# iracigt/ceres-raytracer

Measured on AMD Instinct MI355X. Metric: Mrays/sec (primary+shadow) on dragon.obj 1920x1080; 1/2/4/8-GPU scaling, higher is better.
Workload: dtype f32; 1 GPU; dragon_1080: dragon.obj 1920x1080 primary+shadow, 16 copies of the config view per step; views=config, W=1920, H=1080, row_block=1080, parallelism=one GPU, whole frames, float_framebuffer=True, streams=8

## Files before the change

ceres-raytracer_amd/__init__.py:

```python
import ctypes
import os
import sys

import numpy as np

_PKG = os.path.dirname(os.path.abspath(__file__))
LIB_PATH = os.environ.get("CERES_LIB") or os.path.join(_PKG, "libceres_hip.so")
CLI_PATH = os.path.join(_PKG, "render")

if _PKG not in sys.path:
    sys.path.insert(0, _PKG)
import configs

MODE_FULL, MODE_PRIMARY = 0, 1
MODE_ROBUST = 0x10
MODE_QBVH4 = 0x20
MODE_FMA = 0x40
ARITH_EXACT, ARITH_FMA = 0, 1


def cfg_mode(cfg, arith=ARITH_EXACT):
    return ((MODE_PRIMARY if cfg["mode"] == "primary" else MODE_FULL) | (MODE_ROBUST if cfg.get("robust") else 0)
            | (MODE_FMA if arith else 0))
SCENE_STATS = 1
SCENE_FIRST_ORDER = 2

EXPORTED_SYMBOLS = (
    "ceres_obj_load", "ceres_proc_mesh", "ceres_rotate_triangles", "ceres_bvh_build", "ceres_bvh_build_gpu",
    "ceres_bvh_build_device", "ceres_obj_load_gpu", "ceres_obj_parse_device", "ceres_rotate_triangles_device",
    "ceres_device_free", "ceres_camera_basis", "ceres_obj_load_f64", "ceres_proc_mesh_f64", "ceres_rotate_triangles_f64",
    "ceres_bvh_build_f64", "ceres_camera_basis_f64", "ceres_orbit_cameras_f64", "ceres_scene_create_f64",
    "ceres_render_f64", "ceres_render_records_f64", "ceres_obj_load_f64_arith", "ceres_proc_mesh_f64_arith",
    "ceres_rotate_triangles_f64_arith", "ceres_bvh_build_f64_arith", "ceres_camera_basis_f64_arith",
    "ceres_orbit_cameras_f64_arith",
    "ceres_free", "ceres_scene_create", "ceres_scene_create_device", "ceres_scene_destroy", "ceres_scene_info", "ceres_scene_shadow_stacks", "ceres_render_f32",
    "ceres_render_device", "ceres_render_batch_device", "ceres_render_multi_f32", "ceres_device_count", "ceres_assemble_rgb8_packed", "ceres_render_records", "ceres_tiling_local_rows",
    "ceres_scene_set_timing", "ceres_scene_read_timing", "ceres_scene_wave_log", "ceres_fetch_counters",
    "ceres_debug_compact_order", "ceres_debug_kept_tiles",
    "ceres_cpu_scene_create", "ceres_cpu_scene_destroy", "ceres_render_cpu_f32", "ceres_cpu_scene_create_f64",
    "ceres_render_cpu_f64",
    "ceres_orbit_cameras", "ceres_assemble_rgb8",
    "ceres_kernel_names", "ceres_last_error", "ceres_version",
    "ceres_obj_load_arith", "ceres_proc_mesh_arith", "ceres_rotate_triangles_arith", "ceres_bvh_build_arith",
    "ceres_camera_basis_arith", "ceres_orbit_cameras_arith", "ceres_content_hash",
    "ceres_bvh_build_gpu_arith", "ceres_bvh_build_device_arith", "ceres_obj_load_gpu_arith",
    "ceres_obj_parse_device_arith", "ceres_rotate_triangles_device_arith",
    "ceres_trace_rays", "ceres_trace_rays_device", "ceres_trace_rays_cpu",
    "ceres_trace_rays_f64", "ceres_trace_rays_f64_device", "ceres_trace_rays_cpu_f64",
    "ceres_shade_rays", "ceres_shade_rays_device", "ceres_shade_rays_cpu", "ceres_camera_rays",
    "ceres_shade_rays_f64", "ceres_shade_rays_f64_device", "ceres_shade_rays_cpu_f64", "ceres_camera_rays_f64",
    "ceres_scene_refit", "ceres_scene_refit_device", "ceres_scene_refit_f64", "ceres_scene_refit_f64_device",
    "ceres_cpu_scene_refit", "ceres_cpu_scene_refit_f64", "ceres_scene_read_boxes",
    "ceres_scene_sah_cost", "ceres_scene_rebuild", "ceres_scene_rebuild_device", "ceres_scene_update",
    "ceres_scene_update_device", "ceres_cpu_scene_sah_cost", "ceres_cpu_scene_rebuild", "ceres_cpu_scene_rebuild_f64",
    "ceres_cpu_scene_update", "ceres_cpu_scene_update_f64",
)

HIT_DTYPE = np.dtype([("prim", np.int32), ("t", np.float32), ("u", np.float32), ("v", np.float32)])
FLT_MAX = np.float32(np.finfo(np.float32).max)
HIT64_DTYPE = np.dtype([("prim", np.int32), ("pad", np.uint32), ("t", np.float64), ("u", np.float64), ("v", np.float64)])
DBL_MAX = np.float64(np.finfo(np.float64).max)


class CeresError(RuntimeError):
    pass


class _Stats(ctypes.Structure):
    _fields_ = [("rays", ctypes.c_uint64), ("hits", ctypes.c_uint64), ("primary_rays", ctypes.c_uint64),
                ("shadow_rays", ctypes.c_uint64), ("node_pairs", ctypes.c_uint64), ("tri_tests", ctypes.c_uint64),
                ("ms", ctypes.c_double)]


class _UpdateInfo(ctypes.Structure):
    _fields_ = [("cost", ctypes.c_double), ("built_cost", ctypes.c_double), ("new_cost", ctypes.c_double),
                ("rebuilt", ctypes.c_int32), ("reserved", ctypes.c_int32)]

    def as_dict(self):
        return dict(cost=self.cost, built_cost=self.built_cost, new_cost=self.new_cost, rebuilt=int(self.rebuilt))


class Tiling(ctypes.Structure):
    _fields_ = [("row_block", ctypes.c_uint32), ("rank", ctypes.c_uint32), ("world", ctypes.c_uint32),
                ("bands", ctypes.c_uint32)]


_lib = None
_fp = ctypes.POINTER(ctypes.c_float)
_dp = ctypes.POINTER(ctypes.c_double)
_u32p = ctypes.POINTER(ctypes.c_uint32)
_u64p = ctypes.POINTER(ctypes.c_uint64)
_sz = ctypes.c_size_t
_vp = ctypes.c_void_p


def build(verbose=False):
    import subprocess
    r = subprocess.run(["make", "-C", os.path.join(_PKG, "csrc"), "-j4", "all"], capture_output=True, text=True)
    if verbose or r.returncode:
        sys.stdout.write(r.stdout)
        sys.stderr.write(r.stderr)
    if r.returncode:
        raise CeresError("build of libceres_hip.so failed")


def lib():
    global _lib
    if _lib is not None:
        return _lib
    if not os.path.exists(LIB_PATH):
        raise CeresError(f"{LIB_PATH} is missing: run __graft_entry__.build() (no CPU fallback exists)")
    if "torch" not in sys.modules:
        try:
            import torch
        except ImportError:
            pass
    L = ctypes.CDLL(LIB_PATH)
    L.ceres_last_error.restype = ctypes.c_char_p
    L.ceres_version.restype = ctypes.c_char_p
    L.ceres_kernel_names.restype = ctypes.c_char_p
    L.ceres_obj_load.argtypes = [ctypes.c_char_p, ctypes.POINTER(_fp), ctypes.POINTER(_fp), ctypes.POINTER(_sz)]
    L.ceres_proc_mesh.argtypes = [ctypes.c_int, ctypes.POINTER(_fp), ctypes.POINTER(_fp), ctypes.POINTER(_sz)]
    L.ceres_rotate_triangles.argtypes = [_fp, _sz, ctypes.c_int, ctypes.c_float]
    L.ceres_bvh_build.argtypes = [_fp, _sz, ctypes.POINTER(_u32p), ctypes.POINTER(_sz), ctypes.POINTER(_u64p)]
    L.ceres_bvh_build_gpu.argtypes = [_fp, _sz, ctypes.POINTER(_u32p), ctypes.POINTER(_sz), ctypes.POINTER(_u64p),
                                      ctypes.c_int]
    L.ceres_bvh_build_device.argtypes = [_vp, _sz, _vp, _vp, ctypes.POINTER(_sz), _vp]
    L.ceres_obj_load_gpu.argtypes = [ctypes.c_char_p, ctypes.POINTER(_fp), ctypes.POINTER(_fp), ctypes.POINTER(_sz),
                                     ctypes.c_int]
    L.ceres_obj_parse_device.argtypes = [_vp, _sz, ctypes.POINTER(_vp), ctypes.POINTER(_vp), ctypes.POINTER(_sz), _vp]
    L.ceres_rotate_triangles_device.argtypes = [_vp, _sz, ctypes.c_int, ctypes.c_float, _vp]
    L.ceres_device_free.argtypes = [_vp]
    L.ceres_device_free.restype = None
    L.ceres_camera_basis.argtypes = [_fp, _fp, _fp, ctypes.c_float, _sz, _sz, _fp]
    L.ceres_obj_load_f64.argtypes = [ctypes.c_char_p, ctypes.POINTER(_dp), ctypes.POINTER(_dp), ctypes.POINTER(_sz)]
    L.ceres_proc_mesh_f64.argtypes = [ctypes.c_int, ctypes.POINTER(_dp), ctypes.POINTER(_dp), ctypes.POINTER(_sz)]
    L.ceres_rotate_triangles_f64.argtypes = [_dp, _sz, ctypes.c_int, ctypes.c_double]
    L.ceres_bvh_build_f64.argtypes = [_dp, _sz, ctypes.POINTER(_u64p), ctypes.POINTER(_sz), ctypes.POINTER(_u64p)]
    L.ceres_camera_basis_f64.argtypes = [_dp, _dp, _dp, ctypes.c_double, _sz, _sz, _dp]
    L.ceres_orbit_cameras_f64.argtypes = [_dp, _dp, _dp, _dp, ctypes.c_double, _sz, _sz, _dp, ctypes.c_double,
                                          ctypes.c_uint32, ctypes.c_int, _dp, _dp, _dp]
    L.ceres_obj_load_f64_arith.argtypes = [ctypes.c_char_p, ctypes.POINTER(_dp), ctypes.POINTER(_dp), ctypes.POINTER(_sz),
                                           ctypes.c_int]
    L.ceres_proc_mesh_f64_arith.argtypes = [ctypes.c_int, ctypes.POINTER(_dp), ctypes.POINTER(_dp), ctypes.POINTER(_sz),
                                            ctypes.c_int]
    L.ceres_rotate_triangles_f64_arith.argtypes = [_dp, _sz, ctypes.c_int, ctypes.c_double, ctypes.c_int]
    L.ceres_bvh_build_f64_arith.argtypes = [_dp, _sz, ctypes.POINTER(_u64p), ctypes.POINTER(_sz), ctypes.POINTER(_u64p),
                                            ctypes.c_int]
    L.ceres_camera_basis_f64_arith.argtypes = [_dp, _dp, _dp, ctypes.c_double, _sz, _sz, _dp, ctypes.c_int]
    L.ceres_orbit_cameras_f64_arith.argtypes = [_dp, _dp, _dp, _dp, ctypes.c_double, _sz, _sz, _dp, ctypes.c_double,
                                                ctypes.c_uint32, ctypes.c_int, _dp, _dp, _dp, ctypes.c_int]
    L.ceres_scene_create_f64.argtypes = [_dp, _sz, _dp, _vp, _sz, _u64p, ctypes.c_int, ctypes.c_uint32]
    L.ceres_scene_create_f64.restype = _vp
    L.ceres_render_f64.argtypes = [_vp, _dp, _dp, ctypes.c_int, _dp, ctypes.POINTER(ctypes.c_uint8), _sz, _sz,
                                   ctypes.POINTER(_Stats)]
    L.ceres_render_records_f64.argtypes = [_vp, _dp, _dp, ctypes.c_int, _sz, _sz, ctypes.POINTER(ctypes.c_int32), _dp,
                                           ctypes.POINTER(ctypes.c_int8), ctypes.POINTER(_Stats)]
    L.ceres_orbit_cameras.argtypes = [_fp, _fp, _fp, _fp, ctypes.c_float, _sz, _sz, _fp, ctypes.c_float,
                                      ctypes.c_uint32, ctypes.c_int, _fp, _fp, _fp]
    L.ceres_free.argtypes = [_vp]
    L.ceres_free.restype = None
    L.ceres_scene_create.argtypes = [_fp, _sz, _fp, _vp, _sz, _u64p, ctypes.c_int, ctypes.c_uint32]
    L.ceres_scene_create.restype = _vp
    L.ceres_scene_create_device.argtypes = [_vp, _sz, _vp, _vp, _sz, _vp, ctypes.c_int, ctypes.c_uint32, _vp]
    L.ceres_scene_create_device.restype = _vp
    L.ceres_scene_destroy.argtypes = [_vp]
    L.ceres_scene_destroy.restype = None
    L.ceres_scene_info.argtypes = [_vp, _u32p, _u32p, ctypes.POINTER(_sz), ctypes.POINTER(_sz)]
    L.ceres_scene_shadow_stacks.argtypes = [_vp, _u32p, _u32p]
    L.ceres_render_f32.argtypes = [_vp, _fp, _fp, ctypes.c_int, _fp, ctypes.POINTER(ctypes.c_uint8), _sz, _sz,
                                   ctypes.POINTER(_Stats)]
    L.ceres_render_device.argtypes = [_vp, _fp, _fp, ctypes.c_int, _sz, _sz, ctypes.POINTER(Tiling), _vp, _vp, _vp, _vp]
    L.ceres_render_batch_device.argtypes = [_vp, ctypes.c_uint32, _fp, _fp, ctypes.c_int, _sz, _sz,
                                            ctypes.POINTER(Tiling), _vp, _vp, _vp, _vp]
    L.ceres_render_multi_f32.argtypes = [ctypes.POINTER(_vp), ctypes.c_uint32, ctypes.c_uint32, _fp, _fp, ctypes.c_int, _fp,
                                         ctypes.POINTER(ctypes.c_uint8), _sz, _sz, ctypes.POINTER(_Stats)]
    L.ceres_assemble_rgb8_packed.argtypes = [_vp, _vp, ctypes.c_uint32, _sz, _sz, ctypes.c_uint32, ctypes.c_uint32, _vp]
    L.ceres_assemble_rgb8.argtypes = [_vp, _sz, _vp, ctypes.c_uint32, _sz, _sz, ctypes.c_uint32, ctypes.c_uint32, _vp]
    L.ceres_render_records.argtypes = [_vp, _fp, _fp, ctypes.c_int, _sz, _sz, ctypes.POINTER(ctypes.c_int32), _fp,
                                       ctypes.POINTER(ctypes.c_int8), ctypes.POINTER(_Stats)]
    L.ceres_tiling_local_rows.argtypes = [_sz, ctypes.POINTER(Tiling)]
    L.ceres_tiling_local_rows.restype = _sz
    L.ceres_scene_set_timing.argtypes = [_vp, ctypes.c_int]
    L.ceres_scene_read_timing.argtypes = [_vp, ctypes.POINTER(ctypes.c_double), ctypes.POINTER(ctypes.c_double),
                                          _u64p]
    L.ceres_scene_wave_log.argtypes = [_vp, _u64p, _sz, ctypes.POINTER(_sz)]
    L.ceres_fetch_counters.argtypes = [ctypes.c_int, _u64p, ctypes.c_int]
    if hasattr(L, "ceres_debug_compact_order"):
        L.ceres_debug_compact_order.argtypes = [_vp, _u32p, _u32p, _u32p, _sz]
        L.ceres_debug_kept_tiles.argtypes = [_sz, _sz, ctypes.c_uint32, ctypes.c_uint32, ctypes.POINTER(ctypes.c_uint16), _u32p,
                                             _u32p, _sz]
    L.ceres_cpu_scene_create.argtypes = [_fp, _sz, _fp, _vp, _sz, _u64p]
    L.ceres_cpu_scene_create.restype = _vp
    L.ceres_cpu_scene_destroy.argtypes = [_vp]
    L.ceres_cpu_scene_destroy.restype = None
    L.ceres_render_cpu_f32.argtypes = [_vp, _fp, _fp, ctypes.c_int, _fp, ctypes.POINTER(ctypes.c_uint8), _sz, _sz,
                                       ctypes.POINTER(_Stats), ctypes.c_int]
    L.ceres_cpu_scene_create_f64.argtypes = [_dp, _sz, _dp, _vp, _sz, _u64p]
    L.ceres_cpu_scene_create_f64.restype = _vp
    L.ceres_render_cpu_f64.argtypes = [_vp, _dp, _dp, ctypes.c_int, _dp, ctypes.POINTER(ctypes.c_uint8), _sz, _sz,
                                       ctypes.POINTER(_Stats), ctypes.c_int]
    L.ceres_trace_rays.argtypes = [_vp, _vp, _sz, ctypes.c_int, _vp, _vp, ctypes.POINTER(_Stats)]
    L.ceres_trace_rays_device.argtypes = [_vp, _vp, _sz, ctypes.c_int, _vp, _vp, _vp, _vp]
    L.ceres_trace_rays_cpu.argtypes = [_vp, _vp, _sz, ctypes.c_int, _vp, _vp, ctypes.POINTER(_Stats), ctypes.c_int]
    L.ceres_trace_rays_f64.argtypes = L.ceres_trace_rays.argtypes
    L.ceres_trace_rays_f64_device.argtypes = L.ceres_trace_rays_device.argtypes
    L.ceres_trace_rays_cpu_f64.argtypes = L.ceres_trace_rays_cpu.argtypes
    L.ceres_shade_rays.argtypes = [_vp, _vp, _sz, _fp, ctypes.c_int, _vp, _vp, _vp, _vp, ctypes.POINTER(_Stats)]
    L.ceres_shade_rays_device.argtypes = [_vp, _vp, _sz, _fp, ctypes.c_int, _vp, _vp, _vp, _vp, _vp, _vp]
    L.ceres_shade_rays_cpu.argtypes = L.ceres_shade_rays.argtypes + [ctypes.c_int]
    L.ceres_camera_rays.argtypes = [_fp, _sz, _sz, ctypes.c_int, _vp]
    L.ceres_shade_rays_f64.argtypes = [_vp, _vp, _sz, _dp, ctypes.c_int, _vp, _vp, _vp, _vp, ctypes.POINTER(_Stats)]
    L.ceres_shade_rays_f64_device.argtypes = [_vp, _vp, _sz, _dp, ctypes.c_int, _vp, _vp, _vp, _vp, _vp, _vp]
    L.ceres_shade_rays_cpu_f64.argtypes = L.ceres_shade_rays_f64.argtypes + [ctypes.c_int]
    L.ceres_camera_rays_f64.argtypes = [_dp, _sz, _sz, ctypes.c_int, _vp]
    L.ceres_scene_refit.argtypes = [_vp, _fp, _sz, _fp]
    L.ceres_scene_refit_f64.argtypes = [_vp, _dp, _sz, _dp]
    L.ceres_scene_refit_device.argtypes = [_vp, _vp, _sz, _vp, _vp]
    L.ceres_scene_refit_f64_device.argtypes = [_vp, _vp, _sz, _vp, _vp]
    L.ceres_cpu_scene_refit.argtypes = [_vp, _fp, _sz, _fp]
    L.ceres_cpu_scene_refit_f64.argtypes = [_vp, _dp, _sz, _dp]
    L.ceres_scene_read_boxes.argtypes = [_vp, _vp, ctypes.POINTER(_sz), _fp, ctypes.POINTER(_sz)]
    _ui = ctypes.POINTER(_UpdateInfo)
    L.ceres_scene_sah_cost.argtypes = [_vp, _dp, _vp]
    L.ceres_scene_rebuild.argtypes = [_vp, _fp, _sz, _fp, ctypes.c_int]
    L.ceres_scene_rebuild_device.argtypes = [_vp, _vp, _sz, _vp, ctypes.c_int, _vp]
    L.ceres_scene_update.argtypes = [_vp, _fp, _sz, _fp, ctypes.c_int, ctypes.c_double, _ui]
    L.ceres_scene_update_device.argtypes = [_vp, _vp, _sz, _vp, ctypes.c_int, ctypes.c_double, _ui, _vp]
    L.ceres_cpu_scene_sah_cost.argtypes = [_vp, _dp]
    L.ceres_cpu_scene_rebuild.argtypes = [_vp, _fp, _sz, _fp, ctypes.c_int]
    L.ceres_cpu_scene_rebuild_f64.argtypes = [_vp, _dp, _sz, _dp, ctypes.c_int]
    L.ceres_cpu_scene_update.argtypes = [_vp, _fp, _sz, _fp, ctypes.c_int, ctypes.c_double, _ui]
    L.ceres_cpu_scene_update_f64.argtypes = [_vp, _dp, _sz, _dp, ctypes.c_int, ctypes.c_double, _ui]
    L.ceres_content_hash.argtypes = [_vp, _sz]
    L.ceres_content_hash.restype = ctypes.c_uint64
    L.ceres_obj_load_arith.argtypes = L.ceres_obj_load.argtypes + [ctypes.c_int]
    L.ceres_proc_mesh_arith.argtypes = L.ceres_proc_mesh.argtypes + [ctypes.c_int]
    L.ceres_rotate_triangles_arith.argtypes = L.ceres_rotate_triangles.argtypes + [ctypes.c_int]
    L.ceres_bvh_build_arith.argtypes = L.ceres_bvh_build.argtypes + [ctypes.c_int]
    L.ceres_camera_basis_arith.argtypes = L.ceres_camera_basis.argtypes + [ctypes.c_int]
    L.ceres_orbit_cameras_arith.argtypes = L.ceres_orbit_cameras.argtypes + [ctypes.c_int]
    L.ceres_bvh_build_gpu_arith.argtypes = L.ceres_bvh_build_gpu.argtypes + [ctypes.c_int]
    L.ceres_bvh_build_device_arith.argtypes = L.ceres_bvh_build_device.argtypes + [ctypes.c_int]
    L.ceres_obj_load_gpu_arith.argtypes = L.ceres_obj_load_gpu.argtypes + [ctypes.c_int]
    L.ceres_obj_parse_device_arith.argtypes = L.ceres_obj_parse_device.argtypes + [ctypes.c_int]
    L.ceres_rotate_triangles_device_arith.argtypes = L.ceres_rotate_triangles_device.argtypes + [ctypes.c_int]
    _lib = L
    return L


def _check(rc):
    if rc != 0:
        raise CeresError(f"ceres error {rc}: {lib().ceres_last_error().decode()}")


def _p(a, t):
    return None if a is None else a.ctypes.data_as(ctypes.POINTER(t))


def _take(ptr, count, dtype):
    if count == 0:
        lib().ceres_free(ctypes.cast(ptr, _vp))
        return np.zeros(0, dtype)
    a = np.ctypeslib.as_array(ptr, shape=(count,)).copy().view(dtype)
    lib().ceres_free(ctypes.cast(ptr, _vp))
    return a


class Camera:

    def __init__(self, eye, dir, up, fov, dtype=np.float32, arith=ARITH_EXACT):
        self.dtype = np.dtype(dtype)
        self.eye = np.asarray(eye, self.dtype)
        self.dir = np.asarray(dir, self.dtype)
# ... 457 lines not shown
        rgb = np.empty(3 * W * H, np.uint8) if want_rgb8 else None
        st = _Stats()
        fn = lib().ceres_render_f64 if self.f64 else lib().ceres_render_f32
        _check(fn(self._h, _p(b, ct), _p(s, ct), int(mode), _p(px, ct), _p(rgb, ctypes.c_uint8), W, H, ctypes.byref(st)))
        return px, rgb, dict(rays=st.rays, hits=st.hits, primary_rays=st.primary_rays, shadow_rays=st.shadow_rays,
                             node_pairs=st.node_pairs, tri_tests=st.tri_tests, ms=st.ms)

    def records(self, basis12, sun, W, H, mode=MODE_FULL):
        dt, ct = (np.float64, ctypes.c_double) if self.f64 else (np.float32, ctypes.c_float)
        b = np.ascontiguousarray(basis12, dt)
        s = np.ascontiguousarray(sun, dt)
        prim = np.empty(W * H, np.int32)
        tuv = np.empty(3 * W * H, dt)
        sh = np.empty(W * H, np.int8)
        st = _Stats()
        fn = lib().ceres_render_records_f64 if self.f64 else lib().ceres_render_records
        _check(fn(self._h, _p(b, ct), _p(s, ct), int(mode), W, H, _p(prim, ctypes.c_int32), _p(tuv, ct),
                  _p(sh, ctypes.c_int8), ctypes.byref(st)))
        return prim, tuv.reshape(-1, 3), sh, dict(rays=st.rays, hits=st.hits, node_pairs=st.node_pairs,
                                                  tri_tests=st.tri_tests)

    def render_device(self, basis12, sun, W, H, mode=MODE_FULL, tiling=None, d_pixels=0, d_rgb8=0, d_counters=0,
                      stream=0):
        b = np.ascontiguousarray(basis12, np.float32)
        s = np.ascontiguousarray(sun, np.float32)
        t = ctypes.byref(tiling) if tiling is not None else None
        _check(lib().ceres_render_device(self._h, _p(b, ctypes.c_float), _p(s, ctypes.c_float), int(mode), W, H, t,
                                         d_pixels or None, d_rgb8 or None, d_counters or None, stream or None))

    def render_batch_device(self, basis12, sun3, W, H, mode=MODE_FULL, tiling=None, d_pixels=0, d_rgb8=0,
                            d_counters=0, stream=0):
        b = np.ascontiguousarray(basis12, np.float32).reshape(-1, 12)
        s = np.ascontiguousarray(sun3, np.float32).reshape(-1, 3)
        if b.shape[0] != s.shape[0]:
            raise CeresError("render_batch_device: %d cameras but %d suns" % (b.shape[0], s.shape[0]))
        t = ctypes.byref(tiling) if tiling is not None else None
        _check(lib().ceres_render_batch_device(self._h, b.shape[0], _p(b, ctypes.c_float), _p(s, ctypes.c_float),
                                               int(mode), W, H, t, d_pixels or None, d_rgb8 or None,
                                               d_counters or None, stream or None))

    def trace(self, rays, mode=0, closest=True, occluded=False):
        fn = lib().ceres_trace_rays_f64 if self.f64 else lib().ceres_trace_rays
        return _trace_host(lambda r, n, m, h, o, st: fn(self._h, r, n, m, h, o, st), rays, mode, closest, occluded, self.f64)

    def trace_device(self, d_rays32, n_rays, mode=0, d_hits16=0, d_occluded=0, d_counters=0, stream=0):
        fn = lib().ceres_trace_rays_f64_device if self.f64 else lib().ceres_trace_rays_device
        _check(fn(self._h, d_rays32 or None, int(n_rays), int(mode), d_hits16 or None, d_occluded or None,
                  d_counters or None, stream or None))

    def shade(self, rays, sun, mode=0, pixels=True, rgb8=False, hits=False, status=False):
        fn = lib().ceres_shade_rays_f64 if self.f64 else lib().ceres_shade_rays
        return _shade_host(lambda r, n, s, m, px, q, h, stt, st: fn(self._h, r, n, s, m, px, q, h, stt, st),
                           rays, sun, mode, pixels, rgb8, hits, status, self.f64)

    def shade_device(self, d_rays32, n_rays, sun, mode=0, d_pixels=0, d_rgb8=0, d_hits16=0, d_status=0, d_counters=0,
                     stream=0):
        dt, ct = (np.float64, ctypes.c_double) if self.f64 else (np.float32, ctypes.c_float)
        fn = lib().ceres_shade_rays_f64_device if self.f64 else lib().ceres_shade_rays_device
        s = np.ascontiguousarray(sun, dt).reshape(3)
        _check(fn(self._h, d_rays32 or None, int(n_rays), _p(s, ct), int(mode), d_pixels or None, d_rgb8 or None,
                  d_hits16 or None, d_status or None, d_counters or None, stream or None))

    def set_timing(self, on):
        _check(lib().ceres_scene_set_timing(self._h, 1 if on else 0))

    def wave_log(self, max_waves=1 << 16):
        out = np.zeros(8 * max_waves, np.uint64)
        n = _sz()
        _check(lib().ceres_scene_wave_log(self._h, _p(out, ctypes.c_uint64), max_waves, ctypes.byref(n)))
        return out[: 8 * n.value].reshape(-1, 8)

    def compact_order(self):
        info = np.zeros(8, np.uint32)
        _check(lib().ceres_debug_compact_order(self._h, _p(info, ctypes.c_uint32), None, None, 0))
        if not info[0]:
            return None
        cap = int(info[6]) + 16
        order, source = np.zeros(cap, np.uint32), np.zeros(cap, np.uint32)
        _check(lib().ceres_debug_compact_order(self._h, _p(info, ctypes.c_uint32), _p(order, ctypes.c_uint32),
                                               _p(source, ctypes.c_uint32), cap))
        return {"host_tiles": int(info[1]), "device_tiles": int(info[2]), "groups": int(info[3]), "tpw": int(info[4]),
                "deal": int(info[5]), "order": order[:(int(info[2]) + 7) // 8 * 8], "source": source[:int(info[6])]}

    def read_timing(self):
        p, q, n = ctypes.c_double(), ctypes.c_double(), ctypes.c_uint64()
        _check(lib().ceres_scene_read_timing(self._h, ctypes.byref(p), ctypes.byref(q), ctypes.byref(n)))
        return p.value, q.value, n.value


def source_sha16(repo=None):
    import glob
    import hashlib
    repo = repo or os.path.dirname(_PKG)
    inc = sorted(glob.glob(os.path.join(repo, "include", "*.h")) + glob.glob(os.path.join(repo, "include", "ceres", "*.hpp")))
    csrc = os.path.join(_PKG, "csrc")
    names = sorted(n for n in os.listdir(csrc) if n.endswith((".cpp", ".hip", ".hpp")))
    h = hashlib.sha256()
    for f in inc + [os.path.join(csrc, n) for n in names]:
        with open(f, "rb") as fh:
            h.update(fh.read())
    return h.hexdigest()[:16]


def native_provenance():
    import hashlib
    v = lib().ceres_version().decode()
    built = v.rsplit(" src ", 1)[1] if " src " in v else None
    with open(LIB_PATH, "rb") as fh:
        so_sha = hashlib.sha256(fh.read()).hexdigest()
    now = source_sha16()
    return {"lib": os.path.relpath(LIB_PATH, os.path.dirname(_PKG)), "version": v, "so_sha256": so_sha,
            "built_from_sources_sha16": built, "tree_sources_sha16": now, "built_from_this_tree": built == now}


FETCH_KINDS = ("bvh2_vector", "bvh4_vector", "bvh4_scalar", "tri_vector", "tri_scalar", "shade_vector",
               "store_vector", "order_scalar")
COUNT_LIB_PATH = os.path.join(_PKG, "variants", "libceres_hip_count.so")


def fetch_counters(device=0, reset=True):
    out = np.zeros(8, np.uint64)
    _check(lib().ceres_fetch_counters(int(device), _p(out, ctypes.c_uint64), 1 if reset else 0))
    return {k: int(v) for k, v in zip(FETCH_KINDS, out)}


def render_multi(scenes, basis12, sun, W, H, row_block=8, mode=MODE_FULL, want_pixels=True, want_rgb8=True):
    b = np.ascontiguousarray(basis12, np.float32)
    s = np.ascontiguousarray(sun, np.float32)
    px = np.empty(3 * W * H, np.float32) if want_pixels else None
    rgb = np.empty(3 * W * H, np.uint8) if want_rgb8 else None
    hs = (_vp * len(scenes))(*[sc._h for sc in scenes])
    st = _Stats()
    _check(lib().ceres_render_multi_f32(hs, len(scenes), int(row_block), _p(b, ctypes.c_float), _p(s, ctypes.c_float),
                                        int(mode), _p(px, ctypes.c_float), _p(rgb, ctypes.c_uint8), W, H,
                                        ctypes.byref(st)))
    return px, rgb, dict(rays=st.rays, hits=st.hits, primary_rays=st.primary_rays, shadow_rays=st.shadow_rays,
                         node_pairs=st.node_pairs, tri_tests=st.tri_tests, ms=st.ms)


def orbit_cameras(camera, sun, W, H, n_frames, axis=(0, 1, 0), step_deg=None, rotate_first=True, want_dirs=False):
    n = int(n_frames)
    step = np.float32(360.0) / np.float32(n) if step_deg is None else np.float32(step_deg)
    b = np.zeros((n, 12), np.float32)
    s3 = np.zeros((n, 3), np.float32)
    d3 = np.zeros((n, 3), np.float32)
    ax = np.asarray(axis, np.float32)
    sn = np.asarray(sun, np.float32)
    _check(lib().ceres_orbit_cameras_arith(_p(camera.eye, ctypes.c_float), _p(camera.dir, ctypes.c_float),
                                           _p(camera.up, ctypes.c_float), _p(sn, ctypes.c_float), camera.fov, W, H,
                                           _p(ax, ctypes.c_float), float(step), n, 1 if rotate_first else 0,
                                           _p(b, ctypes.c_float), _p(s3, ctypes.c_float), _p(d3, ctypes.c_float),
                                           camera.arith))
    return (b, s3, d3) if want_dirs else (b, s3)


def bench_views(camera, sun, W, H, F, basis0=None):
    F = int(F)
    b12 = np.zeros((F, 12), np.float32)
    s3 = np.zeros((F, 3), np.float32)
    steps = np.asarray([configs.orbit_step(f, F) for f in range(F)], np.float32)
    b12[0] = camera.basis(W, H) if basis0 is None else np.asarray(basis0, np.float32)
    s3[0] = np.asarray(sun, np.float32)
    for f in range(1, F):
        b, s = orbit_cameras(camera, sun, W, H, 2, axis=configs.BENCH_AXIS, step_deg=float(steps[f]),
                             rotate_first=False)
        b12[f], s3[f] = b[1], s[1]
    return b12, s3, steps


def pose(cfg, frame=0, arith=ARITH_EXACT):
# ... 91 lines not shown
```

ceres-raytracer_amd/csrc/ceres_types.hpp:

```cpp
#pragma once
#include <cstddef>
#include <cstdint>
#include <vector>

namespace ceres {

struct Tri48 {
    float p0[3], e1[3], e2[3], n[3];
};
static_assert(sizeof(Tri48) == 48, "Tri48");

struct RefNode {
    float bounds[6];
    uint32_t primitive_count;
    uint32_t first_child_or_primitive;
};
static_assert(sizeof(RefNode) == 32, "RefNode");

struct alignas(16) SiblingPair {
    float lb[6];
    float rb[6];
    uint32_t lcount, lfirst;
    uint32_t rcount, rfirst;
};
// ... 43 lines not shown
            const int group = w == kNode4Empty ? 2 : (w & kNode4MaxCount) ? 0 : 1;
            if (group != pass) continue;
            t.lo_x[k] = r.lo_x[c]; t.hi_x[k] = r.hi_x[c];
            t.lo_y[k] = r.lo_y[c]; t.hi_y[k] = r.hi_y[c];
            t.lo_z[k] = r.lo_z[c]; t.hi_z[k] = r.hi_z[c];
            t.child[k] = w;
            if (src) ts[k] = src[c];
            nl += group == 0;
            ++k;
        }
    t.nleaf = nl;
    t.unused[0] = t.unused[1] = t.unused[2] = 0;
    r = t;
    if (src) for (int c = 0; c < 4; ++c) src[c] = ts[c];
}

struct alignas(64) QNode4 {
    float ox, oy, oz, sx;
    float sy, sz;
    uint32_t qlx, qhx;
    uint32_t qly, qhy, qlz, qhz;
    uint32_t child[4];
};
static_assert(sizeof(QNode4) == 64, "QNode4");

constexpr int kShards = 32;
struct alignas(128) Shard {
    uint32_t queued;
    uint32_t error;
    unsigned long long hits;
    unsigned long long pairs;
    unsigned long long tests;
    uint32_t pad[24];
};
static_assert(sizeof(Shard) == 128, "Shard");

constexpr int kMaxFrames = 64;
constexpr int kFramesPerLaunch = 56;
struct FrameCam {
    float eye[3], dir[3], iu[3], iv[3], sun[3];
};

constexpr uint32_t kTileXBits = 13, kTileYBits = 13;
constexpr uint32_t pack_tile(uint32_t f, uint32_t y, uint32_t x) { return (f << (kTileXBits + kTileYBits)) | (y << kTileXBits) | x; }

struct CullRect { uint16_t i0, i1, j0, j1; };

struct KParams {
    FrameCam cam[kFramesPerLaunch];
    CullRect cull_rect[kFramesPerLaunch];
    uint32_t frames;
    uint32_t W, H;
    uint32_t row_block, rank, world, local_rows;
    uint32_t bands;
    uint32_t band_magic;
    uint32_t row_blocks_per_frame;
    uint32_t stack_entries;
    uint32_t root_leaf_count, root_leaf_first;
    float root_box[6];
    uint32_t root_box_ok;
    uint32_t cull;
    uint32_t shadow_stack_entries;
    uint32_t steal_first;
    uint32_t packets;
    uint32_t tiles_x;
    uint32_t lds_entries;
    uint32_t tile_packed;
    const uint32_t* tile_order;
    const SiblingPair* pairs;
    const Node4* nodes4;
    const QNode4* qnodes4;
    const Tri48* tris;
    const uint32_t* orig;
    const float* norms;
    float* pixels;
    uint8_t* rgb8;
    Shard* shards;
    int32_t* rec_prim;
    float* rec_tuv;
    int8_t* rec_shadow;
    unsigned long long* wave_log;
    uint32_t fill_stride, fill_magic;
    uint32_t n_tiles;
};

struct CompactArgs {
    uint32_t* buf;
    uint32_t tpw;
    uint32_t deal;
    uint32_t want_tiles;
    uint32_t off_result, off_counts, off_rows;
};
static_assert(sizeof(KParams) + sizeof(CompactArgs) <= 4096, "KParams + CompactArgs must fit the 4 KB kernel-argument limit");
static_assert(sizeof(KParams) <= 4096, "KParams must fit the 4 KB kernel-argument limit");

struct DeviceLayout {
    float root_box[6] = {0, 0, 0, 0, 0, 0};
    SiblingPair* pairs = nullptr;
    Node4* nodes4 = nullptr;
    Tri48* tris = nullptr;
    uint32_t* orig = nullptr;
    size_t n_pairs = 0, n_nodes4 = 0;
    uint32_t depth = 0, stack4 = 0, root_leaf_count = 0, root_leaf_first = 0;
    uint32_t* src4 = nullptr;
};
#ifdef __HIPCC__
int relayout_device(const Tri48* d_tris, uint32_t n_tri, const RefNode* d_nodes, uint32_t n_nodes, const uint32_t* d_prim,
                    hipStream_t stream, DeviceLayout& out);
#endif

int relayout_bvh(const RefNode* nodes, size_t n_nodes, const uint64_t* prim, size_t n_tri, const Tri48* tris,
                 std::vector<SiblingPair>& pairs, std::vector<Tri48>& leaf_tris, std::vector<uint32_t>& orig,
                 uint32_t& depth, uint32_t& root_leaf_count, uint32_t& root_leaf_first);
int build_shadow_bvh4(const std::vector<SiblingPair>& pairs, std::vector<Node4>& out, uint32_t& stack_bound,
                      uint32_t& not_collapsed, std::vector<uint32_t>* src4 = nullptr);
int order_shadow_bvh4(std::vector<Node4>& nodes, uint32_t& first_bound, std::vector<uint32_t>* src4 = nullptr);
int relayout_bvh64(const RefNode64* nodes, size_t n_nodes, const uint64_t* prim, size_t n_tri, const Tri96* tris,
                   std::vector<SiblingPair64>& pairs, std::vector<Tri96>& leaf_tris, std::vector<uint32_t>& orig,
                   uint32_t& depth, uint32_t& root_leaf_count, uint32_t& root_leaf_first);

}
```

ceres-raytracer_amd/csrc/render_hip.hip:

```cpp
#include <hip/hip_runtime.h>

#include <algorithm>
#include <chrono>
#include <cfloat>
#include <cmath>
#include <cstdint>
#include <cstdlib>
#include <cstring>
#include <new>
#include <string>
#include <type_traits>
#include <vector>

#include "ceres_render.h"
#include "ceres_types.hpp"
#include "host_common.hpp"
#include "pow24.hpp"

#pragma clang fp contract(off)

#ifndef CERES_COUNTING
#define CERES_COUNTING 0
#endif
#ifndef CERES_TILES_PER_WAVE
#define CERES_TILES_PER_WAVE 4
#endif
#ifndef CERES_TPW_BY_SIZE
#define CERES_TPW_BY_SIZE 1
#endif
#ifndef CERES_FRAME_MAJOR_PIXELS
#define CERES_FRAME_MAJOR_PIXELS (1u << 20)
#endif
#ifndef CERES_SPLIT_UNIFORM
#define CERES_SPLIT_UNIFORM 1
#endif
#ifndef CERES_ROOT_TEST
#define CERES_ROOT_TEST 1
#endif
#ifndef CERES_OCTANT_SLAB
#define CERES_OCTANT_SLAB 3
#endif
#ifndef CERES_SHADOW_PACKET
#define CERES_SHADOW_PACKET 1
#endif
#ifndef CERES_TRUST_STACK_BOUND
#define CERES_TRUST_STACK_BOUND 1
#endif
#ifndef CERES_PAIR_STORES
#define CERES_PAIR_STORES 1
#endif
#ifndef CERES_STACK_GUARD
#define CERES_STACK_GUARD CERES_COUNTING
#endif
#ifndef CERES_ASSEMBLE_NT
#define CERES_ASSEMBLE_NT 0
#endif
#ifndef CERES_LOCAL_ORDER
#define CERES_LOCAL_ORDER 1
#endif
#ifndef CERES_LOCAL_CHUNK_BATCH
#define CERES_LOCAL_CHUNK_BATCH 128
#endif
#ifndef CERES_XCD_GROUP_TILES
#define CERES_XCD_GROUP_TILES 16
#endif
#ifndef CERES_LOCAL_CHUNK_SOLO
#define CERES_LOCAL_CHUNK_SOLO 16
#endif
#ifndef CERES_RCP_UNIFORM
#define CERES_RCP_UNIFORM 2
#endif
#ifndef CERES_RCP_IFTHEN
#define CERES_RCP_IFTHEN 1
#endif
#ifndef CERES_PK_PACKET
#define CERES_PK_PACKET 1
#endif
#ifndef CERES_LOAD_ALWAYS
#define CERES_LOAD_ALWAYS 1
#endif
#ifndef CERES_CULL
#define CERES_CULL 1
#endif
#ifndef CERES_COMPACT
#define CERES_COMPACT 1
#endif
#ifndef CERES_TRI_SELECT
#define CERES_TRI_SELECT 1
#endif

namespace ceres {

char* error_buffer() {
    static thread_local char buf[kErrorBufferSize] = "";
    return buf;
}

namespace dev {

constexpr int kBlock = 256;

struct F3 { float x, y, z; };
__device__ __forceinline__ F3 operator+(F3 a, F3 b) { return {a.x + b.x, a.y + b.y, a.z + b.z}; }
__device__ __forceinline__ F3 operator-(F3 a, F3 b) { return {a.x - b.x, a.y - b.y, a.z - b.z}; }
__device__ __forceinline__ F3 operator*(F3 a, float s) { return {a.x * s, a.y * s, a.z * s}; }
__device__ __forceinline__ float dot(F3 a, F3 b) { float s = a.x * b.x; s += a.y * b.y; s += a.z * b.z; return s; }
__device__ __forceinline__ F3 cross(F3 a, F3 b) { return {a.y * b.z - a.z * b.y, a.z * b.x - a.x * b.z, a.x * b.y - a.y * b.x}; }
template <bool kU = false>
__device__ __forceinline__ float rcp_exact(float x) {
    const uint32_t m = __float_as_uint(x) & 0x7fffffffu;
    if (kU) {
        const bool slow = m - 0x00800000u >= 0x7e000000u - 0x00800000u;
        if (__builtin_expect(__ballot(slow) != 0, 0)) {
            const float q = 1.0f / x;
            const float r0 = __builtin_amdgcn_rcpf(x);
            return slow ? q : __builtin_fmaf(__builtin_fmaf(-x, r0, 1.0f), r0, r0);
        }
        const float r0 = __builtin_amdgcn_rcpf(x);
        return __builtin_fmaf(__builtin_fmaf(-x, r0, 1.0f), r0, r0);
    }
    if constexpr (CERES_RCP_IFTHEN) {
        const float r0 = __builtin_amdgcn_rcpf(x);
        float r = __builtin_fmaf(__builtin_fmaf(-x, r0, 1.0f), r0, r0);
        if (__builtin_expect(m - 0x00800000u >= 0x7e000000u - 0x00800000u, 0)) r = 1.0f / x;
        return r;
    }
    if (__builtin_expect(m - 0x00800000u >= 0x7e000000u - 0x00800000u, 0)) return 1.0f / x;
    const float r0 = __builtin_amdgcn_rcpf(x);
    return __builtin_fmaf(__builtin_fmaf(-x, r0, 1.0f), r0, r0);
}

__device__ __forceinline__ float rcp_fast(float x) {
    const float r0 = __builtin_amdgcn_rcpf(x);
    return __builtin_fmaf(__builtin_fmaf(-x, r0, 1.0f), r0, r0);
}
__device__ __forceinline__ F3 normalize(F3 v) { float inv = 1.0f / sqrtf(dot(v, v)); return v * inv; }
__device__ __forceinline__ F3 f3(const float* p) { return {p[0], p[1], p[2]}; }

template <bool kG> __device__ __forceinline__ float dotA(F3 a, F3 b) {
    if constexpr (kG) return __builtin_fmaf(a.z, b.z, __builtin_fmaf(a.x, b.x, a.y * b.y));
    else return dot(a, b);
}
template <bool kG> __device__ __forceinline__ float dotB(F3 a, F3 b) {
    if constexpr (kG) return __builtin_fmaf(a.z, b.z, __builtin_fmaf(a.y, b.y, a.x * b.x));
    else return dot(a, b);
}
template <bool kG> __device__ __forceinline__ F3 crossG(F3 a, F3 b) {
    if constexpr (kG)
        return {__builtin_fmaf(a.y, b.z, -(a.z * b.y)), __builtin_fmaf(a.z, b.x, -(a.x * b.z)),
                __builtin_fmaf(a.x, b.y, -(a.y * b.x))};
    else return cross(a, b);
}
template <bool kG> __device__ __forceinline__ F3 normalizeG(F3 v) { float inv = 1.0f / sqrtf(dotA<kG>(v, v)); return v * inv; }

__device__ __forceinline__ bool uniform_id(uint32_t id, uint32_t& r) {
    r = __builtin_amdgcn_readfirstlane(id);
    return __ballot(id != r) == 0;
}
enum FetchKind : int {
    kFBvh2V = 0,
    kFBvh4V,
    kFBvh4S,
    kFTriV,
    kFTriS,
    kFShadeV,
    kFStoreV,
    kFOrderS,
    kFKinds
};
// ... 130 lines not shown
    const float u = dotA<kG>(r, tr.e2) * inv_det;
    const float v = dotB<kG>(r, tr.e1) * inv_det;
    const float w = 1.0f - u - v;
    const float t = dotA<kG>(tr.n, c) * inv_det;
    const float x1 = u >= 0 ? v : -1.0f;
    const float x2 = x1 >= 0 ? w : -1.0f;
    const float x3 = x2 >= 0 ? t : -1.0f;
    return __ballot((x3 >= tmin) & (x3 <= tmax));
}

template <bool kRobust>
struct Slab {
    float ix, iy, iz;
    float sx, sy, sz;
    F3 o;
};
__device__ __forceinline__ float pad_ulps2(float x) {
    return isfinite(x) ? __uint_as_float(__float_as_uint(x) + 2u) : x;
}
template <bool kRobust, class RK = CamRay>
__device__ __forceinline__ Slab<kRobust> make_slab(F3 o, F3 d) {
    Slab<kRobust> s;
    if constexpr (kRobust) {
        s.ix = 1.0f / d.x; s.iy = 1.0f / d.y; s.iz = 1.0f / d.z;
        s.sx = pad_ulps2(s.ix); s.sy = pad_ulps2(s.iy); s.sz = pad_ulps2(s.iz);
    } else {
        auto safe_inv = [](float x) {
            const float c = fabsf(x) < FLT_EPSILON ? copysignf(FLT_EPSILON, x) : x;
            if constexpr (RK::kUnitDir) return rcp_fast(c);
            else return rcp_exact<false>(c);
        };
        s.ix = safe_inv(d.x); s.iy = safe_inv(d.y); s.iz = safe_inv(d.z);
        s.sx = (-o.x) * s.ix; s.sy = (-o.y) * s.iy; s.sz = (-o.z) * s.iz;
    }
    s.o = o;
    return s;
}
template <bool kRobust, int kOct = -1>
__device__ __forceinline__ void slab_box(const Slab<kRobust>& s, float lox, float hix, float loy, float hiy, float loz,
                                         float hiz, float tmin, float tmax, float& e, float& x) {
    if constexpr (!kRobust && kOct >= 0) {
        const float nx = (kOct & 1) ? hix : lox, fx = (kOct & 1) ? lox : hix;
        const float ny = (kOct & 2) ? hiy : loy, fy = (kOct & 2) ? loy : hiy;
        const float nz = (kOct & 4) ? hiz : loz, fz = (kOct & 4) ? loz : hiz;
        e = fmaxf(__builtin_fmaf(nx, s.ix, s.sx), fmaxf(__builtin_fmaf(ny, s.iy, s.sy), fmaxf(__builtin_fmaf(nz, s.iz, s.sz), tmin)));
        x = fminf(__builtin_fmaf(fx, s.ix, s.sx), fminf(__builtin_fmaf(fy, s.iy, s.sy), fminf(__builtin_fmaf(fz, s.iz, s.sz), tmax)));
    } else if constexpr (kRobust) {
        const bool nx = __float_as_uint(s.ix) >> 31, ny = __float_as_uint(s.iy) >> 31, nz = __float_as_uint(s.iz) >> 31;
        const float ex = ((nx ? hix : lox) - s.o.x) * s.ix, xx = ((nx ? lox : hix) - s.o.x) * s.sx;
        const float ey = ((ny ? hiy : loy) - s.o.y) * s.iy, xy = ((ny ? loy : hiy) - s.o.y) * s.sy;
        const float ez = ((nz ? hiz : loz) - s.o.z) * s.iz, xz = ((nz ? loz : hiz) - s.o.z) * s.sz;
        e = fmaxf(ex, fmaxf(ey, fmaxf(ez, tmin)));
        x = fminf(xx, fminf(xy, fminf(xz, tmax)));
    } else {
        const float a0 = __builtin_fmaf(lox, s.ix, s.sx), a1 = __builtin_fmaf(hix, s.ix, s.sx);
        const float b0 = __builtin_fmaf(loy, s.iy, s.sy), b1 = __builtin_fmaf(hiy, s.iy, s.sy);
        const float c0 = __builtin_fmaf(loz, s.iz, s.sz), c1 = __builtin_fmaf(hiz, s.iz, s.sz);
        e = fmaxf(fminf(a0, a1), fmaxf(fminf(b0, b1), fmaxf(fminf(c0, c1), tmin)));
        x = fminf(fmaxf(a0, a1), fminf(fmaxf(b0, b1), fminf(fmaxf(c0, c1), tmax)));
    }
}

template <typename Fn>
__device__ __forceinline__ bool with_uniform_octant(const Slab<false>& s, Fn&& fn) {
    const uint32_t oct = (__float_as_uint(s.ix) >> 31) | (__float_as_uint(s.iy) >> 31) << 1 | (__float_as_uint(s.iz) >> 31) << 2;
    uint32_t r;
    if (!uniform_id(oct, r)) return false;
    switch (r) {
        case 0: fn(std::integral_constant<int, 0>{}); break;
        case 1: fn(std::integral_constant<int, 1>{}); break;
        case 2: fn(std::integral_constant<int, 2>{}); break;
        case 3: fn(std::integral_constant<int, 3>{}); break;
        case 4: fn(std::integral_constant<int, 4>{}); break;
        case 5: fn(std::integral_constant<int, 5>{}); break;
        case 6: fn(std::integral_constant<int, 6>{}); break;
        default: fn(std::integral_constant<int, 7>{}); break;
    }
    return true;
}

template <bool kAnyHit, bool kStats, int kS = kBlock, typename StkT = uint32_t*, bool kRobust = false, int kOct = -1,
          bool kG = false, class RK = CamRay, class PT>
__device__ __forceinline__ bool trace(const PT& P, F3 o, F3 d, StkT stk, Hit& best,
                                      uint32_t& n_pairs, uint32_t& n_tests, bool& overflow, RK rk = RK{}) {
    const float tmin = rk.tmin();
    float tmax = rk.tmax();
    bool have = false;
    constexpr bool kU = CERES_RCP_UNIFORM == 1 || (CERES_RCP_UNIFORM == 2 && kOct == -2);
    if (P.root_leaf_count) {
        if (kStats) n_tests += P.root_leaf_count;
        for (uint32_t k = P.root_leaf_first; k < P.root_leaf_first + P.root_leaf_count; ++k) {
            float t, u, v;
            CERES_COUNT_V(kFTriV, 48);
            if (tri_test<kG, kU, RK>(load_tri(P.tris + k), o, d, tmin, tmax, t, u, v)) {
                best = {k, t, u, v}; have = true;
                if (kAnyHit) return true;
                tmax = t;
            }
        }
        return have;
    }
    const Slab<kRobust> sl = make_slab<kRobust, RK>(o, d);
    if constexpr (!kRobust && kOct == -1 && (CERES_OCTANT_SLAB & 1)) {
        bool r = false;
        if (with_uniform_octant(sl, [&](auto k) {
                r = trace<kAnyHit, kStats, kS, StkT, kRobust, decltype(k)::value, kG, RK>(P, o, d, stk, best, n_pairs, n_tests, overflow, rk);
            }))
            return r;
    }
    if (P.root_box_ok) {
        float e, x;
        slab_box<kRobust, kOct>(sl, P.root_box[0], P.root_box[1], P.root_box[2], P.root_box[3], P.root_box[4],
                          P.root_box[5], tmin, tmax, e, x);
        if (!(e <= x)) {
            if (kStats) ++n_pairs;
            return false;
        }
    }
    uint32_t sp = 0;
    if (CERES_TRI_SELECT && !kAnyHit) best.slot = kNoSlot;
    const float4* q = reinterpret_cast<const float4*>(P.pairs);
    float4 A = q[0], B = q[1], C = q[2];
    uint4 L = reinterpret_cast<const uint4*>(q)[3];
    CERES_COUNT_V(kFBvh2V, 64);
    while (true) {
        if (kStats) ++n_pairs;
        const uint32_t top = stk[(sp ? sp - 1 : 0) * kS];
        float le, lx, re, rx;
        slab_box<kRobust, kOct>(sl, A.x, A.y, A.z, A.w, B.x, B.y, tmin, tmax, le, lx);
        slab_box<kRobust, kOct>(sl, B.z, B.w, C.x, C.y, C.z, C.w, tmin, tmax, re, rx);
        const bool hit_l = le <= lx, hit_r = re <= rx;
        const bool go_l = hit_l && !L.x, go_r = hit_r && !L.z;
        const bool both = go_l && go_r, none = !go_l && !go_r;
        const bool swap = le > re;
        const bool done = none && sp == 0;
        const uint32_t near = both ? (swap ? L.w : L.y) : (go_l ? L.y : L.w);
        const uint32_t nxt = none ? top : near;
        if (kStats || !CERES_TRUST_STACK_BOUND || RK::kClampStack) {
            overflow |= both && sp >= P.stack_entries;
            stk[(sp < P.stack_entries ? sp : P.stack_entries) * kS] = swap ? L.y : L.w;
            sp = both ? (sp < P.stack_entries ? sp + 1 : sp) : (none ? (sp ? sp - 1 : 0) : sp);
        } else {
            stk[sp * kS] = swap ? L.y : L.w;
            sp = sp + (both ? 1u : 0u) - (none ? 1u : 0u);
        }
        const uint32_t nl = hit_l ? L.x : 0u, nr = hit_r ? L.z : 0u;
        const uint32_t n_leaf = nl + nr, k2 = L.w - nl;
        if (kStats) n_tests += n_leaf;
        float4 nA, nB, nC;
        uint4 nL;
        if (RK::kLoadAlways || (CERES_LOAD_ALWAYS && kOct != -2)) {
            const float4* nq = reinterpret_cast<const float4*>(P.pairs + (done ? 0u : nxt));
            nA = nq[0]; nB = nq[1]; nC = nq[2]; nL = reinterpret_cast<const uint4*>(nq)[3];
            CERES_COUNT_V(kFBvh2V, 64);
        } else if (!done) {
            const float4* nq = reinterpret_cast<const float4*>(P.pairs + nxt);
            nA = nq[0]; nB = nq[1]; nC = nq[2]; nL = reinterpret_cast<const uint4*>(nq)[3];
            CERES_COUNT_V(kFBvh2V, 64);
        }
        for (uint32_t j = 0; j < n_leaf; ++j) {
            const uint32_t idx = (j < nl ? L.y : k2) + j;
            float t, u, v;
            if (CERES_TRI_SELECT && !kAnyHit) {
                const bool h = tri_test_u<kG, kU, RK>(P.tris, idx, o, d, tmin, tmax, t, u, v);
                best.slot = h ? idx : best.slot; best.t = h ? t : best.t;
                best.u = h ? u : best.u; best.v = h ? v : best.v;
                tmax = h ? t : tmax;
                continue;
            }
            if (tri_test_u<kG, kU, RK>(P.tris, idx, o, d, tmin, tmax, t, u, v)) {
                best = {idx, t, u, v}; have = true;
                if (kAnyHit) return true;
                tmax = t;
            }
        }
        if (done) break;
        A = nA; B = nB; C = nC; L = nL;
    }
    if (CERES_TRI_SELECT && !kAnyHit) return best.slot != kNoSlot;
    return have;
}

template <bool kStats, int kS, typename StkT, bool kRobust, int kOct, bool kG>
__device__ __forceinline__ bool guarded_trace(const KParams& P, F3 o, F3 d, StkT stk, Hit& best, uint32_t& n_pairs,
                                              uint32_t& n_tests, bool& overflow) {
    constexpr bool kGuard = !kStats && CERES_TRUST_STACK_BOUND && CERES_STACK_GUARD;
    const uint32_t slot = P.stack_entries * kS;
    if (kGuard) stk[slot] = stack_guard<StkT>();
    const bool hit = trace<false, kStats, kS, StkT, kRobust, kOct, kG>(P, o, d, stk, best, n_pairs, n_tests, overflow);
    if (kGuard) overflow |= uint32_t(stk[slot]) != stack_guard<StkT>();
    return hit;
}

struct N4 { float4 lx, hx, ly, hy, lz, hz; uint4 ch; };
__device__ __forceinline__ N4 load_n4(const Node4* n) {
    const float4* q = reinterpret_cast<const float4*>(n);
    const uint4* u = reinterpret_cast<const uint4*>(n);
    return {q[0], q[1], q[2], q[3], q[4], q[5], u[6]};
}
__device__ __forceinline__ uint32_t n4_count(uint32_t w) { return w & kNode4MaxCount; }
__device__ __forceinline__ uint32_t n4_first(uint32_t w) { return w >> kNode4CountBits; }
__device__ __forceinline__ N4 load_n4_u(const Node4* nodes, uint32_t cur) {
    uint32_t r;
    if (uniform_id(cur, r)) {
        CERES_COUNT_S(kFBvh4S, 112);
        const Node4* q = nodes + r;
        return {sload_f4(q, 0), sload_f4(q, 1), sload_f4(q, 2), sload_f4(q, 3), sload_f4(q, 4), sload_f4(q, 5),
                sload_u4(q, 6)};
    }
    CERES_COUNT_V(kFBvh4V, 112);
    return load_n4(nodes + cur);
}
__device__ __forceinline__ float4 qdecode(uint32_t w, float scale, float origin) {
    return make_float4(__builtin_fmaf(float(w & 0xffu), scale, origin), __builtin_fmaf(float((w >> 8) & 0xffu), scale, origin),
                       __builtin_fmaf(float((w >> 16) & 0xffu), scale, origin), __builtin_fmaf(float(w >> 24), scale, origin));
}
__device__ __forceinline__ N4 load_q4_u(const QNode4* nodes, uint32_t cur) {
    float4 a, b;
    uint4 c, d;
    uint32_t r;
    if (uniform_id(cur, r)) {
        CERES_COUNT_S(kFBvh4S, 64);
        const QNode4* q = nodes + r;
        a = sload_f4(q, 0); b = sload_f4(q, 1); c = sload_u4(q, 2); d = sload_u4(q, 3);
    } else {
        CERES_COUNT_V(kFBvh4V, 64);
        const float4* q = reinterpret_cast<const float4*>(nodes + cur);
        a = q[0]; b = q[1];
        c = reinterpret_cast<const uint4*>(q)[2]; d = reinterpret_cast<const uint4*>(q)[3];
    }
    return {qdecode(__float_as_uint(b.z), a.w, a.x), qdecode(__float_as_uint(b.w), a.w, a.x),
            qdecode(c.x, b.x, a.y), qdecode(c.y, b.x, a.y), qdecode(c.z, b.y, a.z), qdecode(c.w, b.y, a.z), d};
}
template <bool kQ, class PT>
__device__ __forceinline__ N4 load_shadow_node(const PT& P, uint32_t cur) {
    if constexpr (kQ) return load_q4_u(P.qnodes4, cur);
    else return load_n4_u(P.nodes4, cur);
}
__device__ __forceinline__ float pick(float4 v, uint32_t c) { return c == 0 ? v.x : c == 1 ? v.y : c == 2 ? v.z : v.w; }
__device__ __forceinline__ uint32_t pick(uint4 v, uint32_t c) { return c == 0 ? v.x : c == 1 ? v.y : c == 2 ? v.z : v.w; }

template <bool kStats, int kS = kBlock, typename StkT = uint32_t*, bool kRobust = false, bool kQ = false, int kOct = -1,
          bool kG = false, class RK = CamRay, class PT>
__device__ __forceinline__ bool trace_any4(const PT& P, F3 o, F3 d, StkT stk, uint32_t& n_pairs,
                                           uint32_t& n_tests, bool& overflow, RK rk = RK{}) {
    const float tmin = rk.tmin(), tmax = rk.tmax();
    if (P.root_leaf_count) {
        Hit h;
        return trace<true, kStats, kS, StkT, kRobust, -1, kG, RK>(P, o, d, stk, h, n_pairs, n_tests, overflow, rk);
    }
    const Slab<kRobust> sl = make_slab<kRobust, RK>(o, d);
    if constexpr (!kRobust && kOct == -1 && (CERES_OCTANT_SLAB & 2)) {
        bool r = false;
        if (with_uniform_octant(sl, [&](auto k) {
                r = trace_any4<kStats, kS, StkT, kRobust, kQ, decltype(k)::value, kG, RK>(P, o, d, stk, n_pairs, n_tests, overflow, rk);
            }))
            return r;
    }
    uint32_t sp = 0, cur = 0;
    while (true) {
        if (kStats) ++n_pairs;
        float e[4];
        uint32_t leaf_mask = 0, inner_mask = 0;
        auto classify = [&](const float4& LX, const float4& HX, const float4& LY, const float4& HY, const float4& LZ,
                            const float4& HZ, const uint4& CH) {
            const float lx[4] = {LX.x, LX.y, LX.z, LX.w}, hx[4] = {HX.x, HX.y, HX.z, HX.w};
            const float ly[4] = {LY.x, LY.y, LY.z, LY.w}, hy[4] = {HY.x, HY.y, HY.z, HY.w};
            const float lz[4] = {LZ.x, LZ.y, LZ.z, LZ.w}, hz[4] = {HZ.x, HZ.y, HZ.z, HZ.w};
            const uint32_t chw[4] = {CH.x, CH.y, CH.z, CH.w};
#pragma unroll
            for (int c = 0; c < 4; ++c) {
                float x;
// ... 535 lines not shown
            uint32_t mail = 0, donor = 0;
            const uint32_t r = __popcll(idle & lt_mask);
            const bool thief = !active && r < n_don;
            if (thief) { mail = L.mail[wbase + r]; donor = L.from[wbase + r]; }
            const float ox = __shfl(w.o.x, donor, 64), oy = __shfl(w.o.y, donor, 64), oz = __shfl(w.o.z, donor, 64);
            const float dx = __shfl(w.d.x, donor, 64), dy = __shfl(w.d.y, donor, 64), dz = __shfl(w.d.z, donor, 64);
            const float jx = __shfl(w.ix, donor, 64), jy = __shfl(w.iy, donor, 64), jz = __shfl(w.iz, donor, 64);
            const float tx = __shfl(w.sx, donor, 64), ty = __shfl(w.sy, donor, 64), tz = __shfl(w.sz, donor, 64);
            const uint32_t down = __shfl(owner, donor, 64);
            if (thief) {
                w.o = F3{ox, oy, oz}; w.d = F3{dx, dy, dz};
                w.ix = jx; w.iy = jy; w.iz = jz; w.sx = tx; w.sy = ty; w.sz = tz;
                owner = down;
                cur = mail;
                top = bot = cnt = 0;
                active = true;
            }
            __builtin_amdgcn_wave_barrier();
        }
    }
    __builtin_amdgcn_wave_barrier();
}

template <bool kRobust = false, bool kG = false>
__device__ __forceinline__ RayWork make_shadow_ray(F3 o, F3 sun) {
    RayWork w;
    w.o = o;
    w.d = normalizeG<kG>(sun - o);
    const Slab<kRobust> sl = make_slab<kRobust>(o, w.d);
    w.ix = sl.ix; w.iy = sl.iy; w.iz = sl.iz; w.sx = sl.sx; w.sy = sl.sy; w.sz = sl.sz;
    return w;
}

template <typename StkT, bool kRobust, bool kQ, bool kG>
__device__ __forceinline__ bool shadow_packet(const KParams& P, bool hit, const RayWork& w, uint32_t lane, bool& blocked) {
    if constexpr (!kRobust && !kQ && CERES_SHADOW_PACKET && std::is_same<StkT, uint16_t*>::value) {
        const uint64_t act = __ballot(hit);
        if (!act) { blocked = false; return true; }
        const uint32_t oct = (__float_as_uint(w.ix) >> 31) | (__float_as_uint(w.iy) >> 31) << 1 |
                             (__float_as_uint(w.iz) >> 31) << 2;
        const int first = __builtin_ctzll(act);
        const uint32_t oct0 = uint32_t(__builtin_amdgcn_readlane(int(oct), first));
        const bool finite = isfinite(w.ix) && isfinite(w.iy) && isfinite(w.iz) && isfinite(w.sx) && isfinite(w.sy) &&
                            isfinite(w.sz);
        if (!P.packets || P.shadow_stack_entries > 64 || P.root_leaf_count || __ballot(hit && (oct != oct0 || !finite)))
            return false;
        auto bc = [&](float x) { return hit ? x : __int_as_float(__builtin_amdgcn_readlane(__float_as_int(x), first)); };
        const F3 o{bc(w.o.x), bc(w.o.y), bc(w.o.z)}, d{bc(w.d.x), bc(w.d.y), bc(w.d.z)};
        const Slab<false> sl{bc(w.ix), bc(w.iy), bc(w.iz), bc(w.sx), bc(w.sy), bc(w.sz), o};
        uint64_t occ = 0;
        switch (oct0) {
            case 0: occ = packet_any4<0, kG>(P, sl, o, d, act, lane); break;
            case 1: occ = packet_any4<1, kG>(P, sl, o, d, act, lane); break;
            case 2: occ = packet_any4<2, kG>(P, sl, o, d, act, lane); break;
            case 3: occ = packet_any4<3, kG>(P, sl, o, d, act, lane); break;
            case 4: occ = packet_any4<4, kG>(P, sl, o, d, act, lane); break;
            case 5: occ = packet_any4<5, kG>(P, sl, o, d, act, lane); break;
            case 6: occ = packet_any4<6, kG>(P, sl, o, d, act, lane); break;
            default: occ = packet_any4<7, kG>(P, sl, o, d, act, lane); break;
        }
        blocked = (occ >> lane) & 1u;
        return true;
    }
    return false;
}

template <bool kG, bool kBands = false>
__device__ __forceinline__ void shade_pixel(const KParams& P, uint32_t f, uint32_t lr, uint32_t i, uint32_t pix,
                                            bool blocked, F3 sun_line, uint32_t slot, float hu, float hv,
                                            uint32_t& occluded, float c[3]) {
    if (P.rec_shadow) P.rec_shadow[pix] = blocked ? 1 : 0;
    c[0] = c[1] = c[2] = 0.f;
    if (blocked) {
        ++occluded;
    } else {
        const F3 view = primary_dir<kG>(P, f, i, global_row<kBands>(P, f, lr));
        CERES_COUNT_V(kFShadeV, 40);
        shade<kG>(sun_line, P.norms + 9 * size_t(P.orig[slot]), view, hu, hv, c);
    }
}

constexpr int kFusedB = 64;
constexpr size_t kLdsPerCu = 160 * 1024;
template <bool kStats, typename StkT, int kMinW, bool kRobust, bool kSteal, bool kQ, bool kG, int kTPWo = 0, bool kBands = false>
__global__ __launch_bounds__(kFusedB) __attribute__((amdgpu_waves_per_eu(kMinW))) void ceres_fused(const KParams P) {
    constexpr int kB = kFusedB;
    constexpr bool kPacketsCompiled = !kStats && !kSteal && !kRobust && !kQ && CERES_SHADOW_PACKET && std::is_same<StkT, uint16_t*>::value;
    extern __shared__ __attribute__((aligned(16))) uint32_t lds[];
    __shared__ StealLdsT<kB> L;
    const uint32_t lane = threadIdx.x, tid = lane;
    constexpr uint32_t kTPWp = (kStats || kSteal) ? 1 : kTPWo ? uint32_t(kTPWo) : uint32_t(CERES_TILES_PER_WAVE);
    constexpr bool kPair = CERES_PAIR_STORES && !kStats && !kSteal && kTPWp >= 2 && std::is_same<StkT, uint16_t*>::value;
    __shared__ typename std::conditional<kPair, PairStash, NoStash>::type S;
    auto tile_pixel = [&](uint32_t t, uint32_t& f_, uint32_t& lr_, uint32_t& i_) {
        uint32_t by_, bx_;
        if (P.tile_packed) {
            bx_ = t & ((1u << kTileXBits) - 1u);
            by_ = (t >> kTileXBits) & ((1u << kTileYBits) - 1u);
            f_ = t >> (kTileXBits + kTileYBits);
        } else {
            const uint32_t per_frame_ = P.tiles_x * P.row_blocks_per_frame;
            f_ = t / per_frame_;
            const uint32_t rem = t - f_ * per_frame_;
            by_ = rem / P.tiles_x; bx_ = rem - by_ * P.tiles_x;
        }
        const uint32_t lx = (lane & 1) | ((lane >> 1) & 2) | ((lane >> 2) & 4), ly = ((lane >> 1) & 1) | ((lane >> 2) & 2) | ((lane >> 3) & 4);
        i_ = bx_ * 8u + lx;
        lr_ = by_ * 8u + ly;
        return i_ < P.W && lr_ < P.local_rows && (!kBands || global_row<true>(P, f_, lr_) < P.H);
    };
    bool stashed = false;
    auto flush = [&](uint32_t t_prev) {
        if constexpr (kPair) {
            uint32_t pf, plr, pi;
            if (tile_pixel(t_prev, pf, plr, pi)) store_pixel(P, pf, plr, pi, S.c[0][lane], S.c[1][lane], S.c[2][lane]);
        }
        stashed = false;
    };
    auto emit = [&](uint32_t q, bool last, uint32_t t_prev, bool act, uint32_t f_, uint32_t lr_, uint32_t i_, float c0, float c1,
                    float c2) {
        if constexpr (kPair) {
            if (!(q & 1u) && !last) {
                S.c[0][lane] = c0; S.c[1][lane] = c1; S.c[2][lane] = c2;
                stashed = true;
                return;
            }
            if (stashed) flush(t_prev);
        }
        if (act) store_pixel(P, f_, lr_, i_, c0, c1, c2);
    };
    StkT stk;
    if constexpr (std::is_same<StkT, Stk24>::value)
        stk = Stk24{reinterpret_cast<uint16_t*>(lds) + tid,
                    reinterpret_cast<uint8_t*>(lds) + size_t(P.lds_entries) * kB * 2 + tid};
    else
        stk = reinterpret_cast<StkT>(lds) + tid;
    constexpr uint32_t kTile = 8;
    constexpr uint32_t kTPW = (kStats || kSteal) ? 1 : kTPWo ? uint32_t(kTPWo) : uint32_t(CERES_TILES_PER_WAVE);
    const uint32_t n_tiles = P.n_tiles;
    uint32_t group = blockIdx.x;
    if constexpr (!kStats) {
        const uint32_t tile_groups = (n_tiles + kTPW - 1) / kTPW;
        if (P.fill_stride) {
            const uint32_t oct = blockIdx.x >> 3, x = blockIdx.x & 7u, nfo = (gridDim.x >> 3) - (tile_groups + 7u) / 8u;
            const uint32_t q = __umulhi(oct, P.fill_magic), r = oct - q * P.fill_stride;
            if (r == P.fill_stride - 1 && q < nfo) {
                fill_culled_rows<kBands>(P, q * 8u + x, lane);
                return;
            }
            group = (oct - (q < nfo ? q : nfo)) * 8u + x;
            if (group >= tile_groups) return;
        } else if (blockIdx.x >= tile_groups) {
            fill_culled_rows<kBands>(P, blockIdx.x - tile_groups, lane);
            return;
        }
    }
    uint32_t n_shadow = 0, occluded = 0, n_pairs = 0, n_tests = 0;
    bool overflow = false;
    static_assert(kTPW == 1 || kTPW == 2 || kTPW == 4 || kTPW == 8, "CERES_TILES_PER_WAVE must be 1, 2, 4 or 8");
    uint4 tiles4 = make_uint4(0, 0, 0, 0), tiles4b = make_uint4(0, 0, 0, 0);
    if constexpr (kTPW == 8) {
        tiles4 = sload_u4(P.tile_order + 8 * size_t(group), 0);
        tiles4b = sload_u4(P.tile_order + 8 * size_t(group), 1);
    } else if constexpr (kTPW == 4) {
        tiles4 = sload_u4(P.tile_order + 4 * size_t(group), 0);
    } else if constexpr (kTPW == 2) {
        tiles4.x = sload_u32(P.tile_order + 2 * size_t(group));
        tiles4.y = sload_u32(P.tile_order + 2 * size_t(group) + 1);
    } else {
        tiles4.x = sload_u32(P.tile_order + group);
    }
    CERES_COUNT_S(kFOrderS, 4 * kTPW);
    const uint32_t n_here = kTPW == 1 || n_tiles - group * kTPW >= kTPW ? kTPW : n_tiles - group * kTPW;
    for (uint32_t q = 0; q < n_here; ++q) {
    const uint4 tq = q < 4 ? tiles4 : tiles4b;
    const uint32_t qq = q & 3;
    const uint32_t t = kTPW == 1 ? tiles4.x : qq == 0 ? tq.x : qq == 1 ? tq.y : qq == 2 ? tq.z : tq.w;
    const uint32_t qp = (q - 1) & 3;
    const uint4 tp = q - 1 < 4 ? tiles4 : tiles4b;
    const uint32_t t_prev = qp == 0 ? tp.x : qp == 1 ? tp.y : qp == 2 ? tp.z : tp.w;
    uint32_t f, lr, i;
    bool active = tile_pixel(t, f, lr, i);
    uint32_t px = (f * P.local_rows + lr) * P.W + i;
    auto redecode = [&]() {
        if constexpr (CERES_LEAN_WRITES) {
            uint32_t tr = t;
            asm volatile("" : "+s"(tr));
            active = tile_pixel(tr, f, lr, i);
            px = (f * P.local_rows + lr) * P.W + i;
        }
    };
    bool hit = false;
    Hit h{0, 0.f, 0.f, 0.f};
    RayWork w{};
    uint64_t t_start = 0;
    if (kStats && P.wave_log) t_start = __builtin_amdgcn_s_memrealtime();
    const bool last_q = q + 1 == n_here;
    if (!kStats && P.cull && tile_misses_root(P, f, i >> 3, tile_rows_hit<kBands>(P, f, lr))) {
        if (stashed) flush(t_prev);
        continue;
    }
    if (active) {
        const F3 view = primary_dir<kG>(P, f, i, global_row<kBands>(P, f, lr));
        constexpr int kOctMode = (!kSteal || (CERES_OCTANT_SLAB & 4)) ? -1 : -2;
        hit = guarded_trace<kStats, kB, StkT, kRobust, kOctMode, kG>(P, f3(P.cam[f].eye), view, stk, h, n_pairs,
                                                                   n_tests, overflow);
        if (P.rec_prim) {
            redecode();
            P.rec_prim[px] = hit ? int32_t(P.orig[h.slot]) : -1;
            P.rec_tuv[3 * size_t(px)] = hit ? h.t : 0.f;
            P.rec_tuv[3 * size_t(px) + 1] = hit ? h.u : 0.f;
            P.rec_tuv[3 * size_t(px) + 2] = hit ? h.v : 0.f;
            P.rec_shadow[px] = -1;
        }
        if (hit) {
            CERES_COUNT_V(kFShadeV, 48);
            const TriV tr = load_tri(P.tris + h.slot);
            const F3 normal = normalizeG<kG>(tr.n);
            w = make_shadow_ray<kRobust, kG>(hit_point<kG>(tr, normal, h.u, h.v), f3(P.cam[f].sun));
        }
    }
    const uint32_t n_shadow_t = __popcll(__ballot(hit));
    n_shadow += n_shadow_t;
    uint64_t t_primary = 0;
    uint32_t prim_pairs = n_pairs, shadow_iters = 0;
    if (kStats && P.wave_log) t_primary = __builtin_amdgcn_s_memrealtime();
    bool pk_blocked = false;
    const bool pk = !kStats && !kSteal && shadow_packet<StkT, kRobust, kQ, kG>(P, hit, w, lane, pk_blocked);
    if (pk)
        L.blocked[tid] = pk_blocked ? 1u : 0u;
    else if constexpr (kSteal)
        steal_traverse<kStats, kB, StkT, kRobust, kQ, kG>(P, hit, w, stk, L, tid, lane, n_pairs, n_tests, overflow, &shadow_iters);
    else
        L.blocked[tid] = hit && trace_any4<kStats, kB, StkT, kRobust, kQ, kPacketsCompiled ? -2 : -1, kG>(
                                    P, w.o, w.d, stk, n_pairs, n_tests, overflow) ? 1u : 0u;
    redecode();
    float col[3] = {0.f, 0.f, 0.f};
    if (hit) shade_pixel<kG, kBands>(P, f, lr, i, px, L.blocked[tid] != 0, w.d, h.slot, h.u, h.v, occluded, col);
    emit(q, last_q, t_prev, active, f, lr, i, col[0], col[1], col[2]);
    if (kStats && P.wave_log) {
        const uint64_t t_end = __builtin_amdgcn_s_memrealtime();
        uint32_t mx = prim_pairs;
        for (int off = 32; off > 0; off >>= 1) mx = max(mx, uint32_t(__shfl_xor(int(mx), off, 64)));
        const uint32_t sp = wave_sum(prim_pairs), ss = wave_sum(n_pairs - prim_pairs);
        if (lane == 0) {
            unsigned long long* wl = P.wave_log + 8 * size_t(blockIdx.x);
            wl[0] = t_start; wl[1] = t_primary; wl[2] = t_end; wl[3] = mx; wl[4] = shadow_iters;
            wl[5] = n_shadow_t; wl[6] = sp; wl[7] = ss;
        }
    }
    }
    const uint32_t wo = wave_sum(occluded);
    const uint32_t shard = blockIdx.x % kShards;
    if (lane == 0 && n_shadow) {
        atomicAdd(&P.shards[shard].queued, n_shadow);
        atomicAdd(&P.shards[shard].hits, (unsigned long long)(n_shadow + wo));
    }
    if (kStats) {
        const uint32_t wp = wave_sum(n_pairs), wt = wave_sum(n_tests);
        if (lane == 0) {
            atomicAdd(&P.shards[shard].pairs, (unsigned long long)wp);
            atomicAdd(&P.shards[shard].tests, (unsigned long long)wt);
        }
    }
    if (overflow) atomicOr(&P.shards[shard].error, 1u);
}

__device__ __forceinline__ void order_tile(const KParams& P, uint32_t t, uint32_t& f, uint32_t& by, uint32_t& bx) {
    if (P.tile_packed) {
        bx = t & ((1u << kTileXBits) - 1u);
        by = (t >> kTileXBits) & ((1u << kTileYBits) - 1u);
        f = t >> (kTileXBits + kTileYBits);
    } else {
        const uint32_t per_frame = P.tiles_x * P.row_blocks_per_frame;
        f = t / per_frame;
        const uint32_t rem = t - f * per_frame;
        by = rem / P.tiles_x; bx = rem - by * P.tiles_x;
    }
}

__global__ __launch_bounds__(256) void ceres_cull_rows(const KParams P, const CompactArgs A) {
    const uint32_t lane = threadIdx.x & 63u, task = blockIdx.x * 4u + (threadIdx.x >> 6);
    const uint32_t tile_rows = P.row_blocks_per_frame;
    const uint32_t f = task / tile_rows, by = task - f * tile_rows;
    if (f >= P.frames) return;
    const bool hit = tile_rows_hit(P, f, by * 8u + (lane & 7u));
    if (lane == 0) A.buf[A.off_rows + task] = hit ? 1u : 0u;
}

__device__ __forceinline__ bool group_kept(const KParams& P, const CompactArgs& A, uint32_t g) {
    bool keep = false;
    for (uint32_t i = 0; i < A.tpw; ++i) {
        const uint32_t p = g * A.tpw + i;
        if (p >= P.n_tiles) break;
        uint32_t f, by, bx;
        order_tile(P, P.tile_order[p], f, by, bx);
        if (f >= P.frames || by >= P.row_blocks_per_frame) continue;
        keep = keep || !tile_misses_root(P, f, bx, A.buf[A.off_rows + f * P.row_blocks_per_frame + by] != 0u);
    }
    return keep;
}

constexpr uint32_t kCompactBlock = 1024;

__device__ __forceinline__ uint32_t block_sum_256(uint32_t x, uint32_t* sh) {
    x = wave_sum(x);
    __syncthreads();
    if ((threadIdx.x & 63u) == 0) sh[threadIdx.x >> 6] = x;
    __syncthreads();
    return sh[0] + sh[1] + sh[2] + sh[3];
}

__global__ __launch_bounds__(256) void ceres_order_count(const KParams P, const CompactArgs A) {
    __shared__ uint32_t sh[4];
    const uint32_t groups = (P.n_tiles + A.tpw - 1u) / A.tpw, g0 = blockIdx.x * kCompactBlock + threadIdx.x * 4u;
    uint32_t c = 0;
    for (uint32_t k = 0; k < 4u; ++k)
        if (g0 + k < groups && group_kept(P, A, g0 + k)) ++c;
    c = block_sum_256(c, sh);
    if (threadIdx.x == 0) A.buf[A.off_counts + blockIdx.x] = c;
}

__global__ __launch_bounds__(256) void ceres_order_compact(const KParams P, const CompactArgs A) {
    __shared__ uint32_t sh[4];
    __shared__ uint32_t wsum[4];
    const uint32_t groups = (P.n_tiles + A.tpw - 1u) / A.tpw, g0 = blockIdx.x * kCompactBlock + threadIdx.x * 4u;
    uint32_t before = 0, total = 0;
    for (uint32_t b = threadIdx.x; b < gridDim.x; b += 256u) {
        const uint32_t c = A.buf[A.off_counts + b];
        total += c;
        if (b < blockIdx.x) before += c;
    }
    before = block_sum_256(before, sh);
    total = block_sum_256(total, sh);
    const uint32_t rem = P.n_tiles % A.tpw;
    const uint32_t short_last = rem && group_kept(P, A, groups - 1u) ? A.tpw - rem : 0u;
    const uint32_t kept_tiles = total * A.tpw - short_last;
    const uint32_t run = 8u * A.deal, dealt = A.deal ? kept_tiles / (run * A.tpw) * run : 0u;
    bool keep[4];
    uint32_t mine = 0;
    for (uint32_t k = 0; k < 4u; ++k) {
        keep[k] = g0 + k < groups && group_kept(P, A, g0 + k);
        mine += keep[k] ? 1u : 0u;
    }
    const uint32_t lane = threadIdx.x & 63u, wave = threadIdx.x >> 6;
    uint32_t x = mine;
    for (uint32_t off = 1; off < 64u; off <<= 1) {
        const uint32_t y = __shfl_up(x, off, 64);
        if (lane >= off) x += y;
    }
    if (lane == 63u) wsum[wave] = x;
    __syncthreads();
    uint32_t k = before + x - mine;
    for (uint32_t w = 0; w < wave; ++w) k += wsum[w];
    for (uint32_t j = 0; j < 4u; ++j) {
        if (!keep[j]) continue;
        uint32_t slot = k++;
        if (slot < dealt) {
            const uint32_t r = slot % run;
            slot = slot - r + (r % A.deal) * 8u + r / A.deal;
        }
        for (uint32_t i = 0; i < A.tpw; ++i) {
            const uint32_t p = (g0 + j) * A.tpw + i;
            A.buf[slot * A.tpw + i] = p < P.n_tiles ? P.tile_order[p] : 0u;
        }
    }
    if (blockIdx.x == gridDim.x - 1u) {
        const uint32_t end = total * A.tpw, padded = (kept_tiles + 7u) / 8u * 8u;
        if (end + threadIdx.x < padded) A.buf[end + threadIdx.x] = 0u;
        if (threadIdx.x == 0) {
// ... 168 lines not shown
            q[0] = quantize(col[0]); q[1] = quantize(col[1]); q[2] = quantize(col[2]);
        }
        if (P.status) P.status[r] = hit ? (blocked ? 2 : 1) : 0;
    }
    if (P.counters) {
        const uint32_t nh = __popcll(__ballot(hit)), nb = __popcll(__ballot(blocked));
        if (lane == 0 && nh) {
            atomicAdd(&P.counters[0], (unsigned long long)nh);
            atomicAdd(&P.counters[1], (unsigned long long)(nh + nb));
            atomicAdd(&P.counters[3], (unsigned long long)nh);
        }
        if (blockIdx.x == 0 && lane == 0) {
            atomicAdd(&P.counters[0], (unsigned long long)P.n_rays);
            atomicAdd(&P.counters[2], (unsigned long long)P.n_rays);
        }
        if (overflow) atomicOr(&P.counters[6], 1ull);
    }
}

__device__ __forceinline__ uint32_t rank_rows(uint32_t H, uint32_t rb, uint32_t r, uint32_t world) {
    const uint32_t nb = (H + rb - 1) / rb;
    if (r >= nb) return 0;
    const uint32_t mine = (nb - 1 - r) / world + 1;
    const bool has_last = (nb - 1) % world == r;
    return mine * rb - (has_last ? nb * rb - H : 0);
}

template <bool kVec, bool kPacked = false>
__global__ __launch_bounds__(256) void ceres_assemble(const uint8_t* __restrict__ src, size_t rank_stride,
                                                      uint8_t* __restrict__ dst, uint32_t frames, uint32_t H,
                                                      uint32_t row_bytes, uint32_t rb, uint32_t world) {
    const uint32_t units = kVec ? row_bytes / 16 : row_bytes;
    for (uint32_t oy = blockIdx.y; oy < frames * H; oy += gridDim.y) {
        const uint32_t f = oy / H, y = oy - f * H;
        const uint32_t j = H - 1 - y;
        const uint32_t b = j / rb, r = b % world;
        const uint32_t k = (b / world) * rb + j % rb;
        const uint32_t n = rank_rows(H, rb, r, world);
        size_t base = size_t(r) * rank_stride;
        if (kPacked) {
            base = 0;
            for (uint32_t p = 0; p < r; ++p) base += size_t(frames) * rank_rows(H, rb, p, world) * row_bytes;
        }
        const uint8_t* s = src + base + (size_t(f) * n + (n - 1 - k)) * row_bytes;
        uint8_t* d = dst + size_t(oy) * row_bytes;
        for (uint32_t u = blockIdx.x * blockDim.x + threadIdx.x; u < units; u += gridDim.x * blockDim.x) {
            if (kVec) {
#if CERES_ASSEMBLE_NT
                const U4v x = __builtin_nontemporal_load(reinterpret_cast<const U4v*>(s) + u);
                __builtin_nontemporal_store(x, reinterpret_cast<U4v*>(d) + u);
#else
                reinterpret_cast<uint4*>(d)[u] = reinterpret_cast<const uint4*>(s)[u];
#endif
            }
            else d[u] = s[u];
        }
    }
}

}
}

using namespace ceres;

#include "scene_internal.hpp"

namespace {

#define HIP_TRY(expr)                                                                         \
    do {                                                                                      \
        hipError_t e_ = (expr);                                                               \
        if (e_ != hipSuccess) return set_error(CERES_EHIP, "%s: %s", #expr, hipGetErrorString(e_)); \
    } while (0)

template <typename T>
void dfree(T*& p) { if (p) { (void)hipFree(p); p = nullptr; } }

}

void ceres::scene_release(ceres_scene* s) {
    if (!s) return;
    (void)hipSetDevice(s->device);
    dfree(s->d_pairs64); dfree(s->d_tris64); dfree(s->d_norms64);
    dfree(s->d_src4); dfree(s->d_refit_levels); dfree(s->d_refit_root); dfree(s->d_cost);
    if (s->d_refit_stage) { (void)hipFree(s->d_refit_stage); s->d_refit_stage = nullptr; }
    for (auto& o : s->orders) dfree(o.d);
    for (auto& d : s->retired) dfree(d);
    for (auto& c : s->compact) dfree(c.d);
    s->orders.clear(); s->retired.clear(); s->retired_bytes = 0; s->compact.clear();
    dfree(s->d_pairs); dfree(s->d_nodes4); dfree(s->d_qnodes4); dfree(s->d_tris); dfree(s->d_orig); dfree(s->d_norms);
    dfree(s->d_shards); dfree(s->d_counters); dfree(s->d_wave_log); dfree(s->d_pixels); dfree(s->d_rgb8);
    for (auto e : s->ev_pool) (void)hipEventDestroy(e);
    for (auto e : s->ev_used) (void)hipEventDestroy(e);
    s->ev_pool.clear(); s->ev_used.clear();
    for (auto e : s->band_events) (void)hipEventDestroy(e);
    s->band_events.clear();
    dfree(s->d_band_counters);
    dfree(s->d_lit); dfree(s->d_lit_count);
    if (s->h_lit_pinned) (void)hipHostFree(s->h_lit_pinned);
    s->h_lit_pinned = nullptr;
    if (s->h_small) (void)hipHostFree(s->h_small);
    s->h_small = nullptr;
    if (s->ev_count) (void)hipEventDestroy(s->ev_count);
    s->ev_count = nullptr;
    if (s->copy_stream) (void)hipStreamDestroy(s->copy_stream);
    s->copy_stream = nullptr;
    if (s->stream) (void)hipStreamDestroy(s->stream);
    s->stream = nullptr;
}

namespace {

size_t local_rows_of(size_t H, uint32_t rb, uint32_t rank, uint32_t world);
size_t local_rows_of(size_t H, const ceres_tiling& t) {
    if (t.bands && t.world > 1) return t.row_block;
    return local_rows_of(H, t.row_block, t.rank, t.world);
}
size_t local_rows_of(size_t H, uint32_t rb, uint32_t rank, uint32_t world) {
    const size_t nblocks = (H + rb - 1) / rb;
    size_t rows = 0;
    for (size_t b = rank; b < nblocks; b += world) rows += std::min<size_t>(rb, H - b * rb);
    return rows;
}

int ensure_workspace(ceres_scene* s, size_t px, bool want_px, bool want_rgb) {
    if ((want_px || want_rgb) && px > s->px_cap) {
        dfree(s->d_pixels); dfree(s->d_rgb8);
        HIP_TRY(hipMalloc(&s->d_pixels, px * 3 * sizeof(float)));
        HIP_TRY(hipMalloc(&s->d_rgb8, px * 3));
        s->px_cap = px;
    }
    return CERES_OK;
}

int retire_buffer(ceres_scene* s, uint32_t* d, size_t words) {
    s->retired.push_back(d);
    s->retired_bytes += (words * sizeof(uint32_t) + kAllocGranule - 1) / kAllocGranule * kAllocGranule;
    if (s->retired_bytes > ceres::kRetiredBytes || s->retired.size() >= ceres::kMaxRetired) {
        HIP_TRY(hipDeviceSynchronize());
        for (auto& r : s->retired) dfree(r);
        s->retired.clear();
        s->retired_bytes = 0;
    }
    return CERES_OK;
}

static void prepare_host_count(ceres_scene::TileOrder& o, const std::vector<uint32_t>& ids, uint32_t bx, uint32_t by, uint32_t tpw);

int upload_tile_order(ceres_scene* s, size_t W, size_t H, const ceres_tiling& t, uint32_t frames, uint32_t tile,
                      std::vector<uint32_t>& order, hipStream_t stream, const ceres_scene::TileOrder** out, bool packed,
                      uint32_t bx, uint32_t by, bool keep_curve, std::vector<uint32_t>* curve = nullptr, uint32_t deal = 0) {
    const size_t n = order.size();
    ceres_scene::TileOrder o;
    if (keep_curve) {
        prepare_host_count(o, curve ? *curve : order, bx, by, tile >> 16);
        keep_curve = o.countable;
    }
    if (packed) {
        const uint32_t per_frame = bx * by;
        auto pack = [&](std::vector<uint32_t>& v) {
            for (auto& id : v) {
                const uint32_t f = id / per_frame, rem = id - f * per_frame, y = rem / bx;
                id = pack_tile(f, y, rem - y * bx);
            }
        };
        pack(order);
        if (keep_curve && curve) pack(*curve);
// ... 134 lines not shown
        if (want_curve) {
            curve.resize(n);
            for (size_t p = 0; p < n; ++p) curve[p] = mk[p].second;
        }
        deal = uint32_t(cw);
        return;
    }
    uint64_t st = 0x9e3779b97f4a7c15ull;
    for (size_t b0 = 0; b0 < n; b0 += dev::kTileShuffleWindow) {
        const size_t len = std::min<size_t>(dev::kTileShuffleWindow, n - b0);
        for (size_t q = len - 1; q > 0; --q) {
            st = st * 6364136223846793005ull + 1442695040888963407ull;
            std::swap(order[b0 + q], order[b0 + size_t((st >> 33) % (q + 1))]);
        }
    }
    if (CERES_XCD_GROUP_TILES && frames > 1) xcd_group_rows(order, bx, per_frame, tpw);
}

int quantize_nodes4(const std::vector<Node4>& in, std::vector<QNode4>& out) {
    out.assign(in.size(), QNode4{});
    for (size_t k = 0; k < in.size(); ++k) {
        const Node4& n = in[k];
        QNode4& q = out[k];
        const float* lo[3] = {n.lo_x, n.lo_y, n.lo_z};
        const float* hi[3] = {n.hi_x, n.hi_y, n.hi_z};
        float org[3], scl[3];
        uint32_t ql[3] = {0, 0, 0}, qh[3] = {0, 0, 0};
        for (int a = 0; a < 3; ++a) {
            float mn = INFINITY, mx = -INFINITY;
            for (int c = 0; c < 4; ++c)
                if (n.child[c] != kNode4Empty) { mn = std::min(mn, lo[a][c]); mx = std::max(mx, hi[a][c]); }
            if (mn > mx) { mn = 0.f; mx = 0.f; }
            if (!std::isfinite(mn) || !std::isfinite(mx))
                return set_error(CERES_EUNSUPPORTED, "CERES_MODE_QBVH4: non-finite BVH bounds");
            const double ext = double(mx) - double(mn);
            int e = ext > 0 ? int(std::ceil(std::log2(ext / 250.0))) : -126;
            e = std::max(e, -126);
            float sc = std::ldexp(1.0f, e);
            org[a] = mn;
            for (int c = 0; c < 4; ++c) {
                uint32_t bl = 255, bh = 0;
                if (n.child[c] != kNode4Empty) {
                    double fl = std::floor((double(lo[a][c]) - double(mn)) / double(sc));
                    double fh = std::ceil((double(hi[a][c]) - double(mn)) / double(sc));
                    int il = int(std::max(0.0, std::min(255.0, fl))), ih = int(std::max(0.0, std::min(255.0, fh)));
                    while (il > 0 && std::fma(float(il), sc, mn) > lo[a][c]) --il;
                    while (ih < 255 && std::fma(float(ih), sc, mn) < hi[a][c]) ++ih;
                    if (std::fma(float(il), sc, mn) > lo[a][c] || std::fma(float(ih), sc, mn) < hi[a][c])
                        return set_error(CERES_EUNSUPPORTED, "CERES_MODE_QBVH4: bound not representable");
                    bl = uint32_t(il); bh = uint32_t(ih);
                }
                ql[a] |= bl << (8 * c);
                qh[a] |= bh << (8 * c);
            }
            scl[a] = sc;
        }
        q.ox = org[0]; q.oy = org[1]; q.oz = org[2];
        q.sx = scl[0]; q.sy = scl[1]; q.sz = scl[2];
        q.qlx = ql[0]; q.qhx = qh[0]; q.qly = ql[1]; q.qhy = qh[1]; q.qlz = ql[2]; q.qhz = qh[2];
        for (int c = 0; c < 4; ++c) q.child[c] = n.child[c];
    }
    return CERES_OK;
}

int build_qnodes4(ceres_scene* s) {
    if (!s->n_nodes4 || !s->d_nodes4) return CERES_OK;
    std::vector<Node4> n4(s->n_nodes4);
    HIP_TRY(hipMemcpy(n4.data(), s->d_nodes4, n4.size() * sizeof(Node4), hipMemcpyDeviceToHost));
    std::vector<QNode4> q;
    if (int rc = quantize_nodes4(n4, q)) return rc;
    HIP_TRY(hipMalloc(&s->d_qnodes4, q.size() * sizeof(QNode4)));
    HIP_TRY(hipMemcpy(s->d_qnodes4, q.data(), q.size() * sizeof(QNode4), hipMemcpyHostToDevice));
    return CERES_OK;
}

void set_root_box(ceres_scene* s, const float root[6], const SiblingPair& p0) {
    for (int k = 0; k < 6; ++k) s->root_box[k] = root[k];
    auto inside = [&](const float* c) {
        return c[0] >= root[0] && c[1] <= root[1] && c[2] >= root[2] && c[3] <= root[3] && c[4] >= root[4] && c[5] <= root[5];
    };
    s->root_box_ok = (!s->root_leaf_count && inside(p0.lb) && inside(p0.rb)) ? 1u : 0u;
}

static CullRect cull_rect(const FrameCam& c, const float root[6], uint32_t W, uint32_t H) {
    const CullRect keep{0u, 0xffffu, 0u, 0xffffu};
    if (W > 0xffffu || H > 0xffffu) return keep;
    double e[3], iu[3], iv[3], d[3];
    for (int k = 0; k < 3; ++k) { e[k] = c.eye[k]; iu[k] = c.iu[k]; iv[k] = c.iv[k]; d[k] = c.dir[k]; }
    double sc = 0;
    for (int k = 0; k < 3; ++k) sc = std::max(sc, std::fabs(e[k]));
    for (int k = 0; k < 6; ++k) sc = std::max(sc, std::fabs(double(root[k])));
    const double pad = 1e-4 * sc;
    auto cr = [](const double* a, const double* b, double* o) {
        o[0] = a[1] * b[2] - a[2] * b[1]; o[1] = a[2] * b[0] - a[0] * b[2]; o[2] = a[0] * b[1] - a[1] * b[0]; };
    double c0[3], c1[3], c2[3];
    cr(iv, d, c0); cr(d, iu, c1); cr(iu, iv, c2);
    const double det = iu[0] * c0[0] + iu[1] * c0[1] + iu[2] * c0[2];
    double u0 = HUGE_VAL, u1 = -HUGE_VAL, v0 = HUGE_VAL, v1 = -HUGE_VAL;
    for (int k = 0; k < 8; ++k) {
        const double X[3] = {(k & 1) ? root[1] + pad : root[0] - pad, (k & 2) ? root[3] + pad : root[2] - pad,
                             (k & 4) ? root[5] + pad : root[4] - pad};
        const double r[3] = {X[0] - e[0], X[1] - e[1], X[2] - e[2]};
        const double pw = r[0] * c0[0] + r[1] * c0[1] + r[2] * c0[2], qw = r[0] * c1[0] + r[1] * c1[1] + r[2] * c1[2];
        const double ww = r[0] * c2[0] + r[1] * c2[1] + r[2] * c2[2];
        if (!(ww / det > 0.01 * std::sqrt(r[0] * r[0] + r[1] * r[1] + r[2] * r[2]))) return keep;
        u0 = std::min(u0, pw / ww); u1 = std::max(u1, pw / ww); v0 = std::min(v0, qw / ww); v1 = std::max(v1, qw / ww);
    }
    const double m = 2e-3 * (1 + std::max(std::max(std::fabs(u0), std::fabs(u1)), std::max(std::fabs(v0), std::fabs(v1))));
    auto lo = [](double x, uint32_t n) { return x <= 0 ? 0u : x >= n ? n : uint32_t(std::floor(x)); };
    const double a0 = (u0 - m + 1) * W / 2 - 0.5 - 1, a1 = (u1 + m + 1) * W / 2 - 0.5 + 1;
    const double b0 = (v0 - m + 1) * H / 2 - 0.5 - 1, b1 = (v1 + m + 1) * H / 2 - 0.5 + 1;
    if (!(a0 == a0 && a1 == a1 && b0 == b0 && b1 == b1)) return keep;
    if (a1 < 0 || b1 < 0) return CullRect{1u, 0u, 1u, 0u};
    return CullRect{uint16_t(lo(a0, W)), uint16_t(std::min<double>(std::ceil(a1), 0xffff)),
                    uint16_t(lo(b0, H)), uint16_t(std::min<double>(std::ceil(b1), 0xffff))};
}

static bool launch_culls_a_tile(const KParams& P) {
    const uint32_t tiles_x = (P.W + 7u) / 8u;
    for (uint32_t f = 0; f < P.frames; ++f) {
        const CullRect& r = P.cull_rect[f];
        const bool all_cols = dev::cull_cols_hit(r, P.W, 0) && dev::cull_cols_hit(r, P.W, tiles_x - 1);
        for (uint32_t lr0 = 0; lr0 < P.local_rows; lr0 += 8) {
            bool exists = false, hit = false;
            for (uint32_t lr = lr0; lr < lr0 + 8 && lr < P.local_rows; ++lr) {
                const uint32_t j = P.world == 1 ? lr
                                   : P.bands    ? ((P.rank + f) % P.world) * P.row_block + lr
                                                : ((lr / P.row_block) * P.world + P.rank) * P.row_block + lr % P.row_block;
                if (P.bands && P.world > 1 && j >= P.H) continue;
                exists = true;
                hit = hit || (j >= r.j0 && j <= r.j1);
            }
            if (exists && !(hit && all_cols)) return true;
        }
    }
    return false;
}

static void prepare_host_count(ceres_scene::TileOrder& o, const std::vector<uint32_t>& ids, uint32_t bx, uint32_t by, uint32_t tpw) {
    const size_t n = ids.size(), pf = size_t(bx) * by;
    o.shapes.clear(); o.h_curve.clear(); o.countable = false;
    bool same = tpw <= 4 && pf % tpw == 0;
    for (size_t p = 0; same && p < n; ++p) same = ids[p % pf] < pf && ids[p] == ids[p % pf] + (p / pf) * pf;
    std::vector<ceres_scene::TileOrder::SubsetBoxes> shapes;
    const size_t stride = size_t(bx) + 1;
    for (size_t g = 0; same && g < pf / tpw; ++g)
        for (uint32_t mask = 1; same && mask < (1u << tpw); ++mask) {
            uint32_t x0 = ~0u, x1 = 0, y0 = ~0u, y1 = 0;
            for (uint32_t i = 0; i < tpw; ++i)
                if (mask >> i & 1u) {
                    const uint32_t id = ids[g * tpw + i], y = id / bx, x = id - y * bx;
                    x0 = std::min(x0, x); x1 = std::max(x1, x); y0 = std::min(y0, y); y1 = std::max(y1, y);
                }
            auto it = std::find_if(shapes.begin(), shapes.end(), [&](const auto& b) { return b.w == x1 - x0 && b.h == y1 - y0; });
            if (it == shapes.end()) {
                if (shapes.size() == ceres::kCountShapes) { same = false; break; }
                shapes.emplace_back();
                it = shapes.end() - 1;
                it->w = x1 - x0; it->h = y1 - y0;
                it->sum.assign((size_t(by) + 1) * stride, 0);
            }
            it->sum[(size_t(y0) + 1) * stride + x0 + 1] += (__builtin_popcount(mask) & 1) ? 1 : -1;
        }
    if (same) {
        for (auto& b : shapes)
            for (size_t y = 1; y <= by; ++y)
                for (size_t x = 1; x <= bx; ++x)
                    b.sum[y * stride + x] += b.sum[(y - 1) * stride + x] + b.sum[y * stride + x - 1] - b.sum[(y - 1) * stride + x - 1];
        o.shapes = std::move(shapes);
        o.countable = true;
    } else if (n <= ceres::kCountWalkTiles) {
        o.h_curve = ids;
        o.countable = true;
    }
}

static uint32_t count_kept_tiles(const KParams& P, const ceres_scene::TileOrder& o, uint32_t tpw) {
    const uint32_t tiles_x = P.tiles_x, tile_rows = P.row_blocks_per_frame, per_frame = tiles_x * tile_rows;
    std::vector<uint32_t> c0(P.frames, 1u), c1(P.frames, 0u), r0(P.frames, 1u), r1(P.frames, 0u);
    for (uint32_t f = 0; f < P.frames; ++f) {
        const CullRect& r = P.cull_rect[f];
        bool any = false;
        for (uint32_t bx = 0; bx < tiles_x; ++bx)
            if (dev::cull_cols_hit(r, P.W, bx)) { if (!any) c0[f] = bx; c1[f] = bx; any = true; }
        any = false;
        for (uint32_t by = 0; by < tile_rows; ++by) {
            const uint32_t lo = 8u * by, hi = std::min(lo + 7u, P.local_rows - 1u);
            if (std::max<uint32_t>(lo, r.j0) <= std::min<uint32_t>(hi, r.j1)) { if (!any) r0[f] = by; r1[f] = by; any = true; }
        }
    }
    if (!o.shapes.empty()) {
        const size_t stride = size_t(tiles_x) + 1;
        int64_t kept = 0;
        for (uint32_t f = 0; f < P.frames; ++f)
            for (const auto& b : o.shapes) {
                if (c0[f] + b.w > c1[f] || r0[f] + b.h > r1[f]) continue;
                const size_t xa = c0[f], xb = size_t(c1[f]) - b.w + 1, ya = r0[f], yb = size_t(r1[f]) - b.h + 1;
                kept += int64_t(b.sum[yb * stride + xb]) - b.sum[ya * stride + xb] - b.sum[yb * stride + xa] + b.sum[ya * stride + xa];
            }
// ... 117 lines not shown
        std::memcpy(c.eye, basis12 + 12 * f, 12); std::memcpy(c.dir, basis12 + 12 * f + 3, 12);
        std::memcpy(c.iu, basis12 + 12 * f + 6, 12); std::memcpy(c.iv, basis12 + 12 * f + 9, 12);
        std::memcpy(c.sun, sun + 3 * f, 12);
    }
    P.frames = frames;
    P.W = uint32_t(W); P.H = uint32_t(H);
    P.row_block = t.row_block; P.rank = t.rank; P.world = t.world; P.local_rows = uint32_t(rows);
    P.bands = t.bands;
    P.band_magic = t.bands ? uint32_t(((uint64_t(1) << 32) + t.world - 1) / t.world) : 0u;
    P.row_blocks_per_frame = by;
    P.stack_entries = s->stack_entries;
    P.shadow_stack_entries = s->shadow_stack_entries;
    P.packets = (s->n_pairs * sizeof(SiblingPair) + s->n_nodes4 * sizeof(Node4) + s->n_tri * sizeof(Tri48)) <
                kDramSceneBytes ? 1u : 0u;
    P.root_leaf_count = s->root_leaf_count; P.root_leaf_first = s->root_leaf_first;
    for (int k = 0; k < 6; ++k) P.root_box[k] = s->root_box[k];
    P.root_box_ok = CERES_ROOT_TEST ? s->root_box_ok : 0u;
    P.cull = (CERES_CULL && P.root_box_ok && !(s->flags & CERES_SCENE_STATS) && !d_rec_prim && W <= 0xffffu && H <= 0xffffu) ? 1u : 0u;
    uint32_t fill_tasks = 0;
    if (P.cull) {
        for (uint32_t f = 0; f < frames; ++f) P.cull_rect[f] = cull_rect(P.cam[f], P.root_box, P.W, P.H);
        if (rows && launch_culls_a_tile(P)) fill_tasks = frames * uint32_t((rows + 7) / 8);
        else P.cull = 0u;
    }
    P.pairs = s->d_pairs; P.nodes4 = s->d_nodes4; P.tris = s->d_tris; P.orig = s->d_orig; P.norms = s->d_norms;
    P.qnodes4 = s->d_qnodes4;
    P.pixels = d_pixels; P.rgb8 = d_rgb8; P.shards = s->d_shards;
    P.rec_prim = d_rec_prim; P.rec_tuv = d_rec_tuv; P.rec_shadow = d_rec_shadow;

    const bool stats = (s->flags & CERES_SCENE_STATS) != 0;
    const bool full = mode == CERES_MODE_FULL;
    hipEvent_t e0 = nullptr, e1 = nullptr;
    if (s->timing && rows) {
        while (s->ev_pool.size() < 2) { hipEvent_t e; HIP_TRY(hipEventCreate(&e)); s->ev_pool.push_back(e); }
        e0 = s->ev_pool.back(); s->ev_pool.pop_back();
        e1 = s->ev_pool.back(); s->ev_pool.pop_back();
        s->ev_used.push_back(e0); s->ev_used.push_back(e1);
    }
    constexpr uint32_t ftile = 8;
    const uint32_t fbx = uint32_t((W + ftile - 1) / ftile), fby = uint32_t((rows + ftile - 1) / ftile);
    const ceres_scene::TileOrder* tile_order = nullptr;
    const bool packed = frames <= (1u << (32 - kTileXBits - kTileYBits)) &&
                        fbx <= (1u << kTileXBits) && fby <= (1u << kTileYBits);
    const uint32_t tpw = (!stats && (frames > 1 || t.bands)) ? batch_tiles_per_wave(size_t(W) * rows, stack_width(s->n_pairs, s->n_nodes4), qbvh)
                                                : 1u;
    if (full && rows)
        if (int rc = ensure_tile_order(s, W, H, t, rows, frames, fbx, fby, ftile, stream, &tile_order, packed, tpw)) return rc;
    const bool need_clean = d_counters || !full;
    if (first && need_clean && s->shards_dirty) HIP_TRY(hipMemsetAsync(s->d_shards, 0, sizeof(Shard) * kShards, stream));
    s->shards_dirty = true;
    if (rows) {
        if (e0) HIP_TRY(hipEventRecord(e0, stream));
        if (full) {
            const int stw = stack_width(s->n_pairs, s->n_nodes4);
            const bool st16 = stw == 2;
            const bool steal = frames == 1 && !t.bands;
            P.steal_first = steal && !stats && ((s->flags & CERES_SCENE_FIRST_ORDER) ||
                                                lds_limits_waves(std::max(s->stack_entries + 1, s->shadow_stack_entries), stw))
                                ? 1u : 0u;
            P.shadow_stack_entries = (!steal || P.steal_first) ? s->shadow_stack_first : s->shadow_stack_entries;
            P.lds_entries = uint32_t(std::max(s->stack_entries + 1, P.shadow_stack_entries));
            const size_t flds = size_t(P.lds_entries) * dev::kFusedB * stw;
            if (int rc = check_fused_lds(s, P, stw, flds)) return rc;
            if (!stats)
                if (const char* g = std::getenv("CERES_DEBUG_GUARD_SLOT")) {
                    const long k = std::strtol(g, nullptr, 10);
                    if (k > 0 && uint32_t(k) < P.stack_entries) P.stack_entries = uint32_t(k);
                }
            P.tile_order = tile_order->d;
            P.tile_packed = packed ? 1u : 0u;
            P.tiles_x = fbx;
            P.row_blocks_per_frame = fby;
            uint32_t n_tiles = fbx * fby * frames;
            bool compacted = false;
            if (CERES_COMPACT && P.cull && fill_tasks && tile_order->d_curve && tpw > 1 && P.packets) {
                const uint32_t kept = count_kept_tiles(P, *tile_order, tpw);
                if (kept < n_tiles) {
                    const uint32_t groups = (n_tiles + tpw - 1) / tpw, nb = (groups + dev::kCompactBlock - 1) / dev::kCompactBlock;
                    ceres::CompactArgs A{};
                    A.tpw = tpw; A.deal = tile_order->deal; A.want_tiles = kept;
                    A.off_result = (groups * tpw + 8u + 3u) / 4u * 4u;
                    A.off_counts = A.off_result + 4u;
                    A.off_rows = A.off_counts + nb;
                    ceres_scene::CompactBuf* cb = nullptr;
                    if (int rc = compact_buffer(s, stream, size_t(A.off_rows) + size_t(frames) * fby, &cb)) return rc;
                    A.buf = cb->d;
                    KParams Q = P;
                    Q.tile_order = tile_order->d_curve;
                    Q.n_tiles = n_tiles;
                    hipLaunchKernelGGL(dev::ceres_cull_rows, dim3((frames * fby + 3u) / 4u), dim3(256), 0, stream, Q, A);
                    hipLaunchKernelGGL(dev::ceres_order_count, dim3(nb), dim3(256), 0, stream, Q, A);
                    hipLaunchKernelGGL(dev::ceres_order_compact, dim3(nb), dim3(256), 0, stream, Q, A);
                    HIP_TRY(hipGetLastError());
                    cb->src = tile_order->d_curve; cb->n = n_tiles; cb->host_tiles = kept; cb->tpw = tpw;
                    cb->deal = A.deal; cb->off_result = A.off_result;
                    P.tile_order = cb->d;
                    n_tiles = kept;
                    compacted = true;
                }
            }
            if (!stats && frames > 1) { s->last_fused_stream = stream; s->last_fused_compacted = compacted; }
            P.n_tiles = n_tiles;
            const uint32_t tile_groups = (n_tiles + tpw - 1) / tpw;
            dim3 fgrid(tile_groups + fill_tasks), fblock(dev::kFusedB);
            if (CERES_FILL_SPREAD > (steal ? 1 : 0) && fill_tasks) {
                const uint64_t nto = (tile_groups + 7) / 8, nfo = (fill_tasks + 7) / 8, stride = (nto + nfo) / nfo;
                if (stride >= 2 && (nto + nfo) * stride < (uint64_t(1) << 32)) {
                    fgrid.x = uint32_t((nto + nfo) * 8);
                    P.fill_stride = uint32_t(stride);
                    P.fill_magic = uint32_t(((uint64_t(1) << 32) + stride - 1) / stride);
                }
            }
            if (stats) {
                const size_t waves = size_t(fbx) * fby * frames;
                if (s->wave_log_waves < waves) {
                    dfree(s->d_wave_log);
                    HIP_TRY(hipMalloc(&s->d_wave_log, waves * 64));
                    s->wave_log_waves = waves;
                }
                HIP_TRY(hipMemsetAsync(s->d_wave_log, 0, waves * 64, stream));
                P.wave_log = s->d_wave_log;
                s->last_grid_waves = waves;
            }
            constexpr int w32 = CERES_FUSED_MINW32;
            auto fused = [&](auto rt, auto st, auto gt) {
                constexpr bool R = decltype(rt)::value, T = decltype(st)::value, G = decltype(gt)::value;
                constexpr int w16 = T ? CERES_FUSED_MINW16_SOLO : CERES_FUSED_MINW16;
                if constexpr (!R) {
                    if (qbvh) {
                        if (st16) hipLaunchKernelGGL((dev::ceres_fused<false, uint16_t*, w16, false, T, true, G>), fgrid, fblock, flds, stream, P);
                        else if (stw == 3) hipLaunchKernelGGL((dev::ceres_fused<false, dev::Stk24, w32, false, T, true, G>), fgrid, fblock, flds, stream, P);
                        else hipLaunchKernelGGL((dev::ceres_fused<false, uint32_t*, w32, false, T, true, G>), fgrid, fblock, flds, stream, P);
                        return;
                    }
                }
                if (stats && st16) hipLaunchKernelGGL((dev::ceres_fused<true, uint16_t*, 1, R, T, false, G>), fgrid, fblock, flds, stream, P);
                else if (stats && stw == 3) hipLaunchKernelGGL((dev::ceres_fused<true, dev::Stk24, w32, R, T, false, G>), fgrid, fblock, flds, stream, P);
                else if (stats) hipLaunchKernelGGL((dev::ceres_fused<true, uint32_t*, w32, R, T, false, G>), fgrid, fblock, flds, stream, P);
                else if (st16) {
                    if constexpr (!T) {
                        if (tpw == 2) { hipLaunchKernelGGL((dev::ceres_fused<false, uint16_t*, w16, R, T, false, G, 2>), fgrid, fblock, flds, stream, P); return; }
                    }
                    constexpr int w16b = T ? CERES_FUSED_MINW16_SOLO : CERES_FUSED_MINW16_TPW4;
                    hipLaunchKernelGGL((dev::ceres_fused<false, uint16_t*, w16b, R, T, false, G>), fgrid, fblock, flds, stream, P);
                }
                else if (stw == 3) hipLaunchKernelGGL((dev::ceres_fused<false, dev::Stk24, w32, R, T, false, G>), fgrid, fblock, flds, stream, P);
                else hipLaunchKernelGGL((dev::ceres_fused<false, uint32_t*, w32, R, T, false, G>), fgrid, fblock, flds, stream, P);
            };
            auto fused_g = [&](auto rt, auto st) {
                if (gfma) fused(rt, st, std::true_type{});
                else fused(rt, st, std::false_type{});
            };
            auto fused_s = [&](auto rt) {
                if (steal) fused_g(rt, std::true_type{});
                else fused_g(rt, std::false_type{});
            };
            auto fused_bands = [&](auto gt) {
                constexpr bool G = decltype(gt)::value;
                if (st16) {
                    if (tpw == 2) hipLaunchKernelGGL((dev::ceres_fused<false, uint16_t*, CERES_FUSED_MINW16, false, false, false, G, 2, true>), fgrid, fblock, flds, stream, P);
                    else hipLaunchKernelGGL((dev::ceres_fused<false, uint16_t*, CERES_FUSED_MINW16_TPW4, false, false, false, G, 0, true>), fgrid, fblock, flds, stream, P);
                } else if (stw == 3) hipLaunchKernelGGL((dev::ceres_fused<false, dev::Stk24, w32, false, false, false, G, 0, true>), fgrid, fblock, flds, stream, P);
                else hipLaunchKernelGGL((dev::ceres_fused<false, uint32_t*, w32, false, false, false, G, 0, true>), fgrid, fblock, flds, stream, P);
            };
            if (t.bands) {
                if (gfma) fused_bands(std::true_type{});
                else fused_bands(std::false_type{});
            } else if (robust) fused_s(std::true_type{});
            else fused_s(std::false_type{});
        } else {
            const size_t lds = size_t(s->stack_entries + 1) * dev::kBlock * 4;
            if (lds > s->max_lds_per_block)
                return set_error(CERES_EINVAL, "render: primary-only traversal stack needs %zu B of LDS per workgroup (%zu available)",
                                 lds, s->max_lds_per_block);
            uint32_t fill_y = (((fill_tasks + dev::kBlock / 64 - 1) / (dev::kBlock / 64)) + bx - 1) / bx;
            if (size_t(by) * frames + fill_y > 65535u) { P.cull = 0u; fill_y = 0; }
            const dim3 grid(bx, by * frames + fill_y), block(dev::kBlock);
            auto primary = [&](auto rt, auto gt) {
                constexpr bool R = decltype(rt)::value, G = decltype(gt)::value;
                if (stats) hipLaunchKernelGGL((dev::ceres_primary<true, R, G>), grid, block, lds, stream, P);
                else hipLaunchKernelGGL((dev::ceres_primary<false, R, G>), grid, block, lds, stream, P);
            };
            auto primary_g = [&](auto rt) {
                if (gfma) primary(rt, std::true_type{});
                else primary(rt, std::false_type{});
            };
            if (robust) primary_g(std::true_type{});
            else primary_g(std::false_type{});
        }
        HIP_TRY(hipGetLastError());
        if (e1) HIP_TRY(hipEventRecord(e1, stream));
    }
    if (d_counters && last) {
        hipLaunchKernelGGL(dev::ceres_finalize, dim3(1), dim3(64), 0, stream, s->d_shards,
                           batch_primary, d_counters);
        HIP_TRY(hipGetLastError());
        s->shards_dirty = false;
    }
    return CERES_OK;
}

int launch(ceres_scene* s, uint32_t frames, const float* basis12, const float* sun, int mode, size_t W, size_t H,
           const ceres_tiling* tiling, float* d_pixels, uint8_t* d_rgb8, uint64_t* d_counters, hipStream_t stream,
           int32_t* d_rec_prim = nullptr, float* d_rec_tuv = nullptr, int8_t* d_rec_shadow = nullptr) {
    if (frames == 0 || frames > uint32_t(kMaxFrames))
        return set_error(CERES_EINVAL, "render: %u frames per batch (1..%d)", frames, kMaxFrames);
    if (!basis12 || !sun) return set_error(CERES_EINVAL, "render: null argument");
    ceres_tiling t{uint32_t(H), 0, 1};
    if (tiling) t = *tiling;
    if (t.world == 0 || t.rank >= t.world || t.row_block == 0) return set_error(CERES_EINVAL, "render: bad tiling");
    uint64_t primary = uint64_t(frames) * W * local_rows_of(H, t);
    if (t.bands && t.world > 1) {
        primary = 0;
        for (uint32_t f = 0; f < frames; ++f) {
            const size_t b = (t.rank + f) % t.world, top = b * size_t(t.row_block);
            primary += uint64_t(W) * (top < H ? std::min<size_t>(t.row_block, H - top) : 0);
        }
    }
    if (frames <= uint32_t(kFramesPerLaunch))
        return launch_chunk(s, frames, basis12, sun, mode, W, H, tiling, d_pixels, d_rgb8, d_counters, stream, d_rec_prim,
                            d_rec_tuv, d_rec_shadow, true, true, primary);
    const size_t fp = W * local_rows_of(H, t);
    const uint32_t n_launch = (frames + kFramesPerLaunch - 1) / kFramesPerLaunch;
    for (uint32_t c = 0, f0 = 0; c < n_launch; ++c) {
        const uint32_t n = frames / n_launch + (c < frames % n_launch ? 1u : 0u);
        const size_t o = size_t(f0) * fp;
        ceres_tiling tc = t;
        if (t.bands) tc.rank = (t.rank + f0) % t.world;
        if (int rc = launch_chunk(s, n, basis12 + 12 * size_t(f0), sun + 3 * size_t(f0), mode, W, H, &tc,
                                  d_pixels ? d_pixels + 3 * o : nullptr, d_rgb8 ? d_rgb8 + 3 * o : nullptr, d_counters,
                                  stream, d_rec_prim ? d_rec_prim + o : nullptr, d_rec_tuv ? d_rec_tuv + 3 * o : nullptr,
                                  d_rec_shadow ? d_rec_shadow + o : nullptr, f0 == 0, f0 + n >= frames, primary))
            return rc;
        f0 += n;
    }
    return CERES_OK;
}

void fill_stats(ceres_stats* st, const uint64_t c[8], double ms) {
    if (!st) return;
    st->rays = c[0]; st->hits = c[1]; st->primary_rays = c[2]; st->shadow_rays = c[3];
    st->node_pairs = c[4]; st->tri_tests = c[5]; st->ms = ms;
}

}

namespace ceres {
int scene_after_refit(ceres_scene* s, const float root[6], const SiblingPair& p0) {
    set_root_box(s, root, p0);
    dfree(s->d_qnodes4);
    return CERES_OK;
}
int scene_adopt_layout(ceres_scene* s, DeviceLayout& L, hipStream_t st) {
    SiblingPair p0{};
    if (!L.root_leaf_count) {
        HIP_TRY(hipMemcpyAsync(&p0, L.pairs, sizeof p0, hipMemcpyDeviceToHost, st));
        HIP_TRY(hipStreamSynchronize(st));
    }
    s->d_pairs = L.pairs; s->d_nodes4 = L.nodes4; s->d_tris = L.tris; s->d_orig = L.orig;
    s->d_src4 = L.src4;
    s->n_pairs = L.n_pairs; s->n_nodes4 = L.n_nodes4;
    s->depth = L.depth; s->root_leaf_count = L.root_leaf_count; s->root_leaf_first = L.root_leaf_first;
    s->stack_entries = std::max<uint32_t>(1, L.depth);
    s->shadow_stack_entries = std::max<uint32_t>(1, L.stack4);
    s->shadow_stack_first = s->shadow_stack_entries;
    if (!L.root_leaf_count) {
        set_root_box(s, L.root_box, p0);
    } else {
        for (int k = 0; k < 6; ++k) s->root_box[k] = 0.f;
        s->root_box_ok = 0;
    }
    L = DeviceLayout{};
    return CERES_OK;
}
int frame_tile_order(ceres_scene* s, size_t W, size_t H, uint32_t tile, hipStream_t stream, const uint32_t** out) {
    const ceres_tiling t{uint32_t(H), 0, 1};
    const ceres_scene::TileOrder* o = nullptr;
    if (int rc = ensure_tile_order(s, W, H, t, H, 1, uint32_t((W + tile - 1) / tile), uint32_t((H + tile - 1) / tile), tile,
                                   stream, &o, false, 1u)) return rc;
    *out = o->d;
    return CERES_OK;
}
}

extern "C" {

const char* ceres_last_error(void) { return error_buffer(); }
extern const char ceres_src_sha[];
const char* ceres_version(void) {
    static const std::string v = std::string("ceres-mi355x 0.5 (gfx950) src ") + ceres_src_sha;
    return v.c_str();
}
int ceres_device_count(void) {
    int n = 0;
    if (hipGetDeviceCount(&n) != hipSuccess) return set_error(CERES_EHIP, "hipGetDeviceCount failed");
    return n;
}
const char* ceres_kernel_names(void) {
    return "ceres_fused,ceres_primary,ceres_finalize,ceres_assemble,ceres_cull_rows,ceres_order_count,ceres_order_compact,ceres_trace_rays_k,ceres_trace_rays64_k,ceres_shade_rays_k,ceres_shade_rays64_k";
}

size_t ceres_tiling_local_rows(size_t height, const ceres_tiling* t) {
    if (!t) return height;
    if (t->world == 0 || t->row_block == 0 || t->rank >= t->world) return 0;
    return local_rows_of(height, *t);
}

ceres_scene* ceres_scene_create(const float* tri48, size_t n_tri, const float* norm36, const void* nodes32,
                                size_t n_nodes, const uint64_t* prim64, int device, uint32_t flags) {
    if (!tri48 || !norm36 || !nodes32 || !prim64 || n_tri == 0 || n_nodes == 0) {
        set_error(CERES_EINVAL, "ceres_scene_create: empty scene or null argument");
        return nullptr;
    }
    if (n_tri > 0xffffffffull || n_nodes > 0xffffffffull) { set_error(CERES_EUNSUPPORTED, "scene too large"); return nullptr; }
    std::vector<SiblingPair> pairs;
    std::vector<Tri48> leaf_tris;
    std::vector<uint32_t> orig;
    uint32_t depth = 0, rlc = 0, rlf = 0;
    if (relayout_bvh(static_cast<const RefNode*>(nodes32), n_nodes, prim64, n_tri, reinterpret_cast<const Tri48*>(tri48),
                     pairs, leaf_tris, orig, depth, rlc, rlf))
        return nullptr;
    std::vector<Node4> nodes4;
    std::vector<uint32_t> src4;
    uint32_t stack4 = 0, not_collapsed = 0;
    if (!rlc && build_shadow_bvh4(pairs, nodes4, stack4, not_collapsed, &src4)) return nullptr;

    uint32_t stack4_first = stack4;
    if (!rlc && ((flags & CERES_SCENE_FIRST_ORDER) ||
                 lds_limits_waves(std::max(depth + 1, stack4), stack_width(pairs.size(), nodes4.size()))) &&
        order_shadow_bvh4(nodes4, stack4_first, &src4))
        return nullptr;
    if (nodes4.empty()) nodes4.emplace_back();
    src4.resize(nodes4.size() * 4, kNode4NoSource);
    auto* s = new (std::nothrow) ceres_scene;
    if (!s) { set_error(CERES_ENOMEM, "out of host memory"); return nullptr; }
    s->n_nodes4 = nodes4.size();
    s->shadow_stack_entries = std::max<uint32_t>(1, stack4);
    s->shadow_stack_first = std::max<uint32_t>(1, std::min(stack4, stack4_first));
    s->device = device; s->flags = flags; s->n_tri = n_tri; s->n_pairs = pairs.size();
    s->depth = depth; s->root_leaf_count = rlc; s->root_leaf_first = rlf;
    s->stack_entries = std::max<uint32_t>(1, depth);
    set_root_box(s, static_cast<const RefNode*>(nodes32)[0].bounds, pairs[0]);
    auto fail = [&]() -> ceres_scene* { scene_release(s); delete s; return nullptr; };
    int ndev = 0;
    if (hipGetDeviceCount(&ndev) != hipSuccess || ndev == 0) { set_error(CERES_EHIP, "no HIP device available"); return fail(); }
    if (device < 0 || device >= ndev) { set_error(CERES_EINVAL, "device %d out of range (%d devices)", device, ndev); return fail(); }
    auto body = [&]() -> int {
        HIP_TRY(hipSetDevice(device));
        hipDeviceProp_t prop;
        HIP_TRY(hipGetDeviceProperties(&prop, device));
        if (std::strncmp(prop.gcnArchName, "gfx950", 6) != 0)
            return set_error(CERES_EHIP, "device %d is %s, this build targets gfx950 only", device, prop.gcnArchName);
        s->num_cus = prop.multiProcessorCount;
        s->max_lds_per_block = prop.sharedMemPerBlock;
        HIP_TRY(hipStreamCreateWithFlags(&s->stream, hipStreamNonBlocking));
        HIP_TRY(hipMalloc(&s->d_pairs, pairs.size() * sizeof(SiblingPair)));
        HIP_TRY(hipMalloc(&s->d_nodes4, nodes4.size() * sizeof(Node4)));
        HIP_TRY(hipMemcpy(s->d_nodes4, nodes4.data(), nodes4.size() * sizeof(Node4), hipMemcpyHostToDevice));
        HIP_TRY(hipMalloc(&s->d_src4, src4.size() * sizeof(uint32_t)));
        HIP_TRY(hipMemcpy(s->d_src4, src4.data(), src4.size() * sizeof(uint32_t), hipMemcpyHostToDevice));
        HIP_TRY(hipMalloc(&s->d_tris, n_tri * sizeof(Tri48)));
        HIP_TRY(hipMalloc(&s->d_orig, n_tri * sizeof(uint32_t)));
        HIP_TRY(hipMalloc(&s->d_norms, n_tri * 36));
        HIP_TRY(hipMalloc(&s->d_shards, sizeof(Shard) * kShards));
        HIP_TRY(hipMalloc(&s->d_counters, 8 * sizeof(uint64_t)));
        HIP_TRY(hipMemcpy(s->d_pairs, pairs.data(), pairs.size() * sizeof(SiblingPair), hipMemcpyHostToDevice));
        HIP_TRY(hipMemcpy(s->d_tris, leaf_tris.data(), n_tri * sizeof(Tri48), hipMemcpyHostToDevice));
        HIP_TRY(hipMemcpy(s->d_orig, orig.data(), n_tri * sizeof(uint32_t), hipMemcpyHostToDevice));
        HIP_TRY(hipMemcpy(s->d_norms, norm36, n_tri * 36, hipMemcpyHostToDevice));
        return CERES_OK;
    };
    if (body()) return fail();
    return s;
}

ceres_scene* ceres_scene_create_device(const float* d_tri48, size_t n_tri, const float* d_norm36, const uint32_t* d_nodes32,
                                       size_t n_nodes, const uint32_t* d_prim32, int device, uint32_t flags, void* stream) {
    if (!d_tri48 || !d_norm36 || !d_nodes32 || !d_prim32 || n_tri == 0 || n_nodes == 0) {
        set_error(CERES_EINVAL, "ceres_scene_create_device: empty scene or null argument");
        return nullptr;
    }
    if (n_tri > 0xffffffffull || n_nodes > 0xffffffffull) { set_error(CERES_EUNSUPPORTED, "scene too large"); return nullptr; }
    auto* s = new (std::nothrow) ceres_scene;
    if (!s) { set_error(CERES_ENOMEM, "out of host memory"); return nullptr; }
    DeviceLayout L;
    auto fail = [&]() -> ceres_scene* {
        if (L.pairs) (void)hipFree(L.pairs);
        if (L.nodes4) (void)hipFree(L.nodes4);
        if (L.tris) (void)hipFree(L.tris);
        if (L.orig) (void)hipFree(L.orig);
        if (L.src4) (void)hipFree(L.src4);
        scene_release(s); delete s; return nullptr;
    };
    int ndev = 0;
    if (hipGetDeviceCount(&ndev) != hipSuccess || ndev == 0) { set_error(CERES_EHIP, "no HIP device available"); return fail(); }
    if (device < 0 || device >= ndev) { set_error(CERES_EINVAL, "device %d out of range (%d devices)", device, ndev); return fail(); }
    s->device = device; s->flags = flags; s->n_tri = n_tri;
    auto body = [&]() -> int {
        HIP_TRY(hipSetDevice(device));
        hipDeviceProp_t prop;
        HIP_TRY(hipGetDeviceProperties(&prop, device));
        if (std::strncmp(prop.gcnArchName, "gfx950", 6) != 0)
            return set_error(CERES_EHIP, "device %d is %s, this build targets gfx950 only", device, prop.gcnArchName);
        s->num_cus = prop.multiProcessorCount;
        s->max_lds_per_block = prop.sharedMemPerBlock;
        HIP_TRY(hipStreamCreateWithFlags(&s->stream, hipStreamNonBlocking));
        hipStream_t st = stream ? static_cast<hipStream_t>(stream) : s->stream;
        if (int rc = relayout_device(reinterpret_cast<const Tri48*>(d_tri48), uint32_t(n_tri),
                                     reinterpret_cast<const RefNode*>(d_nodes32), uint32_t(n_nodes), d_prim32, st, L))
            return rc;
        if (int rc = scene_adopt_layout(s, L, st)) return rc;
        HIP_TRY(hipMalloc(&s->d_norms, n_tri * 36));
        HIP_TRY(hipMemcpyAsync(s->d_norms, d_norm36, n_tri * 36, hipMemcpyDeviceToDevice, st));
        HIP_TRY(hipMalloc(&s->d_shards, sizeof(Shard) * kShards));
        HIP_TRY(hipMalloc(&s->d_counters, 8 * sizeof(uint64_t)));
        HIP_TRY(hipStreamSynchronize(st));
        return CERES_OK;
    };
    if (body()) return fail();
    return s;
}

void ceres_scene_destroy(ceres_scene* s) {
    if (!s) return;
    scene_release(s);
    delete s;
}

int ceres_scene_info(const ceres_scene* s, uint32_t* depth, uint32_t* stack_entries, size_t* n_pairs, size_t* device_bytes) {
    if (!s) return set_error(CERES_EINVAL, "null scene");
    if (depth) *depth = s->depth;
    if (stack_entries) *stack_entries = s->stack_entries;
    if (n_pairs) *n_pairs = s->n_pairs;
    if (device_bytes)
        *device_bytes = s->n_pairs * sizeof(SiblingPair) + s->n_nodes4 * sizeof(Node4) + s->n_tri * (sizeof(Tri48) + 4 + 36);
    return CERES_OK;
}

int ceres_scene_shadow_stacks(const ceres_scene* s, uint32_t* nearest_first, uint32_t* first_passing) {
    if (!s) return set_error(CERES_EINVAL, "null scene");
    if (nearest_first) *nearest_first = s->shadow_stack_entries;
    if (first_passing) *first_passing = s->shadow_stack_first;
    return CERES_OK;
}

int ceres_render_device(ceres_scene* s, const float basis12[12], const float sun[3], int mode, size_t W, size_t H,
                        const ceres_tiling* tiling, float* d_pixels, uint8_t* d_rgb8, uint64_t* d_counters, void* stream) {
    return launch(s, 1, basis12, sun, mode, W, H, tiling, d_pixels, d_rgb8, d_counters, static_cast<hipStream_t>(stream));
}

int ceres_render_batch_device(ceres_scene* s, uint32_t frames, const float* basis12, const float* sun3, int mode,
                              size_t W, size_t H, const ceres_tiling* tiling, float* d_pixels, uint8_t* d_rgb8,
// ... 514 lines not shown
                (rgb8 && hipMemcpyAsync(rgb8, dq, n_rays * 3, hipMemcpyDeviceToHost, s->stream) != hipSuccess) ||
                (hits16 && hipMemcpyAsync(hits16, dh, n_rays * 16, hipMemcpyDeviceToHost, s->stream) != hipSuccess) ||
                (status && hipMemcpyAsync(status, ds, n_rays, hipMemcpyDeviceToHost, s->stream) != hipSuccess) ||
                hipStreamSynchronize(s->stream) != hipSuccess || hipEventElapsedTime(&ms, e0, e1) != hipSuccess))
        rc = set_error(CERES_EHIP, "ceres_shade_rays: copy back failed");
    cleanup();
    if (rc) return rc;
    fill_stats(stats, c, double(ms));
    if (c[6]) return set_error(CERES_ESTACK, "traversal stack overflow");
    return CERES_OK;
}

int ceres_scene_wave_log(ceres_scene* s, uint64_t* out, size_t max_waves, size_t* n_waves) {
    if (!s || !out || !n_waves) return set_error(CERES_EINVAL, "ceres_scene_wave_log: null argument");
    if (!s->d_wave_log) return set_error(CERES_EINVAL, "wave log needs a CERES_SCENE_STATS scene and a full-mode render");
    HIP_TRY(hipSetDevice(s->device));
    HIP_TRY(hipDeviceSynchronize());
    const size_t n = std::min(max_waves, s->last_grid_waves);
    HIP_TRY(hipMemcpy(out, s->d_wave_log, n * 64, hipMemcpyDeviceToHost));
    *n_waves = n;
    return CERES_OK;
}

int ceres_debug_compact_order(ceres_scene* s, uint32_t info[8], uint32_t* order, uint32_t* source, size_t cap) {
    if (!s || !info) return set_error(CERES_EINVAL, "ceres_debug_compact_order: null argument");
    for (int k = 0; k < 8; ++k) info[k] = 0;
    if (!s->last_fused_compacted) return CERES_OK;
    const ceres_scene::CompactBuf* b = nullptr;
    for (const auto& c : s->compact)
        if (c.stream == s->last_fused_stream) b = &c;
    if (!b || !b->d) return set_error(CERES_EINVAL, "ceres_debug_compact_order: the launch's buffer is gone");
    HIP_TRY(hipSetDevice(s->device));
    HIP_TRY(hipStreamSynchronize(b->stream));
    uint32_t res[2] = {0, 0};
    HIP_TRY(hipMemcpy(res, b->d + b->off_result, sizeof res, hipMemcpyDeviceToHost));
    info[0] = 1; info[1] = b->host_tiles; info[2] = res[1]; info[3] = res[0]; info[4] = b->tpw; info[5] = b->deal; info[6] = b->n;
    const size_t padded = std::min<size_t>((size_t(res[1]) + 7) / 8 * 8, b->off_result);
    if (order) {
        if (cap < padded) return set_error(CERES_EINVAL, "ceres_debug_compact_order: %zu words needed", padded);
        HIP_TRY(hipMemcpy(order, b->d, padded * sizeof(uint32_t), hipMemcpyDeviceToHost));
    }
    if (source) {
        if (cap < b->n) return set_error(CERES_EINVAL, "ceres_debug_compact_order: %u words needed", b->n);
        HIP_TRY(hipMemcpy(source, b->src, size_t(b->n) * sizeof(uint32_t), hipMemcpyDeviceToHost));
    }
    return CERES_OK;
}

int ceres_debug_kept_tiles(size_t W, size_t H, uint32_t frames, uint32_t tpw, const uint16_t* rects, uint32_t info[4],
                           uint32_t* source, size_t cap) {
    if (!rects || !info) return set_error(CERES_EINVAL, "ceres_debug_kept_tiles: null argument");
    if (frames < 2 || frames > uint32_t(kFramesPerLaunch) || W == 0 || H == 0 || W > 0xffffu || H > 0xffffu ||
        (tpw != 2 && tpw != 4 && tpw != 8))
        return set_error(CERES_EINVAL, "ceres_debug_kept_tiles: 2..%d frames of at most 65535 x 65535 pixels, 2, 4 or 8 tiles per wave",
                         kFramesPerLaunch);
    const ceres_tiling t{uint32_t(H), 0, 1};
    const uint32_t bx = uint32_t((W + 7) / 8), by = uint32_t((H + 7) / 8);
    const bool packed = frames <= (1u << (32 - kTileXBits - kTileYBits)) && bx <= (1u << kTileXBits) && by <= (1u << kTileYBits);
    std::vector<uint32_t> order, curve;
    uint32_t deal = 0;
    build_tile_order(0, W, H, t, H, frames, bx, by, 8, tpw, true, order, curve, deal);
    ceres_scene::TileOrder o;
    std::vector<uint32_t>& src = deal ? curve : order;
    o.n = uint32_t(src.size());
    prepare_host_count(o, src, bx, by, tpw);
    if (packed)
        for (auto& id : src) {
            const uint32_t f = id / (bx * by), rem = id - f * (bx * by), y = rem / bx;
            id = pack_tile(f, y, rem - y * bx);
        }
    KParams P{};
    P.frames = frames; P.W = uint32_t(W); P.H = uint32_t(H); P.local_rows = uint32_t(H); P.row_block = uint32_t(H); P.world = 1;
    P.tiles_x = bx; P.row_blocks_per_frame = by; P.tile_packed = packed ? 1u : 0u;
    for (uint32_t f = 0; f < frames; ++f) P.cull_rect[f] = CullRect{rects[4 * f], rects[4 * f + 1], rects[4 * f + 2], rects[4 * f + 3]};
    info[0] = o.countable ? count_kept_tiles(P, o, tpw) : o.n;
    info[1] = o.n; info[2] = deal; info[3] = (packed ? 1u : 0u) | (!o.countable ? 0u : o.shapes.empty() ? 2u : 4u);
    if (source) {
        if (cap < o.n) return set_error(CERES_EINVAL, "ceres_debug_kept_tiles: %u words needed", o.n);
        std::memcpy(source, src.data(), size_t(o.n) * sizeof(uint32_t));
    }
    return CERES_OK;
}

int ceres_fetch_counters(int device, uint64_t out[8], int reset) {
    if (!out) return set_error(CERES_EINVAL, "ceres_fetch_counters: null argument");
#if CERES_COUNTING
    static_assert(dev::kFKinds == 8, "ceres_fetch_counters reports 8 kinds");
    HIP_TRY(hipSetDevice(device));
    HIP_TRY(hipDeviceSynchronize());
    unsigned long long h[dev::kFetchShards][dev::kFKinds];
    HIP_TRY(hipMemcpyFromSymbol(h, HIP_SYMBOL(dev::g_fetch), sizeof h));
    for (int k = 0; k < dev::kFKinds; ++k) {
        out[k] = 0;
        for (int q = 0; q < dev::kFetchShards; ++q) out[k] += h[q][k];
    }
    if (reset) {
        std::memset(h, 0, sizeof h);
        HIP_TRY(hipMemcpyToSymbol(HIP_SYMBOL(dev::g_fetch), h, sizeof h));
    }
    return CERES_OK;
#else
    (void)device; (void)reset;
    std::memset(out, 0, 8 * sizeof(uint64_t));
    return set_error(CERES_EUNSUPPORTED, "ceres_fetch_counters: only the counting build (make count) tallies fetches");
#endif
}

int ceres_scene_set_timing(ceres_scene* s, int enable) {
    if (!s) return set_error(CERES_EINVAL, "null scene");
    s->timing = enable != 0;
    return CERES_OK;
}

int ceres_scene_read_timing(ceres_scene* s, double* kernel_ms, double* shadow_ms, uint64_t* renders) {
    if (!s) return set_error(CERES_EINVAL, "null scene");
    HIP_TRY(hipSetDevice(s->device));
    double p = 0;
    const size_t n = s->ev_used.size() / 2;
    for (size_t k = 0; k < n; ++k) {
        hipEvent_t e0 = s->ev_used[2 * k], e1 = s->ev_used[2 * k + 1];
        HIP_TRY(hipEventSynchronize(e1));
        float a = 0.f;
        HIP_TRY(hipEventElapsedTime(&a, e0, e1));
        p += a;
    }
    for (auto e : s->ev_used) s->ev_pool.push_back(e);
    s->ev_used.clear();
    if (kernel_ms) *kernel_ms = p;
    if (shadow_ms) *shadow_ms = 0.0;
    if (renders) *renders = n;
    return CERES_OK;
}

}
```

ceres-raytracer_amd/csrc/scene_internal.hpp:

```cpp
#pragma once
#include <hip/hip_runtime.h>

#include <cstdint>
#include <utility>
#include <vector>

#include "ceres_types.hpp"

using ceres::SiblingPair; using ceres::SiblingPair64; using ceres::Node4; using ceres::Tri48; using ceres::Tri96;
using ceres::Shard;

struct ceres_scene {
    int device = 0;
    uint32_t flags = 0;
    size_t n_tri = 0, n_pairs = 0;
    uint32_t depth = 0, stack_entries = 1, root_leaf_count = 0, root_leaf_first = 0;
    float root_box[6] = {0, 0, 0, 0, 0, 0};
    uint32_t root_box_ok = 0;
    uint32_t shadow_stack_entries = 1;
    uint32_t shadow_stack_first = 1;
    size_t n_nodes4 = 0;
    SiblingPair* d_pairs = nullptr;
    Node4* d_nodes4 = nullptr;
    ceres::QNode4* d_qnodes4 = nullptr;
    struct TileOrder {
        size_t W = 0, H = 0;
        uint32_t row_block = 0, rank = 0, world = 0, frames = 0, tile = 0, bands = 0;
        bool packed = false;
        uint32_t* d = nullptr;
        size_t cap = 0;
        uint64_t used = 0;
        const uint32_t* d_curve = nullptr;
        uint32_t n = 0, deal = 0;
        struct SubsetBoxes {
            uint32_t w = 0, h = 0;
            std::vector<int32_t> sum;
        };
        std::vector<SubsetBoxes> shapes;
        std::vector<uint32_t> h_curve;
        bool countable = false;
    };
    struct CompactBuf {
        hipStream_t stream = nullptr;
        uint32_t* d = nullptr;
        size_t cap = 0;
        uint64_t used = 0;
        const uint32_t* src = nullptr;
        uint32_t n = 0, host_tiles = 0, tpw = 0, deal = 0, off_result = 0;
    };
    std::vector<CompactBuf> compact;
    hipStream_t last_fused_stream = nullptr;
    bool last_fused_compacted = false;
    std::vector<TileOrder> orders;
    std::vector<uint32_t*> retired;
    size_t retired_bytes = 0;
    uint64_t order_clock = 0;
    Tri48* d_tris = nullptr;
    uint32_t* d_orig = nullptr;
    float* d_norms = nullptr;
    Shard* d_shards = nullptr;
    bool shards_dirty = true;
    uint64_t* d_counters = nullptr;
    float* d_pixels = nullptr;
    uint8_t* d_rgb8 = nullptr;
    size_t px_cap = 0;
    hipStream_t stream = nullptr;
    hipStream_t copy_stream = nullptr;
    uint64_t* d_band_counters = nullptr;
    std::vector<hipEvent_t> band_events;
    uint4* d_lit = nullptr;
    uint32_t* d_lit_count = nullptr;
    size_t lit_cap = 0;
    uint32_t* h_small = nullptr;
    std::vector<uint4> h_lit;
    uint4* h_lit_pinned = nullptr;
    bool lit_zc = false;
    double last_lit_frac = 0.0;
    uint32_t dense_calls = 0;
    hipEvent_t ev_count = nullptr;
    int num_cus = 256;
    size_t max_lds_per_block = 64 * 1024;
    unsigned long long* d_wave_log = nullptr;
    size_t wave_log_waves = 0, last_grid_waves = 0;
    bool timing = false;
    std::vector<hipEvent_t> ev_pool;
    std::vector<hipEvent_t> ev_used;
    bool f64 = false;
    SiblingPair64* d_pairs64 = nullptr;
    Tri96* d_tris64 = nullptr;
    double* d_norms64 = nullptr;
    uint32_t* d_src4 = nullptr;
    uint32_t* d_refit_levels = nullptr;
    std::vector<uint32_t> refit_level_off;
    float* d_refit_root = nullptr;
    void* d_refit_stage = nullptr;
    double* d_cost = nullptr;
    double built_cost = 0.0;
    bool built_cost_known = false;
};

namespace ceres {
void host_fill_zero(float* dst, size_t n);
void host_scatter_lit(float* dst, const uint32_t* lit4, size_t n);
void scene_release(ceres_scene* s);
int scene_after_refit(ceres_scene* s, const float root[6], const SiblingPair& p0);
int scene_adopt_layout(ceres_scene* s, ceres::DeviceLayout& L, hipStream_t stream);
constexpr uint32_t kCostBlocks = 512;
int frame_tile_order(ceres_scene* s, size_t W, size_t H, uint32_t tile, hipStream_t stream, const uint32_t** out);
constexpr size_t kMaxTileOrders = 16;
constexpr size_t kCountWalkTiles = size_t(1) << 16;
constexpr size_t kCountShapes = 32;
constexpr size_t kMaxCompactBufs = 16;
constexpr size_t kDramSceneBytes = size_t(64) << 20;
#ifndef CERES_RETIRED_BYTES
#define CERES_RETIRED_BYTES (64u << 20)
#endif
constexpr size_t kRetiredBytes = CERES_RETIRED_BYTES;
constexpr size_t kMaxRetired = 64;
constexpr size_t kAllocGranule = 4096;
}
```

ceres-raytracer_amd/csrc/scene_refit.hip:

```cpp
#include <hip/hip_runtime.h>

#include <cstdint>
#include <cstring>
#include <vector>

#include "ceres_render.h"
#include "ceres_types.hpp"
#include "host_common.hpp"
#include "scene_internal.hpp"

namespace ceres {
namespace refit {

template <class S> __device__ __forceinline__ S lesser(S a, S b) { return b < a ? b : a; }
template <class S> __device__ __forceinline__ S greater(S a, S b) { return a < b ? b : a; }

template <class S> __device__ __forceinline__ void box_empty(S* b) {
    b[0] = b[2] = b[4] = S(INFINITY);
    b[1] = b[3] = b[5] = -S(INFINITY);
}
template <class S> __device__ __forceinline__ void box_point(S* b, S x, S y, S z) {
    b[0] = lesser(b[0], x); b[1] = greater(b[1], x);
    b[2] = lesser(b[2], y); b[3] = greater(b[3], y);
    b[4] = lesser(b[4], z); b[5] = greater(b[5], z);
// ... 118 lines not shown
    const uint64_t i = uint64_t(begin) + uint64_t(blockIdx.x) * 256u + threadIdx.x;
    if (i >= end) return;
    const uint32_t pair = list[i];
    if (pair >= n_pairs) return;
    const Pair& P = pairs[pair];
    const uint32_t count[2] = {P.lcount, P.rcount}, first[2] = {P.lfirst, P.rfirst};
    for (int side = 0; side < 2; ++side) {
        if (count[side] || first[side] >= n_pairs) continue;
        const uint32_t pos = atomicAdd(&list[n_pairs], 1u);
        if (pos < n_pairs) list[pos] = first[side];
    }
}

template <bool F64>
int ensure_levels(ceres_scene* s, hipStream_t st) {
    using L = Lay<F64>;
    if (!F64 && !s->d_refit_root) RF_TRY(hipMalloc(&s->d_refit_root, 18 * sizeof(float)));
    if (s->root_leaf_count || !s->refit_level_off.empty()) return CERES_OK;
    const uint32_t np = uint32_t(s->n_pairs);
    uint32_t* list = nullptr;
    RF_TRY(hipMalloc(&list, (size_t(np) + 1) * sizeof(uint32_t)));
    auto body = [&](std::vector<uint32_t>& off) -> int {
        const uint32_t zero = 0, one = 1;
        RF_TRY(hipMemcpyAsync(list, &zero, 4, hipMemcpyHostToDevice, st));
        RF_TRY(hipMemcpyAsync(list + np, &one, 4, hipMemcpyHostToDevice, st));
        for (uint32_t begin = 0, end = 1; begin < end;) {
            if (off.size() > 65) return set_error(CERES_EINVAL, "refit: sibling pairs deeper than 64 levels");
            hipLaunchKernelGGL((k_next_level<typename L::Pair>), grid_for(end - begin), dim3(256), 0, st, L::pairs(s), np, list, begin, end);
            RF_TRY(hipGetLastError());
            uint32_t tail = 0;
            RF_TRY(hipMemcpyAsync(&tail, list + np, 4, hipMemcpyDeviceToHost, st));
            RF_TRY(hipStreamSynchronize(st));
            if (tail > np) return set_error(CERES_EINVAL, "refit: sibling pairs do not form a tree");
            off.push_back(end);
            begin = end;
            end = tail;
        }
        return CERES_OK;
    };
    std::vector<uint32_t> off{0};
    if (int rc = body(off)) { (void)hipFree(list); return rc; }
    s->d_refit_levels = list;
    s->refit_level_off = std::move(off);
    return CERES_OK;
}

template <bool F64>
int refit_device(ceres_scene* s, const void* d_tri, size_t n_tri, const void* d_norm, hipStream_t stream, const char* who) {
    using L = Lay<F64>;
    using Pair = typename L::Pair; using Tri = typename L::Tri; using S = typename L::S;
    if (!s || !d_tri) return set_error(CERES_EINVAL, "%s: null argument", who);
    if (s->f64 != F64) return set_error(CERES_EINVAL, "%s: the scene is a %s scene", who, s->f64 ? "double" : "float");
    if (n_tri != s->n_tri) return set_error(CERES_EINVAL, "%s: %zu triangles, the scene has %zu", who, n_tri, s->n_tri);
    if (reinterpret_cast<uintptr_t>(d_tri) & 15u) return set_error(CERES_EINVAL, "%s: triangles not 16-byte aligned", who);
    RF_TRY(hipSetDevice(s->device));
    hipStream_t st = stream;
    if (int rc = ensure_levels<F64>(s, st)) return rc;
    const uint32_t nt = uint32_t(n_tri), np = uint32_t(s->n_pairs);
    hipLaunchKernelGGL((k_regather<L::kTriVec>), grid_for(nt), dim3(256), 0, st, static_cast<const uint4*>(d_tri), s->d_orig, nt,
                       reinterpret_cast<uint4*>(L::tris(s)));
    RF_TRY(hipGetLastError());
    if (d_norm) RF_TRY(hipMemcpyAsync(L::norms(s), d_norm, n_tri * L::kNormBytes, hipMemcpyDeviceToDevice, st));
    if (!s->root_leaf_count) {
        hipLaunchKernelGGL((k_leaf_boxes<Pair, Tri, S>), grid_for(2ull * np), dim3(256), 0, st, L::pairs(s), np, L::tris(s), nt);
        RF_TRY(hipGetLastError());
        const std::vector<uint32_t>& off = s->refit_level_off;
        const int levels = int(off.size()) - 1;
        for (int l = levels - 2; l >= 0; --l) {
            const uint32_t n = off[l + 1] - off[l];
            hipLaunchKernelGGL((k_inner_boxes<Pair, S>), grid_for(2ull * n), dim3(256), 0, st, L::pairs(s), np,
                               s->d_refit_levels + off[l], n);
            RF_TRY(hipGetLastError());
        }
    }
    if constexpr (!F64) {
        if (!s->root_leaf_count && s->d_src4 && s->d_nodes4) {
            hipLaunchKernelGGL(k_nodes4_boxes, grid_for(4ull * s->n_nodes4), dim3(256), 0, st, s->d_nodes4, uint32_t(s->n_nodes4),
                               s->d_src4, s->d_pairs, np);
            RF_TRY(hipGetLastError());
        }
        hipLaunchKernelGGL(k_root_box, dim3(1), dim3(64), 0, st, s->d_pairs, s->d_tris, nt, s->root_leaf_count, s->root_leaf_first,
                           s->d_refit_root);
        RF_TRY(hipGetLastError());
        float h[18];
        RF_TRY(hipMemcpyAsync(h, s->d_refit_root, sizeof h, hipMemcpyDeviceToHost, st));
        RF_TRY(hipStreamSynchronize(st));
        SiblingPair p0{};
        std::memcpy(p0.lb, h + 6, sizeof p0.lb);
        std::memcpy(p0.rb, h + 12, sizeof p0.rb);
        return scene_after_refit(s, h, p0);
    } else {
        RF_TRY(hipStreamSynchronize(st));
        return CERES_OK;
    }
}

template <bool F64>
int refit_host(ceres_scene* s, const void* tri, size_t n_tri, const void* norm, const char* who) {
    using L = Lay<F64>;
    if (!s || !tri) return set_error(CERES_EINVAL, "%s: null argument", who);
    if (s->f64 != F64) return set_error(CERES_EINVAL, "%s: the scene is a %s scene", who, s->f64 ? "double" : "float");
    if (n_tri != s->n_tri) return set_error(CERES_EINVAL, "%s: %zu triangles, the scene has %zu", who, n_tri, s->n_tri);
    RF_TRY(hipSetDevice(s->device));
    const size_t tri_bytes = n_tri * sizeof(typename L::Tri), norm_bytes = n_tri * L::kNormBytes;
    if (!s->d_refit_stage) RF_TRY(hipMalloc(&s->d_refit_stage, tri_bytes + norm_bytes));
    char* stage = static_cast<char*>(s->d_refit_stage);
    RF_TRY(hipMemcpyAsync(stage, tri, tri_bytes, hipMemcpyHostToDevice, s->stream));
    if (norm) RF_TRY(hipMemcpyAsync(stage + tri_bytes, norm, norm_bytes, hipMemcpyHostToDevice, s->stream));
    return refit_device<F64>(s, stage, n_tri, norm ? stage + tri_bytes : nullptr, s->stream, who);
}

}
}

using namespace ceres;

extern "C" {

int ceres_scene_refit(ceres_scene* s, const float* tri48, size_t n_tri, const float* norm36) {
    return refit::refit_host<false>(s, tri48, n_tri, norm36, "ceres_scene_refit");
}
int ceres_scene_refit_device(ceres_scene* s, const float* d_tri48, size_t n_tri, const float* d_norm36, void* stream) {
    return refit::refit_device<false>(s, d_tri48, n_tri, d_norm36, static_cast<hipStream_t>(stream), "ceres_scene_refit_device");
}
int ceres_scene_refit_f64(ceres_scene* s, const double* tri96, size_t n_tri, const double* norm72) {
    return refit::refit_host<true>(s, tri96, n_tri, norm72, "ceres_scene_refit_f64");
}
int ceres_scene_refit_f64_device(ceres_scene* s, const double* d_tri96, size_t n_tri, const double* d_norm72, void* stream) {
    return refit::refit_device<true>(s, d_tri96, n_tri, d_norm72, static_cast<hipStream_t>(stream), "ceres_scene_refit_f64_device");
}

int ceres_scene_read_boxes(ceres_scene* s, void* pair_boxes, size_t* n_pairs, float* node4_boxes, size_t* n_nodes4) {
    if (!s) return set_error(CERES_EINVAL, "ceres_scene_read_boxes: null scene");
    RF_TRY(hipSetDevice(s->device));
    RF_TRY(hipDeviceSynchronize());
    const bool tree = !s->root_leaf_count;
    const size_t np = tree ? s->n_pairs : 0, n4 = tree && !s->f64 ? s->n_nodes4 : 0;
    if (n_pairs) *n_pairs = np;
    if (n_nodes4) *n_nodes4 = n4;
    if (pair_boxes && np) {
        if (s->f64) RF_TRY(hipMemcpy2D(pair_boxes, 96, s->d_pairs64, sizeof(SiblingPair64), 96, np, hipMemcpyDeviceToHost));
        else RF_TRY(hipMemcpy2D(pair_boxes, 48, s->d_pairs, sizeof(SiblingPair), 48, np, hipMemcpyDeviceToHost));
    }
    if (node4_boxes && n4) RF_TRY(hipMemcpy2D(node4_boxes, 96, s->d_nodes4, sizeof(Node4), 96, n4, hipMemcpyDeviceToHost));
    return CERES_OK;
}

}
```

include/ceres_render.h:

```cpp
#ifndef CERES_RENDER_H
#define CERES_RENDER_H

#include <stddef.h>
#include <stdint.h>

#ifdef __cplusplus
extern "C" {
#endif

typedef enum {
    CERES_OK = 0,
    CERES_EINVAL = -1,
    CERES_EIO = -2,
    CERES_ENOMEM = -3,
    CERES_EHIP = -4,
    CERES_ESTACK = -5,
    CERES_EUNSUPPORTED = -6
} ceres_status;

typedef enum {
    CERES_MODE_FULL = 0,
    CERES_MODE_PRIMARY = 1,
    CERES_MODE_ROBUST = 0x10,
    CERES_MODE_QBVH4 = 0x20,
// ... 101 lines not shown
int ceres_scene_refit_f64(ceres_scene* scene, const double* tri96, size_t n_tri, const double* norm72);
int ceres_scene_refit_f64_device(ceres_scene* scene, const double* d_tri96, size_t n_tri, const double* d_norm72,
                                 void* stream);
int ceres_scene_read_boxes(ceres_scene* scene, void* pair_boxes, size_t* n_pairs, float* node4_boxes, size_t* n_nodes4);

typedef struct {
    double cost;
    double built_cost;
    double new_cost;
    int32_t rebuilt;
    int32_t reserved;
} ceres_update_info;
int ceres_scene_sah_cost(ceres_scene* scene, double* cost, void* stream);
int ceres_scene_rebuild_device(ceres_scene* scene, const float* d_tri48, size_t n_tri, const float* d_norm36, int arith,
                               void* stream);
int ceres_scene_rebuild(ceres_scene* scene, const float* tri48, size_t n_tri, const float* norm36, int arith);
int ceres_scene_update_device(ceres_scene* scene, const float* d_tri48, size_t n_tri, const float* d_norm36, int arith,
                              double max_ratio, ceres_update_info* info, void* stream);
int ceres_scene_update(ceres_scene* scene, const float* tri48, size_t n_tri, const float* norm36, int arith,
                       double max_ratio, ceres_update_info* info);


int ceres_render_f32(ceres_scene* scene, const float basis12[12], const float sun[3], int mode,
                     float* pixels, uint8_t* rgb8, size_t width, size_t height, ceres_stats* stats);

int ceres_render_device(ceres_scene* scene, const float basis12[12], const float sun[3], int mode,
                        size_t width, size_t height, const ceres_tiling* tiling,
                        float* d_pixels, uint8_t* d_rgb8, uint64_t* d_counters, void* stream);
int ceres_render_batch_device(ceres_scene* scene, uint32_t frames, const float* basis12,
                              const float* sun3, int mode, size_t width, size_t height,
                              const ceres_tiling* tiling, float* d_pixels, uint8_t* d_rgb8,
                              uint64_t* d_counters, void* stream);
int ceres_assemble_rgb8(const uint8_t* d_gathered, size_t rank_stride_bytes, uint8_t* d_out, uint32_t frames,
                        size_t width, size_t height, uint32_t row_block, uint32_t world, void* stream);
int ceres_device_count(void);
int ceres_render_multi_f32(ceres_scene* const* scenes, uint32_t world, uint32_t row_block,
                           const float basis12[12], const float sun[3], int mode, float* pixels,
                           uint8_t* rgb8, size_t width, size_t height, ceres_stats* stats);
int ceres_assemble_rgb8_packed(const uint8_t* d_gathered, uint8_t* d_out, uint32_t frames, size_t width,
                               size_t height, uint32_t row_block, uint32_t world, void* stream);
int ceres_render_records(ceres_scene* scene, const float basis12[12], const float sun[3], int mode,
                         size_t width, size_t height, int32_t* prim, float* tuv, int8_t* shadow,
                         ceres_stats* stats);
size_t ceres_tiling_local_rows(size_t height, const ceres_tiling* tiling);
int ceres_render_f64(ceres_scene* scene, const double basis12[12], const double sun[3], int mode,
                     double* pixels, uint8_t* rgb8, size_t width, size_t height, ceres_stats* stats);
int ceres_render_records_f64(ceres_scene* scene, const double basis12[12], const double sun[3], int mode,
                             size_t width, size_t height, int32_t* prim, double* tuv, int8_t* shadow,
                             ceres_stats* stats);

int ceres_trace_rays_device(ceres_scene* scene, const void* d_rays32, size_t n_rays, int mode, void* d_hits16,
                            uint8_t* d_occluded, uint64_t* d_counters, void* stream);
int ceres_trace_rays(ceres_scene* scene, const void* rays32, size_t n_rays, int mode, void* hits16, uint8_t* occluded,
                     ceres_stats* stats);

int ceres_trace_rays_f64_device(ceres_scene* scene, const void* d_rays64, size_t n_rays, int mode, void* d_hits32,
                                uint8_t* d_occluded, uint64_t* d_counters, void* stream);
int ceres_trace_rays_f64(ceres_scene* scene, const void* rays64, size_t n_rays, int mode, void* hits32, uint8_t* occluded,
                         ceres_stats* stats);

int ceres_shade_rays_device(ceres_scene* scene, const void* d_rays32, size_t n_rays, const float sun[3], int mode,
                            float* d_pixels, uint8_t* d_rgb8, void* d_hits16, uint8_t* d_status, uint64_t* d_counters,
                            void* stream);
int ceres_shade_rays(ceres_scene* scene, const void* rays32, size_t n_rays, const float sun[3], int mode, float* pixels,
                     uint8_t* rgb8, void* hits16, uint8_t* status, ceres_stats* stats);
int ceres_camera_rays(const float basis12[12], size_t width, size_t height, int arith, void* rays32);

int ceres_shade_rays_f64_device(ceres_scene* scene, const void* d_rays64, size_t n_rays, const double sun[3], int mode,
                                double* d_pixels, uint8_t* d_rgb8, void* d_hits32, uint8_t* d_status, uint64_t* d_counters,
                                void* stream);
int ceres_shade_rays_f64(ceres_scene* scene, const void* rays64, size_t n_rays, const double sun[3], int mode, double* pixels,
                         uint8_t* rgb8, void* hits32, uint8_t* status, ceres_stats* stats);
int ceres_camera_rays_f64(const double basis12[12], size_t width, size_t height, int arith, void* rays64);

int ceres_scene_set_timing(ceres_scene* scene, int enable);
int ceres_scene_read_timing(ceres_scene* scene, double* kernel_ms, double* shadow_ms, uint64_t* renders);

int ceres_scene_wave_log(ceres_scene* scene, uint64_t* out, size_t max_waves, size_t* n_waves);

int ceres_debug_compact_order(ceres_scene* scene, uint32_t info[8], uint32_t* order, uint32_t* source, size_t cap);
int ceres_debug_kept_tiles(size_t width, size_t height, uint32_t frames, uint32_t tiles_per_wave, const uint16_t* rects,
                           uint32_t info[4], uint32_t* source, size_t cap);

int ceres_fetch_counters(int device, uint64_t out[8], int reset);

typedef struct ceres_cpu_scene ceres_cpu_scene;
ceres_cpu_scene* ceres_cpu_scene_create(const float* tri48, size_t n_tri, const float* norm36, const void* nodes32,
                                        size_t n_nodes, const uint64_t* prim64);
void ceres_cpu_scene_destroy(ceres_cpu_scene* scene);
int ceres_render_cpu_f32(const ceres_cpu_scene* scene, const float basis12[12], const float sun[3], int mode,
                         float* pixels, uint8_t* rgb8, size_t width, size_t height, ceres_stats* stats, int threads);
ceres_cpu_scene* ceres_cpu_scene_create_f64(const double* tri96, size_t n_tri, const double* norm72, const void* nodes64,
                                            size_t n_nodes, const uint64_t* prim64);
int ceres_render_cpu_f64(const ceres_cpu_scene* scene, const double basis12[12], const double sun[3], int mode,
                         double* pixels, uint8_t* rgb8, size_t width, size_t height, ceres_stats* stats, int threads);
int ceres_cpu_scene_refit(ceres_cpu_scene* scene, const float* tri48, size_t n_tri, const float* norm36);
int ceres_cpu_scene_refit_f64(ceres_cpu_scene* scene, const double* tri96, size_t n_tri, const double* norm72);
int ceres_cpu_scene_sah_cost(const ceres_cpu_scene* scene, double* cost);
int ceres_cpu_scene_rebuild(ceres_cpu_scene* scene, const float* tri48, size_t n_tri, const float* norm36, int arith);
int ceres_cpu_scene_rebuild_f64(ceres_cpu_scene* scene, const double* tri96, size_t n_tri, const double* norm72, int arith);
int ceres_cpu_scene_update(ceres_cpu_scene* scene, const float* tri48, size_t n_tri, const float* norm36, int arith,
                           double max_ratio, ceres_update_info* info);
int ceres_cpu_scene_update_f64(ceres_cpu_scene* scene, const double* tri96, size_t n_tri, const double* norm72, int arith,
                               double max_ratio, ceres_update_info* info);
int ceres_trace_rays_cpu(const ceres_cpu_scene* scene, const void* rays32, size_t n_rays, int mode, void* hits16,
                         uint8_t* occluded, ceres_stats* stats, int threads);
int ceres_trace_rays_cpu_f64(const ceres_cpu_scene* scene, const void* rays64, size_t n_rays, int mode, void* hits32,
                             uint8_t* occluded, ceres_stats* stats, int threads);

int ceres_shade_rays_cpu(const ceres_cpu_scene* scene, const void* rays32, size_t n_rays, const float sun[3], int mode,
                         float* pixels, uint8_t* rgb8, void* hits16, uint8_t* status, ceres_stats* stats, int threads);
int ceres_shade_rays_cpu_f64(const ceres_cpu_scene* scene, const void* rays64, size_t n_rays, const double sun[3], int mode,
                             double* pixels, uint8_t* rgb8, void* hits32, uint8_t* status, ceres_stats* stats, int threads);

uint64_t ceres_content_hash(const void* p, size_t bytes);

const char* ceres_kernel_names(void);

const char* ceres_last_error(void);
const char* ceres_version(void);

#ifdef __cplusplus
}
#endif

#endif
```

Before: 52720 Mrays/s.

## Start tile traversal at per-tile BVH entry node from projected top-level cut

Builds a 64-node cut of the top BVH levels with pairwise lowest-common-ancestor tables. Per frame, each cut box is projected to a screen rectangle, and each 8x8 tile gets the LCA of the cut nodes overlapping it, so traversal can begin below the root. This aims to skip the upper-level box tests repeated by every ray. It adds per-frame rectangle and entry computation, device storage for the cut, and a refresh after refit, and it risks wrong entry nodes if the conservative projection or the containment checks fail.

```diff
diff --git a/ceres-raytracer_amd/__init__.py b/ceres-raytracer_amd/__init__.py
--- a/ceres-raytracer_amd/__init__.py
+++ b/ceres-raytracer_amd/__init__.py
@@ -37,6 +37,8 @@
     "ceres_render_device", "ceres_render_batch_device", "ceres_render_multi_f32", "ceres_device_count", "ceres_assemble_rgb8_packed", "ceres_render_records", "ceres_tiling_local_rows",
     "ceres_scene_set_timing", "ceres_scene_read_timing", "ceres_scene_wave_log", "ceres_fetch_counters",
     "ceres_debug_compact_order", "ceres_debug_kept_tiles",
+    "ceres_entry_cut_words", "ceres_entry_cut_build", "ceres_entry_relayout", "ceres_entry_rects", "ceres_entry_tiles",
+    "ceres_debug_entry_record", "ceres_debug_entry_nodes",
     "ceres_cpu_scene_create", "ceres_cpu_scene_destroy", "ceres_render_cpu_f32", "ceres_cpu_scene_create_f64",
     "ceres_render_cpu_f64",
     "ceres_orbit_cameras", "ceres_assemble_rgb8",
@@ -190,6 +192,15 @@
         L.ceres_debug_compact_order.argtypes = [_vp, _u32p, _u32p, _u32p, _sz]
         L.ceres_debug_kept_tiles.argtypes = [_sz, _sz, ctypes.c_uint32, ctypes.c_uint32, ctypes.POINTER(ctypes.c_uint16), _u32p,
                                              _u32p, _sz]
+    if hasattr(L, "ceres_entry_cut_build"):
+        _u16p = ctypes.POINTER(ctypes.c_uint16)
+        L.ceres_entry_cut_words.restype = _sz
+        L.ceres_entry_cut_build.argtypes = [_vp, _sz, ctypes.c_uint32, _fp, _u32p]
+        L.ceres_entry_relayout.argtypes = [_fp, _sz, _vp, _sz, _u64p, _vp, ctypes.POINTER(_sz), _u32p, _u32p]
+        L.ceres_entry_rects.argtypes = [_u32p, _fp, _sz, _sz, _u16p]
+        L.ceres_entry_tiles.argtypes = [_u32p, _u16p, _sz, _sz, _u32p]
+        L.ceres_debug_entry_record.argtypes = [_vp, ctypes.c_int]
+        L.ceres_debug_entry_nodes.argtypes = [_vp, _u32p, _u32p, _u16p, _u32p, _sz]
     L.ceres_cpu_scene_create.argtypes = [_fp, _sz, _fp, _vp, _sz, _u64p]
     L.ceres_cpu_scene_create.restype = _vp
     L.ceres_cpu_scene_destroy.argtypes = [_vp]
@@ -813,10 +824,79 @@
         return {"host_tiles": int(info[1]), "device_tiles": int(info[2]), "groups": int(info[3]), "tpw": int(info[4]),
                 "deal": int(info[5]), "order": order[:(int(info[2]) + 7) // 8 * 8], "source": source[:int(info[6])]}
 
+    def entry_record(self, on=True):
+        _check(lib().ceres_debug_entry_record(self._h, 1 if on else 0))
+
+    def entry_nodes(self):
+        info = np.zeros(8, np.uint32)
+        table = np.zeros(cut_words(), np.uint32)
+        _check(lib().ceres_debug_entry_nodes(self._h, _p(info, ctypes.c_uint32), _p(table, ctypes.c_uint32), None, None, 0))
+        out = {"cut": CutTable(table) if info[0] else None, "used": bool(info[1])}
+        if info[1]:
+            rects = np.zeros((int(info[2]), 64, 4), np.uint16)
+            entries = np.zeros(max(int(info[3]), 1), np.uint32)
+            _check(lib().ceres_debug_entry_nodes(self._h, _p(info, ctypes.c_uint32), None, _p(rects, ctypes.c_uint16), None,
+                                                 rects.shape[0] * 64))
+            _check(lib().ceres_debug_entry_nodes(self._h, _p(info, ctypes.c_uint32), None, None, _p(entries, ctypes.c_uint32),
+                                                 len(entries)))
+            out.update(rects=rects, entries=entries[:int(info[3])], W=int(info[4]), H=int(info[5]))
+        return out
+
     def read_timing(self):
         p, q, n = ctypes.c_double(), ctypes.c_double(), ctypes.c_uint64()
         _check(lib().ceres_scene_read_timing(self._h, ctypes.byref(p), ctypes.byref(q), ctypes.byref(n)))
         return p.value, q.value, n.value
+
+
+ENTRY_EMPTY, ENTRY_CULLED = 0xffffffff, 0xfefefefe
+
+
+def cut_words():
+    return int(lib().ceres_entry_cut_words())
+
+
+class CutTable:
+
+    def __init__(self, words):
+        self.words = np.ascontiguousarray(words, np.uint32)
+        w = self.words
+        self.n, self.entry_ok = int(w[0]), int(w[1])
+        self.src, self.child = w[4:4 + self.n], w[68:68 + self.n]
+        self.box = w[132:132 + 384].view(np.float32).reshape(64, 6)[:self.n]
+        self.lca = w[516:516 + 4096].reshape(64, 64)
+        self.depth = w[4868:4868 + 4096].reshape(64, 64)
+
+
+def entry_relayout(mesh, bvh):
+    n, rlc = _sz(0), ctypes.c_uint32(0)
+    args = (_p(mesh.tri, ctypes.c_float), len(mesh), bvh.nodes.ctypes.data_as(_vp), bvh.nodes.shape[0], _p(bvh.prim, ctypes.c_uint64))
+    _check(lib().ceres_entry_relayout(*args, None, ctypes.byref(n), None, ctypes.byref(rlc)))
+    pairs, orig = np.zeros((n.value, 16), np.uint32), np.zeros(len(mesh), np.uint32)
+    _check(lib().ceres_entry_relayout(*args, pairs.ctypes.data_as(_vp), ctypes.byref(n), _p(orig, ctypes.c_uint32), ctypes.byref(rlc)))
+    return pairs, orig, int(rlc.value)
+
+
+def entry_cut(pairs, root_leaf_count, root_box):
+    pairs = np.ascontiguousarray(pairs, np.uint32).reshape(-1, 16)
+    table = np.zeros(cut_words(), np.uint32)
+    rb = np.ascontiguousarray(root_box, np.float32).reshape(6)
+    _check(lib().ceres_entry_cut_build(pairs.ctypes.data_as(_vp), pairs.shape[0], int(root_leaf_count), _p(rb, ctypes.c_float),
+                                       _p(table, ctypes.c_uint32)))
+    return CutTable(table)
+
+
+def entry_rects(cut, basis12, W, H):
+    b = np.ascontiguousarray(basis12, np.float32).reshape(12)
+    out = np.zeros((64, 4), np.uint16)
+    _check(lib().ceres_entry_rects(_p(cut.words, ctypes.c_uint32), _p(b, ctypes.c_float), int(W), int(H), _p(out, ctypes.c_uint16)))
+    return out
+
+
+def entry_tiles(cut, rects, W, H):
+    r = np.ascontiguousarray(rects, np.uint16).reshape(64, 4)
+    out = np.zeros(((int(H) + 7) // 8, (int(W) + 7) // 8), np.uint32)
+    _check(lib().ceres_entry_tiles(_p(cut.words, ctypes.c_uint32), _p(r, ctypes.c_uint16), int(W), int(H), _p(out, ctypes.c_uint32)))
+    return out
 
 
 def source_sha16(repo=None):
diff --git a/ceres-raytracer_amd/csrc/ceres_types.hpp b/ceres-raytracer_amd/csrc/ceres_types.hpp
--- a/ceres-raytracer_amd/csrc/ceres_types.hpp
+++ b/ceres-raytracer_amd/csrc/ceres_types.hpp
@@ -149,7 +149,12 @@
     unsigned long long* wave_log;
     uint32_t fill_stride, fill_magic;
     uint32_t n_tiles;
+    uint32_t entry_off;
+    const uint32_t* cut;
 };
+constexpr uint32_t kEntryDebug = 0x80000000u;
+constexpr uint32_t kEntryEmpty = 0xffffffffu;
+constexpr uint32_t kEntryCulled = 0xfefefefeu;
 
 struct CompactArgs {
     uint32_t* buf;
diff --git a/ceres-raytracer_amd/csrc/entry_cut.hpp b/ceres-raytracer_amd/csrc/entry_cut.hpp
--- /dev/null
+++ b/ceres-raytracer_amd/csrc/entry_cut.hpp
@@ -0,0 +1,190 @@
+#pragma once
+#include <cmath>
+#include <cstdint>
+
+#include "ceres_types.hpp"
+
+#if defined(__HIPCC__)
+#define CERES_CUT_HD __host__ __device__
+#else
+#define CERES_CUT_HD
+#endif
+
+namespace ceres {
+
+constexpr uint32_t kCutMax = 64;
+constexpr uint32_t kCutN = 0;
+constexpr uint32_t kCutOk = 1;
+constexpr uint32_t kCutChecks = 2;
+constexpr uint32_t kCutBroken = 3;
+constexpr uint32_t kCutSrc = 4;
+constexpr uint32_t kCutChild = 68;
+constexpr uint32_t kCutBox = 132;
+constexpr uint32_t kCutLca = 516;
+constexpr uint32_t kCutCheckRec = 4612;
+constexpr uint32_t kCutCheckBox = 4740;
+constexpr uint32_t kCutDepth = 4868;
+constexpr uint32_t kCutRootBox = 4868 + 4096;
+constexpr uint32_t kCutWords = kCutRootBox + 6;
+constexpr uint32_t kCutLeaf = 0xffffffffu, kCutRoot = 0xffffffffu;
+
+CERES_CUT_HD inline const float* cut_src_box(const SiblingPair* pairs, uint32_t src) {
+    return (src & 1u) ? pairs[src >> 1].rb : pairs[src >> 1].lb;
+}
+CERES_CUT_HD inline bool cut_inside(const float* c, const float* p) {
+    return c[0] >= p[0] && c[1] <= p[1] && c[2] >= p[2] && c[3] <= p[3] && c[4] >= p[4] && c[5] <= p[5];
+}
+CERES_CUT_HD inline void cut_load_box(const SiblingPair* pairs, uint32_t* T, uint32_t k) {
+    const float* b = cut_src_box(pairs, T[kCutSrc + k]);
+    float* out = reinterpret_cast<float*>(T + kCutBox) + 6 * k;
+    for (int a = 0; a < 6; ++a) out[a] = b[a];
+}
+CERES_CUT_HD inline bool cut_check(const SiblingPair* pairs, const float* root_box, const uint32_t* T, uint32_t k) {
+    const SiblingPair& r = pairs[T[kCutCheckRec + k]];
+    const uint32_t bs = T[kCutCheckBox + k];
+    const float* p = bs == kCutRoot ? root_box : cut_src_box(pairs, bs);
+    return cut_inside(r.lb, p) && cut_inside(r.rb, p);
+}
+CERES_CUT_HD inline void cut_refresh_serial(const SiblingPair* pairs, const float* root_box, uint32_t* T) {
+    for (int a = 0; a < 6; ++a) reinterpret_cast<float*>(T + kCutRootBox)[a] = root_box[a];
+    bool ok = !T[kCutBroken] && T[kCutN] >= 2;
+    for (uint32_t k = 0; k < T[kCutN]; ++k) cut_load_box(pairs, T, k);
+    for (uint32_t k = 0; k < T[kCutChecks]; ++k) ok = cut_check(pairs, root_box, T, k) && ok;
+    T[kCutOk] = ok ? 1u : 0u;
+}
+
+CERES_CUT_HD inline float cut_area(const float* b) {
+    const float dx = b[1] - b[0], dy = b[3] - b[2], dz = b[5] - b[4];
+    return dx * dy + dy * dz + dz * dx;
+}
+
+CERES_CUT_HD inline void cut_build(const SiblingPair* pairs, uint32_t n_pairs, uint32_t root_leaf_count, const float* root_box,
+                               uint32_t* T) {
+    for (uint32_t k = 0; k < kCutWords; ++k) T[k] = 0u;
+    for (uint32_t k = 0; k < kCutMax; ++k) T[kCutChild + k] = kCutLeaf;
+    for (int a = 0; a < 6; ++a) reinterpret_cast<float*>(T + kCutRootBox)[a] = root_box[a];
+    if (root_leaf_count || n_pairs == 0) return;
+    uint64_t path[kCutMax], ipath[kCutMax];
+    uint32_t depth[kCutMax], idepth[kCutMax], irec[kCutMax];
+    uint32_t n = 0, ni = 0, checks = 0;
+    bool broken = false;
+    auto child_of = [&](const SiblingPair& r, int side) {
+        const uint32_t count = side ? r.rcount : r.lcount, first = side ? r.rfirst : r.lfirst;
+        if (count) return kCutLeaf;
+        if (first >= n_pairs || first == 0) { broken = true; return kCutLeaf; }
+        return first;
+    };
+    auto add_check = [&](uint32_t rec, uint32_t box) { T[kCutCheckRec + checks] = rec; T[kCutCheckBox + checks] = box; ++checks; };
+    for (int side = 0; side < 2; ++side) {
+        T[kCutSrc + n] = uint32_t(side); T[kCutChild + n] = child_of(pairs[0], side);
+        path[n] = uint64_t(side); depth[n] = 1;
+        ++n;
+    }
+    add_check(0u, kCutRoot);
+    ipath[ni] = 0; idepth[ni] = 0; irec[ni] = 0; ++ni;
+    while (n < kCutMax) {
+        uint32_t best = kCutMax;
+        float best_area = -1.f;
+        for (uint32_t k = 0; k < n; ++k) {
+            if (T[kCutChild + k] == kCutLeaf) continue;
+            const float a = cut_area(cut_src_box(pairs, T[kCutSrc + k]));
+            if (a > best_area) { best_area = a; best = k; }
+        }
+        if (best == kCutMax) break;
+        const uint32_t rec = T[kCutChild + best], src = T[kCutSrc + best], d = depth[best];
+        const uint64_t p = path[best];
+        add_check(rec, src);
+        ipath[ni] = p; idepth[ni] = d; irec[ni] = rec; ++ni;
+        for (uint32_t k = n; k > best + 1; --k) {
+            T[kCutSrc + k] = T[kCutSrc + k - 1]; T[kCutChild + k] = T[kCutChild + k - 1];
+            path[k] = path[k - 1]; depth[k] = depth[k - 1];
+        }
+        ++n;
+        for (int side = 0; side < 2; ++side) {
+            T[kCutSrc + best + side] = rec << 1 | uint32_t(side);
+            T[kCutChild + best + side] = child_of(pairs[rec], side);
+            path[best + side] = p | uint64_t(side) << d;
+            depth[best + side] = d + 1;
+        }
+    }
+    for (uint32_t t = 0; t < ni; ++t) {
+        const uint32_t d = idepth[t];
+        const uint64_t mask = (uint64_t(1) << d) - 1u;
+        for (uint32_t i = 0; i < n; ++i) {
+            if ((path[i] & mask) != ipath[t] || (path[i] >> d & 1u)) continue;
+            for (uint32_t j = i + 1; j < n; ++j) {
+                if ((path[j] & mask) != ipath[t] || !(path[j] >> d & 1u)) continue;
+                T[kCutLca + i * kCutMax + j] = T[kCutLca + j * kCutMax + i] = irec[t];
+                T[kCutDepth + i * kCutMax + j] = T[kCutDepth + j * kCutMax + i] = d;
+            }
+        }
+    }
+    for (uint32_t k = 0; k < n; ++k) {
+        const bool inner = T[kCutChild + k] != kCutLeaf;
+        T[kCutLca + k * kCutMax + k] = inner ? T[kCutChild + k] : T[kCutSrc + k] >> 1;
+        T[kCutDepth + k * kCutMax + k] = inner ? depth[k] : depth[k] - 1u;
+        if (inner) add_check(T[kCutChild + k], T[kCutSrc + k]);
+    }
+    T[kCutN] = n; T[kCutChecks] = checks; T[kCutBroken] = broken ? 1u : 0u;
+    cut_refresh_serial(pairs, root_box, T);
+}
+
+template <class V> CERES_CUT_HD inline V cut_max(V a, V b) { return a < b ? b : a; }
+template <class V> CERES_CUT_HD inline V cut_min(V a, V b) { return b < a ? b : a; }
+CERES_CUT_HD inline void cut_cross(const double* a, const double* b, double* o) {
+    o[0] = a[1] * b[2] - a[2] * b[1]; o[1] = a[2] * b[0] - a[0] * b[2]; o[2] = a[0] * b[1] - a[1] * b[0];
+}
+CERES_CUT_HD inline uint32_t cut_clamp_floor(double x, uint32_t n) { return x <= 0 ? 0u : x >= n ? n : uint32_t(floor(x)); }
+
+CERES_CUT_HD inline CullRect box_rect(const FrameCam& c, const float box[6], uint32_t W, uint32_t H) {
+    const CullRect keep{0u, 0xffffu, 0u, 0xffffu};
+    if (W > 0xffffu || H > 0xffffu) return keep;
+    double e[3], iu[3], iv[3], d[3];
+    for (int k = 0; k < 3; ++k) { e[k] = c.eye[k]; iu[k] = c.iu[k]; iv[k] = c.iv[k]; d[k] = c.dir[k]; }
+    double sc = 0;
+    for (int k = 0; k < 3; ++k) sc = cut_max(sc, fabs(e[k]));
+    for (int k = 0; k < 6; ++k) sc = cut_max(sc, fabs(double(box[k])));
+    const double pad = 1e-4 * sc;
+    double c0[3], c1[3], c2[3];
+    cut_cross(iv, d, c0); cut_cross(d, iu, c1); cut_cross(iu, iv, c2);
+    const double det = iu[0] * c0[0] + iu[1] * c0[1] + iu[2] * c0[2];
+    double u0 = HUGE_VAL, u1 = -HUGE_VAL, v0 = HUGE_VAL, v1 = -HUGE_VAL;
+    for (int k = 0; k < 8; ++k) {
+        const double X[3] = {(k & 1) ? box[1] + pad : box[0] - pad, (k & 2) ? box[3] + pad : box[2] - pad,
+                             (k & 4) ? box[5] + pad : box[4] - pad};
+        const double r[3] = {X[0] - e[0], X[1] - e[1], X[2] - e[2]};
+        const double pw = r[0] * c0[0] + r[1] * c0[1] + r[2] * c0[2], qw = r[0] * c1[0] + r[1] * c1[1] + r[2] * c1[2];
+        const double ww = r[0] * c2[0] + r[1] * c2[1] + r[2] * c2[2];
+        if (!(ww / det > 0.01 * sqrt(r[0] * r[0] + r[1] * r[1] + r[2] * r[2]))) return keep;
+        u0 = cut_min(u0, pw / ww); u1 = cut_max(u1, pw / ww); v0 = cut_min(v0, qw / ww); v1 = cut_max(v1, qw / ww);
+    }
+    const double m = 2e-3 * (1 + cut_max(cut_max(fabs(u0), fabs(u1)), cut_max(fabs(v0), fabs(v1))));
+    const double a0 = (u0 - m + 1) * W / 2 - 0.5 - 1, a1 = (u1 + m + 1) * W / 2 - 0.5 + 1;
+    const double b0 = (v0 - m + 1) * H / 2 - 0.5 - 1, b1 = (v1 + m + 1) * H / 2 - 0.5 + 1;
+    if (!(a0 == a0 && a1 == a1 && b0 == b0 && b1 == b1)) return keep;
+    if (a1 < 0 || b1 < 0) return CullRect{1u, 0u, 1u, 0u};
+    return CullRect{uint16_t(cut_clamp_floor(a0, W)), uint16_t(cut_min<double>(ceil(a1), 0xffff)),
+                    uint16_t(cut_clamp_floor(b0, H)), uint16_t(cut_min<double>(ceil(b1), 0xffff))};
+}
+
+CERES_CUT_HD inline bool cut_is_keep(const CullRect& r) { return r.i0 == 0u && r.i1 == 0xffffu && r.j0 == 0u && r.j1 == 0xffffu; }
+CERES_CUT_HD inline CullRect cut_lane_rect(const uint32_t* T, const FrameCam& c, uint32_t W, uint32_t H, uint32_t lane) {
+    const uint32_t n = T[kCutN];
+    if (n < 2u || !T[kCutOk]) return CullRect{0u, 0xffffu, 0u, 0xffffu};
+    if (cut_is_keep(box_rect(c, reinterpret_cast<const float*>(T + kCutRootBox), W, H))) return CullRect{0u, 0xffffu, 0u, 0xffffu};
+    if (lane >= n) return CullRect{1u, 0u, 1u, 0u};
+    return box_rect(c, reinterpret_cast<const float*>(T + kCutBox) + 6 * lane, W, H);
+}
+CERES_CUT_HD inline bool cut_rect_hits_tile(const CullRect& r, uint32_t W, uint32_t rows, uint32_t bx, uint32_t by) {
+    const uint32_t a = 8u * bx, b = a + 7u < W - 1u ? a + 7u : W - 1u;
+    const uint32_t p = 8u * by, q = p + 7u < rows - 1u ? p + 7u : rows - 1u;
+    return cut_max<uint32_t>(a, r.i0) <= cut_min<uint32_t>(b, r.i1) && cut_max<uint32_t>(p, r.j0) <= cut_min<uint32_t>(q, r.j1);
+}
+
+CERES_CUT_HD inline bool cut_words_hit_tile(uint32_t x, uint32_t y, uint32_t W, uint32_t rows, uint32_t bx, uint32_t by) {
+    const uint32_t a = 8u * bx, b = a + 7u < W - 1u ? a + 7u : W - 1u;
+    const uint32_t p = 8u * by, q = p + 7u < rows - 1u ? p + 7u : rows - 1u;
+    return cut_max(a, x & 0xffffu) <= cut_min(b, x >> 16) && cut_max(p, y & 0xffffu) <= cut_min(q, y >> 16);
+}
+
+}
diff --git a/ceres-raytracer_amd/csrc/render_hip.hip b/ceres-raytracer_amd/csrc/render_hip.hip
--- a/ceres-raytracer_amd/csrc/render_hip.hip
+++ b/ceres-raytracer_amd/csrc/render_hip.hip
@@ -14,6 +14,7 @@
 
 #include "ceres_render.h"
 #include "ceres_types.hpp"
+#include "entry_cut.hpp"
 #include "host_common.hpp"
 #include "pow24.hpp"
 
@@ -85,6 +86,9 @@
 #ifndef CERES_COMPACT
 #define CERES_COMPACT 1
 #endif
+#ifndef CERES_ENTRY_NODES
+#define CERES_ENTRY_NODES 1
+#endif
 #ifndef CERES_TRI_SELECT
 #define CERES_TRI_SELECT 1
 #endif
@@ -381,7 +385,8 @@
 template <bool kAnyHit, bool kStats, int kS = kBlock, typename StkT = uint32_t*, bool kRobust = false, int kOct = -1,
           bool kG = false, class RK = CamRay, class PT>
 __device__ __forceinline__ bool trace(const PT& P, F3 o, F3 d, StkT stk, Hit& best,
-                                      uint32_t& n_pairs, uint32_t& n_tests, bool& overflow, RK rk = RK{}) {
+                                      uint32_t& n_pairs, uint32_t& n_tests, bool& overflow, RK rk = RK{},
+                                      uint32_t first = 0) {
     const float tmin = rk.tmin();
     float tmax = rk.tmax();
     bool have = false;
@@ -403,7 +408,7 @@
     if constexpr (!kRobust && kOct == -1 && (CERES_OCTANT_SLAB & 1)) {
         bool r = false;
         if (with_uniform_octant(sl, [&](auto k) {
-                r = trace<kAnyHit, kStats, kS, StkT, kRobust, decltype(k)::value, kG, RK>(P, o, d, stk, best, n_pairs, n_tests, overflow, rk);
+                r = trace<kAnyHit, kStats, kS, StkT, kRobust, decltype(k)::value, kG, RK>(P, o, d, stk, best, n_pairs, n_tests, overflow, rk, first);
             }))
             return r;
     }
@@ -418,7 +423,7 @@
     }
     uint32_t sp = 0;
     if (CERES_TRI_SELECT && !kAnyHit) best.slot = kNoSlot;
-    const float4* q = reinterpret_cast<const float4*>(P.pairs);
+    const float4* q = reinterpret_cast<const float4*>(P.pairs + first);
     float4 A = q[0], B = q[1], C = q[2];
     uint4 L = reinterpret_cast<const uint4*>(q)[3];
     CERES_COUNT_V(kFBvh2V, 64);
@@ -482,11 +487,11 @@
 
 template <bool kStats, int kS, typename StkT, bool kRobust, int kOct, bool kG>
 __device__ __forceinline__ bool guarded_trace(const KParams& P, F3 o, F3 d, StkT stk, Hit& best, uint32_t& n_pairs,
-                                              uint32_t& n_tests, bool& overflow) {
+                                              uint32_t& n_tests, bool& overflow, uint32_t first = 0) {
     constexpr bool kGuard = !kStats && CERES_TRUST_STACK_BOUND && CERES_STACK_GUARD;
     const uint32_t slot = P.stack_entries * kS;
     if (kGuard) stk[slot] = stack_guard<StkT>();
-    const bool hit = trace<false, kStats, kS, StkT, kRobust, kOct, kG>(P, o, d, stk, best, n_pairs, n_tests, overflow);
+    const bool hit = trace<false, kStats, kS, StkT, kRobust, kOct, kG>(P, o, d, stk, best, n_pairs, n_tests, overflow, CamRay{}, first);
     if (kGuard) overflow |= uint32_t(stk[slot]) != stack_guard<StkT>();
     return hit;
 }
@@ -1188,10 +1193,12 @@
 
 constexpr int kFusedB = 64;
 constexpr size_t kLdsPerCu = 160 * 1024;
-template <bool kStats, typename StkT, int kMinW, bool kRobust, bool kSteal, bool kQ, bool kG, int kTPWo = 0, bool kBands = false>
+template <bool kStats, typename StkT, int kMinW, bool kRobust, bool kSteal, bool kQ, bool kG, int kTPWo = 0, bool kBands = false,
+          bool kEntryDbg = false>
 __global__ __launch_bounds__(kFusedB) __attribute__((amdgpu_waves_per_eu(kMinW))) void ceres_fused(const KParams P) {
     constexpr int kB = kFusedB;
     constexpr bool kPacketsCompiled = !kStats && !kSteal && !kRobust && !kQ && CERES_SHADOW_PACKET && std::is_same<StkT, uint16_t*>::value;
+    constexpr bool kEntry = CERES_ENTRY_NODES && !kStats && !kSteal && !kRobust && !kQ && !kBands && std::is_same<StkT, uint16_t*>::value;
     extern __shared__ __attribute__((aligned(16))) uint32_t lds[];
     __shared__ StealLdsT<kB> L;
     const uint32_t lane = threadIdx.x, tid = lane;
@@ -1306,11 +1313,27 @@
         if (stashed) flush(t_prev);
         continue;
     }
-    if (active) {
+    uint32_t entry = 0;
+    if constexpr (kEntry) {
+        if (P.entry_off) {
+            const uint2 r = reinterpret_cast<const uint2*>(P.tile_order + (P.entry_off & ~kEntryDebug))[f * kCutMax + lane];
+            const uint64_t reach = __ballot(cut_words_hit_tile(r.x, r.y, P.W, P.local_rows, i >> 3, lr >> 3));
+            entry = kEntryEmpty;
+            if (reach) {
+                const uint32_t lo = uint32_t(__builtin_ctzll(reach)), hi = 63u - uint32_t(__builtin_clzll(reach));
+                entry = sload_u32(P.cut + kCutLca + lo * kCutMax + hi);
+            }
+            if constexpr (kEntryDbg)
+                if (lane == 0)
+                    const_cast<uint32_t*>(P.tile_order)[(P.entry_off & ~kEntryDebug) + P.frames * 2u * kCutMax +
+                                                        (f * P.row_blocks_per_frame + (lr >> 3)) * P.tiles_x + (i >> 3)] = entry;
+        }
+    }
+    if (active && !(kEntry && entry == kEntryEmpty)) {
         const F3 view = primary_dir<kG>(P, f, i, global_row<kBands>(P, f, lr));
         constexpr int kOctMode = (!kSteal || (CERES_OCTANT_SLAB & 4)) ? -1 : -2;
         hit = guarded_trace<kStats, kB, StkT, kRobust, kOctMode, kG>(P, f3(P.cam[f].eye), view, stk, h, n_pairs,
-                                                                   n_tests, overflow);
+                                                                   n_tests, overflow, entry);
         if (P.rec_prim) {
             redecode();
             P.rec_prim[px] = hit ? int32_t(P.orig[h.slot]) : -1;
@@ -1392,6 +1415,27 @@
     if (f >= P.frames) return;
     const bool hit = tile_rows_hit(P, f, by * 8u + (lane & 7u));
     if (lane == 0) A.buf[A.off_rows + task] = hit ? 1u : 0u;
+    if (CERES_ENTRY_NODES && P.entry_off && by == 0) {
+        const CullRect r = cut_lane_rect(P.cut, P.cam[f], P.W, P.H, lane);
+        reinterpret_cast<uint2*>(A.buf + (P.entry_off & ~kEntryDebug))[f * kCutMax + lane] =
+            make_uint2(uint32_t(r.i0) | uint32_t(r.i1) << 16, uint32_t(r.j0) | uint32_t(r.j1) << 16);
+    }
+}
+
+struct Box6 { float b[6]; };
+__global__ void ceres_cut_build(const SiblingPair* pairs, uint32_t n_pairs, uint32_t root_leaf_count, Box6 root, uint32_t* T) {
+    if (blockIdx.x || threadIdx.x) return;
+    cut_build(pairs, n_pairs, root_leaf_count, root.b, T);
+}
+__global__ __launch_bounds__(128) void ceres_cut_refresh(const SiblingPair* pairs, const float* root_box, uint32_t* T) {
+    __shared__ uint32_t bad;
+    if (threadIdx.x == 0) bad = 0u;
+    __syncthreads();
+    if (threadIdx.x < T[kCutN]) cut_load_box(pairs, T, threadIdx.x);
+    if (threadIdx.x < 6u) T[kCutRootBox + threadIdx.x] = __float_as_uint(root_box[threadIdx.x]);
+    if (threadIdx.x < T[kCutChecks] && !cut_check(pairs, root_box, T, threadIdx.x)) atomicOr(&bad, 1u);
+    __syncthreads();
+    if (threadIdx.x == 0) T[kCutOk] = (!bad && !T[kCutBroken] && T[kCutN] >= 2u) ? 1u : 0u;
 }
 
 __device__ __forceinline__ bool group_kept(const KParams& P, const CompactArgs& A, uint32_t g) {
@@ -1726,7 +1770,7 @@
     if (!s) return;
     (void)hipSetDevice(s->device);
     dfree(s->d_pairs64); dfree(s->d_tris64); dfree(s->d_norms64);
-    dfree(s->d_src4); dfree(s->d_refit_levels); dfree(s->d_refit_root); dfree(s->d_cost);
+    dfree(s->d_src4); dfree(s->d_refit_levels); dfree(s->d_refit_root); dfree(s->d_cost); dfree(s->d_cut);
     if (s->d_refit_stage) { (void)hipFree(s->d_refit_stage); s->d_refit_stage = nullptr; }
     for (auto& o : s->orders) dfree(o.d);
     for (auto& d : s->retired) dfree(d);
@@ -2027,39 +2071,7 @@
     s->root_box_ok = (!s->root_leaf_count && inside(p0.lb) && inside(p0.rb)) ? 1u : 0u;
 }
 
-static CullRect cull_rect(const FrameCam& c, const float root[6], uint32_t W, uint32_t H) {
-    const CullRect keep{0u, 0xffffu, 0u, 0xffffu};
-    if (W > 0xffffu || H > 0xffffu) return keep;
-    double e[3], iu[3], iv[3], d[3];
-    for (int k = 0; k < 3; ++k) { e[k] = c.eye[k]; iu[k] = c.iu[k]; iv[k] = c.iv[k]; d[k] = c.dir[k]; }
-    double sc = 0;
-    for (int k = 0; k < 3; ++k) sc = std::max(sc, std::fabs(e[k]));
-    for (int k = 0; k < 6; ++k) sc = std::max(sc, std::fabs(double(root[k])));
-    const double pad = 1e-4 * sc;
-    auto cr = [](const double* a, const double* b, double* o) {
-        o[0] = a[1] * b[2] - a[2] * b[1]; o[1] = a[2] * b[0] - a[0] * b[2]; o[2] = a[0] * b[1] - a[1] * b[0]; };
-    double c0[3], c1[3], c2[3];
-    cr(iv, d, c0); cr(d, iu, c1); cr(iu, iv, c2);
-    const double det = iu[0] * c0[0] + iu[1] * c0[1] + iu[2] * c0[2];
-    double u0 = HUGE_VAL, u1 = -HUGE_VAL, v0 = HUGE_VAL, v1 = -HUGE_VAL;
-    for (int k = 0; k < 8; ++k) {
-        const double X[3] = {(k & 1) ? root[1] + pad : root[0] - pad, (k & 2) ? root[3] + pad : root[2] - pad,
-                             (k & 4) ? root[5] + pad : root[4] - pad};
-        const double r[3] = {X[0] - e[0], X[1] - e[1], X[2] - e[2]};
-        const double pw = r[0] * c0[0] + r[1] * c0[1] + r[2] * c0[2], qw = r[0] * c1[0] + r[1] * c1[1] + r[2] * c1[2];
-        const double ww = r[0] * c2[0] + r[1] * c2[1] + r[2] * c2[2];
-        if (!(ww / det > 0.01 * std::sqrt(r[0] * r[0] + r[1] * r[1] + r[2] * r[2]))) return keep;
-        u0 = std::min(u0, pw / ww); u1 = std::max(u1, pw / ww); v0 = std::min(v0, qw / ww); v1 = std::max(v1, qw / ww);
-    }
-    const double m = 2e-3 * (1 + std::max(std::max(std::fabs(u0), std::fabs(u1)), std::max(std::fabs(v0), std::fabs(v1))));
-    auto lo = [](double x, uint32_t n) { return x <= 0 ? 0u : x >= n ? n : uint32_t(std::floor(x)); };
-    const double a0 = (u0 - m + 1) * W / 2 - 0.5 - 1, a1 = (u1 + m + 1) * W / 2 - 0.5 + 1;
-    const double b0 = (v0 - m + 1) * H / 2 - 0.5 - 1, b1 = (v1 + m + 1) * H / 2 - 0.5 + 1;
-    if (!(a0 == a0 && a1 == a1 && b0 == b0 && b1 == b1)) return keep;
-    if (a1 < 0 || b1 < 0) return CullRect{1u, 0u, 1u, 0u};
-    return CullRect{uint16_t(lo(a0, W)), uint16_t(std::min<double>(std::ceil(a1), 0xffff)),
-                    uint16_t(lo(b0, H)), uint16_t(std::min<double>(std::ceil(b1), 0xffff))};
-}
+static CullRect cull_rect(const FrameCam& c, const float root[6], uint32_t W, uint32_t H) { return box_rect(c, root, W, H); }
 
 static bool launch_culls_a_tile(const KParams& P) {
     const uint32_t tiles_x = (P.W + 7u) / 8u;
@@ -2343,8 +2355,18 @@
                     A.off_result = (groups * tpw + 8u + 3u) / 4u * 4u;
                     A.off_counts = A.off_result + 4u;
                     A.off_rows = A.off_counts + nb;
+                    const bool entry = CERES_ENTRY_NODES && s->d_cut && !robust && !qbvh && st16;
+                    const uint32_t off_entry = (A.off_rows + frames * fby + 1u) / 2u * 2u;
+                    const size_t entry_words = !entry ? 0 : size_t(frames) * 2u * kCutMax + (s->entry_debug ? size_t(n_tiles) : 0);
                     ceres_scene::CompactBuf* cb = nullptr;
-                    if (int rc = compact_buffer(s, stream, size_t(A.off_rows) + size_t(frames) * fby, &cb)) return rc;
+                    if (int rc = compact_buffer(s, stream, size_t(off_entry) + entry_words, &cb)) return rc;
+                    if (entry) {
+                        P.entry_off = off_entry | (s->entry_debug ? kEntryDebug : 0u);
+                        P.cut = s->d_cut;
+                    }
+                    cb->entry_off = P.entry_off; cb->frames = frames; cb->W = P.W; cb->H = P.H;
+                    if (P.entry_off & kEntryDebug)
+                        HIP_TRY(hipMemsetAsync(cb->d + off_entry + size_t(frames) * 2u * kCutMax, 0xfe, size_t(n_tiles) * sizeof(uint32_t), stream));
                     A.buf = cb->d;
                     KParams Q = P;
                     Q.tile_order = tile_order->d_curve;
@@ -2399,6 +2421,14 @@
                 else if (stats && stw == 3) hipLaunchKernelGGL((dev::ceres_fused<true, dev::Stk24, w32, R, T, false, G>), fgrid, fblock, flds, stream, P);
                 else if (stats) hipLaunchKernelGGL((dev::ceres_fused<true, uint32_t*, w32, R, T, false, G>), fgrid, fblock, flds, stream, P);
                 else if (st16) {
+                    if constexpr (!T && !R) {
+                        if (P.entry_off & kEntryDebug) {
+                            constexpr int w16d = CERES_FUSED_MINW16_TPW4;
+                            if (tpw == 2) hipLaunchKernelGGL((dev::ceres_fused<false, uint16_t*, w16, false, false, false, G, 2, false, true>), fgrid, fblock, flds, stream, P);
+                            else hipLaunchKernelGGL((dev::ceres_fused<false, uint16_t*, w16d, false, false, false, G, 0, false, true>), fgrid, fblock, flds, stream, P);
+                            return;
+                        }
+                    }
                     if constexpr (!T) {
                         if (tpw == 2) { hipLaunchKernelGGL((dev::ceres_fused<false, uint16_t*, w16, R, T, false, G, 2>), fgrid, fblock, flds, stream, P); return; }
                     }
@@ -2514,9 +2544,15 @@
 }
 int scene_adopt_layout(ceres_scene* s, DeviceLayout& L, hipStream_t st) {
     SiblingPair p0{};
+    uint32_t* cut = nullptr;
+    if (CERES_ENTRY_NODES) HIP_TRY(hipMalloc(&cut, kCutWords * sizeof(uint32_t)));
     if (!L.root_leaf_count) {
-        HIP_TRY(hipMemcpyAsync(&p0, L.pairs, sizeof p0, hipMemcpyDeviceToHost, st));
-        HIP_TRY(hipStreamSynchronize(st));
+        hipError_t e = hipMemcpyAsync(&p0, L.pairs, sizeof p0, hipMemcpyDeviceToHost, st);
+        if (e == hipSuccess) e = hipStreamSynchronize(st);
+        if (e != hipSuccess) {
+            dfree(cut);
+            return set_error(CERES_EHIP, "scene_adopt_layout: %s", hipGetErrorString(e));
+        }
     }
     s->d_pairs = L.pairs; s->d_nodes4 = L.nodes4; s->d_tris = L.tris; s->d_orig = L.orig;
     s->d_src4 = L.src4;
@@ -2532,6 +2568,21 @@
         s->root_box_ok = 0;
     }
     L = DeviceLayout{};
+    if (cut) {
+        if (s->d_cut) (void)retire_buffer(s, s->d_cut, kCutWords);
+        s->d_cut = cut;
+        dev::Box6 root;
+        for (int k = 0; k < 6; ++k) root.b[k] = s->root_box[k];
+        hipLaunchKernelGGL(dev::ceres_cut_build, dim3(1), dim3(64), 0, st, s->d_pairs, uint32_t(s->n_pairs), s->root_leaf_count, root,
+                           s->d_cut);
+        HIP_TRY(hipGetLastError());
+    }
+    return CERES_OK;
+}
+int scene_refresh_cut(ceres_scene* s, const float* d_root_box, hipStream_t st) {
+    if (!s->d_cut || s->root_leaf_count) return CERES_OK;
+    hipLaunchKernelGGL(dev::ceres_cut_refresh, dim3(1), dim3(128), 0, st, s->d_pairs, d_root_box, s->d_cut);
+    HIP_TRY(hipGetLastError());
     return CERES_OK;
 }
 int frame_tile_order(ceres_scene* s, size_t W, size_t H, uint32_t tile, hipStream_t stream, const uint32_t** out) {
@@ -2629,6 +2680,12 @@
         HIP_TRY(hipMemcpy(s->d_tris, leaf_tris.data(), n_tri * sizeof(Tri48), hipMemcpyHostToDevice));
         HIP_TRY(hipMemcpy(s->d_orig, orig.data(), n_tri * sizeof(uint32_t), hipMemcpyHostToDevice));
         HIP_TRY(hipMemcpy(s->d_norms, norm36, n_tri * 36, hipMemcpyHostToDevice));
+        if (CERES_ENTRY_NODES) {
+            std::vector<uint32_t> cut(kCutWords);
+            cut_build(pairs.data(), uint32_t(pairs.size()), rlc, s->root_box, cut.data());
+            HIP_TRY(hipMalloc(&s->d_cut, kCutWords * sizeof(uint32_t)));
+            HIP_TRY(hipMemcpy(s->d_cut, cut.data(), kCutWords * sizeof(uint32_t), hipMemcpyHostToDevice));
+        }
         return CERES_OK;
     };
     if (body()) return fail();
@@ -3309,6 +3366,107 @@
     return CERES_OK;
 }
 
+size_t ceres_entry_cut_words(void) { return kCutWords; }
+
+int ceres_entry_cut_build(const void* pairs64, size_t n_pairs, uint32_t root_leaf_count, const float root_box[6], uint32_t* table) {
+    if (!pairs64 || !root_box || !table || n_pairs == 0 || n_pairs > 0xffffffffull)
+        return set_error(CERES_EINVAL, "ceres_entry_cut_build: null argument or no pair");
+    cut_build(static_cast<const SiblingPair*>(pairs64), uint32_t(n_pairs), root_leaf_count, root_box, table);
+    return CERES_OK;
+}
+
+int ceres_entry_relayout(const float* tri48, size_t n_tri, const void* nodes32, size_t n_nodes, const uint64_t* prim64,
+                         void* pairs64, size_t* n_pairs, uint32_t* orig, uint32_t* root_leaf_count) {
+    if (!tri48 || !nodes32 || !prim64 || !n_pairs || !root_leaf_count || n_tri == 0 || n_nodes == 0)
+        return set_error(CERES_EINVAL, "ceres_entry_relayout: null argument");
+    std::vector<SiblingPair> pairs;
+    std::vector<Tri48> leaf_tris;
+    std::vector<uint32_t> o;
+    uint32_t depth = 0, rlc = 0, rlf = 0;
+    if (int rc = relayout_bvh(static_cast<const RefNode*>(nodes32), n_nodes, prim64, n_tri, reinterpret_cast<const Tri48*>(tri48),
+                              pairs, leaf_tris, o, depth, rlc, rlf))
+        return rc;
+    if (pairs64) {
+        if (*n_pairs < pairs.size()) return set_error(CERES_EINVAL, "ceres_entry_relayout: %zu pairs needed", pairs.size());
+        std::memcpy(pairs64, pairs.data(), pairs.size() * sizeof(SiblingPair));
+    }
+    if (orig) std::memcpy(orig, o.data(), n_tri * sizeof(uint32_t));
+    *n_pairs = pairs.size();
+    *root_leaf_count = rlc;
+    return CERES_OK;
+}
+
+int ceres_entry_rects(const uint32_t* table, const float basis12[12], size_t W, size_t H, uint16_t* rects) {
+    if (!table || !basis12 || !rects || W == 0 || H == 0 || W > 0xffffffffull || H > 0xffffffffull)
+        return set_error(CERES_EINVAL, "ceres_entry_rects: null argument or empty frame");
+    FrameCam c{};
+    std::memcpy(c.eye, basis12, 12); std::memcpy(c.dir, basis12 + 3, 12);
+    std::memcpy(c.iu, basis12 + 6, 12); std::memcpy(c.iv, basis12 + 9, 12);
+    for (uint32_t k = 0; k < kCutMax; ++k) {
+        const CullRect r = cut_lane_rect(table, c, uint32_t(W), uint32_t(H), k);
+        rects[4 * k] = r.i0; rects[4 * k + 1] = r.i1; rects[4 * k + 2] = r.j0; rects[4 * k + 3] = r.j1;
+    }
+    return CERES_OK;
+}
+
+int ceres_entry_tiles(const uint32_t* table, const uint16_t* rects, size_t W, size_t H, uint32_t* entries) {
+    if (!table || !rects || !entries || W == 0 || H == 0 || W > 0xffffu || H > 0xffffu)
+        return set_error(CERES_EINVAL, "ceres_entry_tiles: null argument or bad frame size");
+    const uint32_t bx = uint32_t((W + 7) / 8), by = uint32_t((H + 7) / 8);
+    for (uint32_t y = 0; y < by; ++y)
+        for (uint32_t x = 0; x < bx; ++x) {
+            uint32_t lo = kCutMax, hi = 0;
+            for (uint32_t k = 0; k < kCutMax; ++k) {
+                const CullRect r{rects[4 * k], rects[4 * k + 1], rects[4 * k + 2], rects[4 * k + 3]};
+                if (!cut_rect_hits_tile(r, uint32_t(W), uint32_t(H), x, y)) continue;
+                if (lo == kCutMax) lo = k;
+                hi = k;
+            }
+            entries[size_t(y) * bx + x] = lo == kCutMax ? kEntryEmpty : table[kCutLca + lo * kCutMax + hi];
+        }
+    return CERES_OK;
+}
+
+int ceres_debug_entry_record(ceres_scene* s, int enable) {
+    if (!s) return set_error(CERES_EINVAL, "ceres_debug_entry_record: null scene");
+    s->entry_debug = enable != 0;
+    return CERES_OK;
+}
+
+int ceres_debug_entry_nodes(ceres_scene* s, uint32_t info[8], uint32_t* table, uint16_t* rects, uint32_t* entries, size_t cap) {
+    if (!s || !info) return set_error(CERES_EINVAL, "ceres_debug_entry_nodes: null argument");
+    for (int k = 0; k < 8; ++k) info[k] = 0;
+    HIP_TRY(hipSetDevice(s->device));
+    HIP_TRY(hipDeviceSynchronize());
+    info[0] = s->d_cut ? kCutWords : 0u;
+    if (table && s->d_cut) HIP_TRY(hipMemcpy(table, s->d_cut, kCutWords * sizeof(uint32_t), hipMemcpyDeviceToHost));
+    if (!s->last_fused_compacted) return CERES_OK;
+    const ceres_scene::CompactBuf* b = nullptr;
+    for (const auto& c : s->compact)
+        if (c.stream == s->last_fused_stream) b = &c;
+    if (!b || !b->d) return set_error(CERES_EINVAL, "ceres_debug_entry_nodes: the launch's buffer is gone");
+    if (!b->entry_off) return CERES_OK;
+    const uint32_t off = b->entry_off & ~kEntryDebug, n_rect = b->frames * kCutMax;
+    uint32_t res[2] = {0, 0};
+    HIP_TRY(hipMemcpy(res, b->d + b->off_result, sizeof res, hipMemcpyDeviceToHost));
+    const uint32_t n_entries = (b->entry_off & kEntryDebug) ? b->n : 0u;
+    info[1] = 1; info[2] = b->frames; info[3] = n_entries; info[4] = b->W; info[5] = b->H; info[6] = res[1];
+    if (rects) {
+        if (cap < n_rect) return set_error(CERES_EINVAL, "ceres_debug_entry_nodes: %u rectangles needed", n_rect);
+        std::vector<uint32_t> w(size_t(n_rect) * 2);
+        HIP_TRY(hipMemcpy(w.data(), b->d + off, w.size() * sizeof(uint32_t), hipMemcpyDeviceToHost));
+        for (size_t k = 0; k < n_rect; ++k) {
+            rects[4 * k] = uint16_t(w[2 * k]); rects[4 * k + 1] = uint16_t(w[2 * k] >> 16);
+            rects[4 * k + 2] = uint16_t(w[2 * k + 1]); rects[4 * k + 3] = uint16_t(w[2 * k + 1] >> 16);
+        }
+    }
+    if (entries && n_entries) {
+        if (cap < n_entries) return set_error(CERES_EINVAL, "ceres_debug_entry_nodes: %u entries needed", n_entries);
+        HIP_TRY(hipMemcpy(entries, b->d + off + size_t(n_rect) * 2, size_t(n_entries) * sizeof(uint32_t), hipMemcpyDeviceToHost));
+    }
+    return CERES_OK;
+}
+
 int ceres_fetch_counters(int device, uint64_t out[8], int reset) {
     if (!out) return set_error(CERES_EINVAL, "ceres_fetch_counters: null argument");
 #if CERES_COUNTING
diff --git a/ceres-raytracer_amd/csrc/scene_internal.hpp b/ceres-raytracer_amd/csrc/scene_internal.hpp
--- a/ceres-raytracer_amd/csrc/scene_internal.hpp
+++ b/ceres-raytracer_amd/csrc/scene_internal.hpp
@@ -47,7 +47,10 @@
         uint64_t used = 0;
         const uint32_t* src = nullptr;
         uint32_t n = 0, host_tiles = 0, tpw = 0, deal = 0, off_result = 0;
+        uint32_t entry_off = 0, frames = 0, W = 0, H = 0;
     };
+    uint32_t* d_cut = nullptr;
+    bool entry_debug = false;
     std::vector<CompactBuf> compact;
     hipStream_t last_fused_stream = nullptr;
     bool last_fused_compacted = false;
@@ -105,6 +108,7 @@
 void scene_release(ceres_scene* s);
 int scene_after_refit(ceres_scene* s, const float root[6], const SiblingPair& p0);
 int scene_adopt_layout(ceres_scene* s, ceres::DeviceLayout& L, hipStream_t stream);
+int scene_refresh_cut(ceres_scene* s, const float* d_root_box, hipStream_t stream);
 constexpr uint32_t kCostBlocks = 512;
 int frame_tile_order(ceres_scene* s, size_t W, size_t H, uint32_t tile, hipStream_t stream, const uint32_t** out);
 constexpr size_t kMaxTileOrders = 16;
diff --git a/ceres-raytracer_amd/csrc/scene_refit.hip b/ceres-raytracer_amd/csrc/scene_refit.hip
--- a/ceres-raytracer_amd/csrc/scene_refit.hip
+++ b/ceres-raytracer_amd/csrc/scene_refit.hip
@@ -224,6 +224,7 @@
         hipLaunchKernelGGL(k_root_box, dim3(1), dim3(64), 0, st, s->d_pairs, s->d_tris, nt, s->root_leaf_count, s->root_leaf_first,
                            s->d_refit_root);
         RF_TRY(hipGetLastError());
+        if (int rc = scene_refresh_cut(s, s->d_refit_root, st)) return rc;
         float h[18];
         RF_TRY(hipMemcpyAsync(h, s->d_refit_root, sizeof h, hipMemcpyDeviceToHost, st));
         RF_TRY(hipStreamSynchronize(st));
diff --git a/include/ceres_render.h b/include/ceres_render.h
--- a/include/ceres_render.h
+++ b/include/ceres_render.h
@@ -207,6 +207,15 @@
 int ceres_debug_kept_tiles(size_t width, size_t height, uint32_t frames, uint32_t tiles_per_wave, const uint16_t* rects,
                            uint32_t info[4], uint32_t* source, size_t cap);
 
+size_t ceres_entry_cut_words(void);
+int ceres_entry_cut_build(const void* pairs64, size_t n_pairs, uint32_t root_leaf_count, const float root_box[6], uint32_t* table);
+int ceres_entry_relayout(const float* tri48, size_t n_tri, const void* nodes32, size_t n_nodes, const uint64_t* prim64,
+                         void* pairs64, size_t* n_pairs, uint32_t* orig, uint32_t* root_leaf_count);
+int ceres_entry_rects(const uint32_t* table, const float basis12[12], size_t width, size_t height, uint16_t* rects);
+int ceres_entry_tiles(const uint32_t* table, const uint16_t* rects, size_t width, size_t height, uint32_t* entries);
+int ceres_debug_entry_record(ceres_scene* scene, int enable);
+int ceres_debug_entry_nodes(ceres_scene* scene, uint32_t info[8], uint32_t* table, uint16_t* rects, uint32_t* entries, size_t cap);
+
 int ceres_fetch_counters(int device, uint64_t out[8], int reset);
 
 typedef struct ceres_cpu_scene ceres_cpu_scene;
```

Measured after the change: 54170 Mrays/s (median of 6 runs). +2.8%, better.
